# GlacioHack/xdem

Hardware: AMD Instinct MI355X
Metric: Mpixels/s full terrain-attribute set, 40000² f32 DEM; variogram Gpairs/s (higher is better)
Workload: dtype f32 in/out, mixed f64/f32 arithmetic (f64 where cancellation demands: stencil sums, curvature numerators, discriminants); 1 GPU; 40000x40000 float32 fBm DEM (H=0.7, 1000+-300 m, res 10 m), Florinsky fit, geometric curvatures, 11 attributes, device-resident in/out (planes: the library's scattered 32 MiB-piece backing, kept by the allocator's calibration of both placements before the warm-up); partition=1 row block(s), halo depth 2, bytes_per_pixel=48, rccl_ranks=1, visible_gpus=1

## Files before the change

include/xdemhip.h:

```cpp
#ifndef XDEMHIP_H
#define XDEMHIP_H

#include <stdint.h>

#ifdef __cplusplus
extern "C" {
#endif

typedef struct xdemhip_ctx xdemhip_ctx;

enum { XDEMHIP_OK = 0, XDEMHIP_EINVAL = -1, XDEMHIP_ENODEV = -2, XDEMHIP_EHIP = -3, XDEMHIP_ENOMEM = -4,
       XDEMHIP_EUNSUPPORTED = -5 };
enum { XDEMHIP_F32 = 0, XDEMHIP_F64 = 1 };
enum { XDEMHIP_HOST = 0, XDEMHIP_DEVICE = 1 };

enum { XDEMHIP_FIT_HORN = 0, XDEMHIP_FIT_ZEVENBERGTHORNE = 1, XDEMHIP_FIT_FLORINSKY = 2 };
enum { XDEMHIP_CURV_GEOMETRIC = 0, XDEMHIP_CURV_DIRECTIONAL = 1 };
enum { XDEMHIP_TRI_RILEY = 0, XDEMHIP_TRI_WILSON = 1 };

enum {
    XDEMHIP_ATTR_SLOPE = 1u << 0,
    XDEMHIP_ATTR_ASPECT = 1u << 1,
    XDEMHIP_ATTR_HILLSHADE = 1u << 2,
    XDEMHIP_ATTR_CURVATURE = 1u << 3,
    XDEMHIP_ATTR_PROFILE_CURVATURE = 1u << 4,
    XDEMHIP_ATTR_TANGENTIAL_CURVATURE = 1u << 5,
    XDEMHIP_ATTR_PLANFORM_CURVATURE = 1u << 6,
    XDEMHIP_ATTR_FLOWLINE_CURVATURE = 1u << 7,
    XDEMHIP_ATTR_MAX_CURVATURE = 1u << 8,
    XDEMHIP_ATTR_MIN_CURVATURE = 1u << 9,
    XDEMHIP_ATTR_TPI = 1u << 10,
    XDEMHIP_ATTR_TRI = 1u << 11,
    XDEMHIP_ATTR_ROUGHNESS = 1u << 12,
    XDEMHIP_ATTR_RUGOSITY = 1u << 13,
    XDEMHIP_ATTR_FRACTAL_ROUGHNESS = 1u << 14,
    XDEMHIP_ATTR_COUNT = 15
};

int xdemhip_version(void);
int xdemhip_create(int device_id, xdemhip_ctx** out_ctx);
void xdemhip_destroy(xdemhip_ctx* ctx);
const char* xdemhip_last_error(const xdemhip_ctx* ctx);
#define XDEMHIP_OWN_STREAM ((void*)(intptr_t)-1)
int xdemhip_set_stream(xdemhip_ctx* ctx, void* hip_stream);
int xdemhip_synchronize(xdemhip_ctx* ctx);
enum { XDEMHIP_ALLOC_CONTIGUOUS = 1, XDEMHIP_ALLOC_RECYCLED = 2, XDEMHIP_ALLOC_CHUNKED = 4, XDEMHIP_ALLOC_SCATTERED = 8 };
int xdemhip_device_alloc(xdemhip_ctx* ctx, size_t bytes, int flags, void** ptr, int* got_contiguous);
int xdemhip_device_free(xdemhip_ctx* ctx, void* ptr);
int xdemhip_last_kernel_ms(xdemhip_ctx* ctx, float* ms);
int xdemhip_clock_probe(xdemhip_ctx* ctx, void* hip_stream, int sleeps, uint64_t* out_device);
int xdemhip_set_option(xdemhip_ctx* ctx, const char* name, int value);

enum { XDEMHIP_RED_SUM_U64 = 0, XDEMHIP_RED_SUM_F64 = 1, XDEMHIP_RED_MIN_U64 = 2, XDEMHIP_RED_MAX_U64 = 3 };
typedef int (*xdemhip_allreduce_fn)(void* host_array, int64_t count, int kind, void* user);
int xdemhip_set_allreduce(xdemhip_ctx* ctx, xdemhip_allreduce_fn fn, void* user);
typedef int (*xdemhip_allreduce_device_fn)(void* device_array, int64_t count, int kind, void* hip_stream, void* user);
int xdemhip_set_allreduce_device(xdemhip_ctx* ctx, xdemhip_allreduce_device_fn fn, void* user);
int xdemhip_reduction_calls(xdemhip_ctx* ctx, int64_t* host_calls, int64_t* device_calls);
int xdemhip_host_ring_sample(const uint8_t* valid, int64_t ny, int64_t nx, double gsd, int64_t runs, const int64_t* cx, const int64_t* cy,
                             int n_rings, const double* ring_lo, const double* ring_hi, int64_t samples, uint64_t seed, int threads,
                             int64_t* out_idx, int64_t* out_count);
int xdemhip_host_gather_points(const void* values, int dtype, int64_t nx, double gsd, int n_blocks, const int64_t* off, const int64_t* idx,
                               int threads, double* x_out, double* y_out, void* v_out, double* sx_out, double* sy_out, void* sv_out);
int xdemhip_host_count_finite(const void* values, int dtype, int64_t n, int threads, int64_t* n_finite, uint8_t* valid_out);
int xdemhip_set_rank(xdemhip_ctx* ctx, int rank, int world);

int xdemhip_terrain(xdemhip_ctx* ctx, const void* dem, int dem_dtype, int64_t H, int64_t W, int64_t row_stride,
                    int64_t halo_top, int64_t halo_bottom, double resolution, int surface_fit, int curv_method,
                    uint32_t attr_mask, int tri_method, int window_size, double hillshade_altitude_deg,
                    double hillshade_azimuth_deg, double hillshade_z_factor, int degrees, int out_dtype,
                    void* const* out_planes, int memspace);

int xdemhip_fractal_constants(int window_size, int max_q, int* q, double* log_q, double* mean_log_q, double* ss_xx);

int xdemhip_texture_shading(xdemhip_ctx* ctx, const void* dem, int dem_dtype, int64_t H, int64_t W, double alpha, int out_dtype,
                            void* out, int memspace);

typedef struct xdemhip_nk_plan xdemhip_nk_plan;
int xdemhip_nk_create(xdemhip_ctx* ctx, const void* ref, const void* tba, const uint8_t* inlier_mask_or_null, int dtype,
                      int64_t H, int64_t W, int memspace, xdemhip_nk_plan** out_plan, int64_t* n_valid);
int xdemhip_nk_step(xdemhip_nk_plan* plan, double shift_x, double shift_y, double res_x, double res_y, int n_bins,
                    double* vshift, int64_t* n_valid, double* y_mean, double* y_std, double* edges, int64_t* counts,
                    double* medians);
int xdemhip_nk_create_block(xdemhip_ctx* ctx, const void* ref_block, const void* tba_block, const uint8_t* inlier_block_or_null,
                            int dtype, int64_t H, int64_t W, int64_t row_begin, int64_t row_end, int64_t halo_top,
                            int64_t halo_bottom, int memspace, xdemhip_nk_plan** out_plan, int64_t* n_valid);
int xdemhip_nk_set_rows(xdemhip_nk_plan* plan, int64_t row_begin, int64_t row_end, int64_t* n_valid);
int xdemhip_nk_step_fit(xdemhip_nk_plan* plan, double shift_x, double shift_y, double res_x, double res_y, double* vshift,
                        int64_t* n_valid, double* y_mean, double* y_std, double* sums );
int xdemhip_nk_step_values(xdemhip_nk_plan* plan, double shift_x, double shift_y, double res_x, double res_y, int n_bins, double* vshift,
                           int64_t* n_valid, double* y_mean, double* y_std, double* edges , void* y_out,
                           uint16_t* bins_out, int memspace);
int xdemhip_nk_set_bin_edges(xdemhip_nk_plan* plan, const double* edges, int n_edges, int decimal);
#define XDEMHIP_BINSTAT_MEDIAN 0
#define XDEMHIP_BINSTAT_MEAN 1
int xdemhip_nk_set_statistic(xdemhip_nk_plan* plan, int bin_stat);
int xdemhip_nk_get_aux(xdemhip_nk_plan* plan, void* slope_tan, void* aspect, uint8_t* valid);
int xdemhip_nk_subsample(xdemhip_nk_plan* plan, const int64_t* ranks, int64_t k, int memspace, int64_t* n_valid);
int xdemhip_nk_route_counts(xdemhip_nk_plan* plan, int64_t* onepass, int64_t* plain);
int xdemhip_nk_predict_counts(xdemhip_nk_plan* plan, int64_t* predicted, int64_t* predicted_dh_only, int64_t* missed);
void xdemhip_nk_destroy(xdemhip_nk_plan* plan);
int xdemhip_binned_median(xdemhip_ctx* ctx, const void* x, const void* y, int dtype, int64_t n, int n_bins, double* edges,
                          int64_t* counts, double* medians);

typedef struct xdemhip_dh_plan xdemhip_dh_plan;
int xdemhip_dh_create(xdemhip_ctx* ctx, const void* ref, const void* tba, const uint8_t* inlier_mask_or_null, int dtype, int64_t H, int64_t W,
                      int memspace, xdemhip_dh_plan** out_plan, int64_t* n_valid);
int xdemhip_dh_subsample(xdemhip_dh_plan* plan, const int64_t* ranks, int64_t k, int memspace, int64_t* n_drawn);
int xdemhip_dh_poly_moments(xdemhip_dh_plan* plan, int order, int64_t row_offset, int64_t H_global, int64_t W_global, double* m_out,
                            double* r_out, int64_t* count);
int xdemhip_dh_median(xdemhip_dh_plan* plan, double* median, int64_t* count);
int xdemhip_dh_values(xdemhip_dh_plan* plan, void* dh_out, int64_t* col_out, int64_t* row_out, int memspace, int64_t* count);
int xdemhip_dh_shift_nmad(xdemhip_dh_plan* plan, double shift_x, double shift_y, double res_x, double res_y, double nfact, double* median,
                          double* nmad, int64_t* count);
int xdemhip_dh_shift_values(xdemhip_dh_plan* plan, double shift_x, double shift_y, double res_x, double res_y, void* dh_out, int memspace,
                            int64_t* count);
void xdemhip_dh_destroy(xdemhip_dh_plan* plan);

enum { XDEMHIP_VAR_PLANE = 0, XDEMHIP_VAR_ROTATED = 1, XDEMHIP_VAR_REF = 2, XDEMHIP_VAR_TBA = 3 };
enum { XDEMHIP_CORR_GRID = 0, XDEMHIP_CORR_PERBIN = 1, XDEMHIP_CORR_POLY = 2, XDEMHIP_CORR_SUMSIN = 3 };
typedef struct xdemhip_varsrc {
    int kind;
    int dtype;
    const void* plane;
    double cos_t, sin_t, res_x, res_y, offset;
} xdemhip_varsrc;
int xdemhip_dh_restrict_finite(xdemhip_dh_plan* plan, const void* var, int dtype, int memspace, int64_t* n_valid);
int xdemhip_dh_var_columns(xdemhip_dh_plan* plan, int n_var, const xdemhip_varsrc* vars, void* dh_out, void* const* var_out, int memspace,
                           int64_t* count);
int xdemhip_corr_apply(xdemhip_ctx* ctx, const void* elev, int dtype, int64_t H, int64_t W, int kind, int n_var, const xdemhip_varsrc* vars,
                       const int* n_tab, const double* a, const double* b, const double* table, const unsigned char* pass, void* out,
                       int64_t* n_missing, int memspace);

int xdemhip_dh_lzd_gradients(xdemhip_dh_plan* plan, const double* transform6, void* gradx_out, void* grady_out, int memspace);
int xdemhip_dh_lzd_centroid(xdemhip_dh_plan* plan, const double* transform6, double* centroid_out, int64_t* count);
int xdemhip_dh_lzd_normal(xdemhip_dh_plan* plan, const double* transform6, const double* matrix16, const double* centroid3, double* sums_out,
                          int64_t* count);
int xdemhip_dh_lzd_values(xdemhip_dh_plan* plan, const double* transform6, const double* matrix16, const double* centroid3, double* out,
                          int64_t* count);
int xdemhip_apply_matrix_rst(xdemhip_ctx* ctx, const void* dem, int dtype, int64_t H, int64_t W, const double* transform6, const double* matrix16,
                             const double* centroid3_or_null, void* out, int memspace);

typedef struct xdemhip_pts_plan xdemhip_pts_plan;
int xdemhip_pts_create(xdemhip_ctx* ctx, const void* raster, const uint8_t* inlier_mask_or_null, int dtype, int64_t H, int64_t W,
                       const double* transform6, const double* x, const double* y, const void* z, int64_t n_pts, int pts_is_ref, int with_nk_aux,
                       int memspace, xdemhip_pts_plan** out_plan, int64_t* n_valid);
int xdemhip_pts_subsample(xdemhip_pts_plan* plan, const int64_t* ranks, int64_t k, int memspace, int64_t* n_selected);
int xdemhip_pts_selection(xdemhip_pts_plan* plan, int64_t* idx_out_or_null, int64_t* count);
int xdemhip_pts_set_bin_edges(xdemhip_pts_plan* plan, const double* edges_or_null, int n_edges, int decimal);
int xdemhip_pts_nk_step(xdemhip_pts_plan* plan, double shift_x, double shift_y, int n_bins, double* vshift, int64_t* n_valid, double* y_mean,
                        double* y_std, double* edges, int64_t* counts, double* medians);
int xdemhip_pts_step_y(xdemhip_pts_plan* plan, void* y_out, int memspace, int64_t* count);
int xdemhip_pts_shift_nmad(xdemhip_pts_plan* plan, double shift_x, double shift_y, double nfact, double* median, double* nmad, int64_t* count);
int xdemhip_pts_shift_values(xdemhip_pts_plan* plan, double shift_x, double shift_y, void* dh_out, void* slope_out_or_null,
                             void* aspect_out_or_null, int memspace, int64_t* count);
void xdemhip_pts_destroy(xdemhip_pts_plan* plan);
int xdemhip_apply_matrix_pts(xdemhip_ctx* ctx, const double* x, const double* y, const double* z, int64_t n, const double* matrix16,
                             const double* centroid3_or_null, int invert, double* x_out, double* y_out, double* z_out, int memspace);

typedef struct xdemhip_icp xdemhip_icp;
int xdemhip_dh_icp_normals(xdemhip_dh_plan* plan, const double* transform6, void* nx_out, void* ny_out, void* nz_out, int memspace, int64_t* n_valid);
int xdemhip_icp_create_plan(xdemhip_dh_plan* plan, const double* transform6, int with_normals, int standardize, xdemhip_icp** out, double* centroid3,
                            double* std_fac, int64_t* count);
int xdemhip_icp_create_points(xdemhip_ctx* ctx, const double* ref3n, int64_t n, const double* query3m, int64_t m, const double* norms3n_or_null,
                              xdemhip_icp** out);
int xdemhip_icp_cloud(xdemhip_icp* icp, double* out7n);
int xdemhip_icp_grid(xdemhip_icp* icp, double* x0_y0_h, int64_t* gx_gy);
int xdemhip_icp_query(xdemhip_icp* icp, const double* matrix16_or_null, int64_t* ind_out, double* dist_out);
int xdemhip_icp_set_pairs(xdemhip_icp* icp, const int64_t* ind, const double* dist);
int xdemhip_icp_pairs(xdemhip_icp* icp, int picky, int64_t* n_kept, int64_t* query_idx_out, int64_t* ref_idx_out);
int xdemhip_icp_sums(xdemhip_icp* icp, const double* step16, int method, double* sums_out, int64_t* count);
int xdemhip_icp_values(xdemhip_icp* icp, double* out9k);
void xdemhip_icp_destroy(xdemhip_icp* icp);

typedef struct xdemhip_cpd xdemhip_cpd;
int xdemhip_cpd_create_plan(xdemhip_dh_plan* plan, const double* transform6, int standardize, xdemhip_cpd** out, double* centroid3, double* std_fac,
                            int64_t* count);
int xdemhip_cpd_create_points(xdemhip_ctx* ctx, const double* ref3n, int64_t n, const double* tba3m, int64_t m, xdemhip_cpd** out);
int xdemhip_cpd_estep(xdemhip_cpd* cpd, const double* matrix16_or_null, double sigma2_or_nan, double weight, double* sums_out, double* sigma2_used);
int xdemhip_cpd_terms(xdemhip_cpd* cpd, double* p1_out, double* pt1_out, double* px_out);
void xdemhip_cpd_destroy(xdemhip_cpd* cpd);

int xdemhip_poly2d_apply(xdemhip_ctx* ctx, const void* elev, int dtype, int64_t H, int64_t W, int64_t row_offset, const double* coeffs,
// ... 79 lines not shown
```

xdem_amd/_lib.py:

```python
from __future__ import annotations

import contextlib
import ctypes
import os
import threading
import weakref

HERE = os.path.dirname(os.path.abspath(__file__))
LIB_PATH = os.path.join(HERE, "csrc", "libxdemhip.so")

OK = 0
F32, F64 = 0, 1
HOST, DEVICE = 0, 1

_lib = None
_lock = threading.Lock()


THIRDPARTY_DEFAULTS = {"nk_nan_rule": 0, "vario_edge": 0, "vario_diff": 0}
_THIRDPARTY_RANGE = {"nk_nan_rule": (0, 3), "vario_edge": (0, 1), "vario_diff": (0, 1)}


def thirdparty_decision() -> dict:
    import json
# ... 44 lines not shown
            raise XdemHipError(
                f"{LIB_PATH} is missing: build it with `python -c 'import __graft_entry__ as g; g.build()'` "
                "(hipcc --offload-arch=gfx950). xdem_amd has no CPU fallback."
            )
        try:
            import torch
        except Exception:
            pass
        L = ctypes.CDLL(LIB_PATH, mode=ctypes.RTLD_GLOBAL)
        c_ctx = ctypes.c_void_p
        L.xdemhip_version.restype = ctypes.c_int
        L.xdemhip_create.argtypes = [ctypes.c_int, ctypes.POINTER(c_ctx)]
        L.xdemhip_destroy.argtypes = [c_ctx]
        L.xdemhip_destroy.restype = None
        L.xdemhip_last_error.argtypes = [c_ctx]
        L.xdemhip_last_error.restype = ctypes.c_char_p
        L.xdemhip_set_stream.argtypes = [c_ctx, ctypes.c_void_p]
        L.xdemhip_synchronize.argtypes = [c_ctx]
        L.xdemhip_device_alloc.argtypes = [c_ctx, ctypes.c_size_t, ctypes.c_int, ctypes.POINTER(ctypes.c_void_p), ctypes.POINTER(ctypes.c_int)]
        L.xdemhip_device_free.argtypes = [c_ctx, ctypes.c_void_p]
        L.xdemhip_set_option.argtypes = [c_ctx, ctypes.c_char_p, ctypes.c_int]
        L.xdemhip_set_test_switch.argtypes = [c_ctx, ctypes.c_char_p, ctypes.c_int]
        L.xdemhip_set_allreduce.argtypes = [c_ctx, ctypes.c_void_p, ctypes.c_void_p]
        L.xdemhip_set_allreduce_device.argtypes = [c_ctx, ctypes.c_void_p, ctypes.c_void_p]
        L.xdemhip_reduction_calls.argtypes = [c_ctx, ctypes.POINTER(ctypes.c_int64), ctypes.POINTER(ctypes.c_int64)]
        L.xdemhip_set_rank.argtypes = [c_ctx, ctypes.c_int, ctypes.c_int]
        L.xdemhip_last_kernel_ms.argtypes = [c_ctx, ctypes.POINTER(ctypes.c_float)]
        L.xdemhip_clock_probe.argtypes = [c_ctx, ctypes.c_void_p, ctypes.c_int, ctypes.c_void_p]
        L.xdemhip_terrain.argtypes = [
            c_ctx, ctypes.c_void_p, ctypes.c_int, ctypes.c_int64, ctypes.c_int64, ctypes.c_int64, ctypes.c_int64,
            ctypes.c_int64, ctypes.c_double, ctypes.c_int, ctypes.c_int, ctypes.c_uint32, ctypes.c_int, ctypes.c_int,
            ctypes.c_double, ctypes.c_double, ctypes.c_double, ctypes.c_int, ctypes.c_int,
            ctypes.POINTER(ctypes.c_void_p), ctypes.c_int,
        ]
        c_i64p, c_dp = ctypes.POINTER(ctypes.c_int64), ctypes.POINTER(ctypes.c_double)
        L.xdemhip_fractal_constants.argtypes = [ctypes.c_int, ctypes.c_int, ctypes.POINTER(ctypes.c_int), c_dp, c_dp, c_dp]
        L.xdemhip_texture_shading.argtypes = [c_ctx, ctypes.c_void_p, ctypes.c_int, ctypes.c_int64, ctypes.c_int64, ctypes.c_double,
                                              ctypes.c_int, ctypes.c_void_p, ctypes.c_int]
        L.xdemhip_nk_create.argtypes = [c_ctx, ctypes.c_void_p, ctypes.c_void_p, ctypes.c_void_p, ctypes.c_int, ctypes.c_int64,
                                        ctypes.c_int64, ctypes.c_int, ctypes.POINTER(ctypes.c_void_p), c_i64p]
        L.xdemhip_nk_create_block.argtypes = [c_ctx, ctypes.c_void_p, ctypes.c_void_p, ctypes.c_void_p, ctypes.c_int, ctypes.c_int64,
                                              ctypes.c_int64, ctypes.c_int64, ctypes.c_int64, ctypes.c_int64, ctypes.c_int64,
                                              ctypes.c_int, ctypes.POINTER(ctypes.c_void_p), c_i64p]
        L.xdemhip_nk_step.argtypes = [ctypes.c_void_p, ctypes.c_double, ctypes.c_double, ctypes.c_double, ctypes.c_double,
                                      ctypes.c_int, c_dp, c_i64p, c_dp, c_dp, c_dp, c_i64p, c_dp]
        L.xdemhip_nk_step_fit.argtypes = [ctypes.c_void_p, ctypes.c_double, ctypes.c_double, ctypes.c_double, ctypes.c_double,
                                          c_dp, c_i64p, c_dp, c_dp, c_dp]
        L.xdemhip_nk_set_bin_edges.argtypes = [ctypes.c_void_p, c_dp, ctypes.c_int, ctypes.c_int]
        L.xdemhip_nk_get_aux.argtypes = [ctypes.c_void_p, ctypes.c_void_p, ctypes.c_void_p, ctypes.c_void_p]
        L.xdemhip_nk_destroy.argtypes = [ctypes.c_void_p]
        L.xdemhip_nk_destroy.restype = None
        L.xdemhip_binned_median.argtypes = [c_ctx, ctypes.c_void_p, ctypes.c_void_p, ctypes.c_int, ctypes.c_int64, ctypes.c_int,
                                            c_dp, c_i64p, c_dp]
        L.xdemhip_mean_filter_nan.argtypes = [c_ctx, ctypes.c_void_p, ctypes.c_int, ctypes.c_int64, ctypes.c_int64, ctypes.c_int,
                                              ctypes.c_int, ctypes.c_void_p, ctypes.c_void_p, ctypes.POINTER(ctypes.c_int), ctypes.c_int]
        L.xdemhip_binstats_bin_numbers.argtypes = [ctypes.c_void_p, ctypes.c_void_p]
        L.xdemhip_convolution.argtypes = [c_ctx, ctypes.c_void_p, ctypes.c_int, ctypes.c_int64, ctypes.c_int64, ctypes.c_int64, c_dp, ctypes.c_int,
                                          ctypes.c_int, ctypes.c_int, ctypes.c_int, ctypes.c_void_p, ctypes.c_int]
        L.xdemhip_perbin_lookup.argtypes = [c_ctx, ctypes.POINTER(ctypes.c_void_p), ctypes.POINTER(ctypes.c_int), ctypes.c_int, ctypes.c_int64,
                                            ctypes.POINTER(ctypes.c_int), c_dp, c_dp, c_dp, ctypes.c_char_p, ctypes.c_int, ctypes.c_void_p,
                                            c_i64p, ctypes.c_int]
        L.xdemhip_bw_create.argtypes = [c_ctx, ctypes.c_void_p, ctypes.c_void_p, ctypes.c_void_p, ctypes.c_int, ctypes.c_int64, ctypes.c_int64,
                                        ctypes.c_int, c_i64p, ctypes.c_int, ctypes.POINTER(ctypes.c_void_p), c_i64p]
        L.xdemhip_bw_nk_step.argtypes = [ctypes.c_void_p, ctypes.c_void_p, c_dp, c_dp, ctypes.c_double, ctypes.c_double, ctypes.c_int,
                                         c_dp, c_i64p, c_dp, c_dp, c_dp, c_i64p, c_dp]
        L.xdemhip_bw_get_aux.argtypes = [ctypes.c_void_p, ctypes.c_void_p, ctypes.c_void_p, ctypes.c_void_p]
        L.xdemhip_bw_destroy.argtypes = [ctypes.c_void_p]
        L.xdemhip_bw_destroy.restype = None
        L.xdemhip_bw_apply.argtypes = [c_ctx, ctypes.c_void_p, ctypes.c_int, ctypes.c_int64, ctypes.c_int64, c_dp, c_dp, c_dp, c_dp,
                                       ctypes.c_void_p, ctypes.c_int]
        L.xdemhip_shift_bilinear.argtypes = [c_ctx, ctypes.c_void_p, ctypes.c_int, ctypes.c_int64, ctypes.c_int64, ctypes.c_double,
                                             ctypes.c_double, ctypes.c_double, ctypes.c_void_p, ctypes.c_int]
        L.xdemhip_set_allreduce.argtypes = [c_ctx, ctypes.c_void_p, ctypes.c_void_p]
        L.xdemhip_nk_set_rows.argtypes = [ctypes.c_void_p, ctypes.c_int64, ctypes.c_int64, c_i64p]
        L.xdemhip_nk_set_statistic.argtypes = [ctypes.c_void_p, ctypes.c_int]
        L.xdemhip_nk_route_counts.argtypes = [ctypes.c_void_p, c_i64p, c_i64p]
        L.xdemhip_host_ring_sample.argtypes = [ctypes.c_void_p, ctypes.c_int64, ctypes.c_int64, ctypes.c_double, ctypes.c_int64, c_i64p, c_i64p,
                                               ctypes.c_int, c_dp, c_dp, ctypes.c_int64, ctypes.c_uint64, ctypes.c_int, c_i64p, c_i64p]
        L.xdemhip_host_gather_points.argtypes = [ctypes.c_void_p, ctypes.c_int, ctypes.c_int64, ctypes.c_double, ctypes.c_int, c_i64p, c_i64p,
                                                 ctypes.c_int, c_dp, c_dp, ctypes.c_void_p, c_dp, c_dp, ctypes.c_void_p]
        L.xdemhip_nk_step_values.argtypes = [ctypes.c_void_p, ctypes.c_double, ctypes.c_double, ctypes.c_double, ctypes.c_double, ctypes.c_int,
                                             c_dp, c_i64p, c_dp, c_dp, c_dp, ctypes.c_void_p, ctypes.c_void_p, ctypes.c_int]
        L.xdemhip_nk_predict_counts.argtypes = [ctypes.c_void_p, c_i64p, c_i64p, c_i64p]
        L.xdemhip_nk_subsample.argtypes = [ctypes.c_void_p, ctypes.c_void_p, ctypes.c_int64, ctypes.c_int, c_i64p]
        L.xdemhip_host_count_finite.argtypes = [ctypes.c_void_p, ctypes.c_int, ctypes.c_int64, ctypes.c_int, c_i64p, ctypes.c_void_p]
        c_u64p = ctypes.POINTER(ctypes.c_uint64)
        L.xdemhip_pairs_create.argtypes = [c_ctx, ctypes.c_int, ctypes.c_void_p, ctypes.c_void_p, ctypes.c_void_p, ctypes.c_void_p,
                                           ctypes.c_void_p, ctypes.c_void_p, ctypes.c_void_p, ctypes.c_void_p, ctypes.c_int,
                                           ctypes.c_void_p, ctypes.c_int, ctypes.c_int, ctypes.POINTER(ctypes.c_void_p), c_i64p]
        L.xdemhip_pairs_sums.argtypes = [ctypes.c_void_p, ctypes.c_int, c_dp, c_i64p]
        L.xdemhip_pairs_hist.argtypes = [ctypes.c_void_p, ctypes.c_int, ctypes.c_int, c_u64p, c_u64p]
        L.xdemhip_pairs_succ.argtypes = [ctypes.c_void_p, c_u64p, c_u64p]
        L.xdemhip_pairs_medians.argtypes = [ctypes.c_void_p, c_i64p, c_dp]
        L.xdemhip_pairs_link_sorted.argtypes = [ctypes.c_void_p, ctypes.c_void_p]
        L.xdemhip_pairs_link_shadow.argtypes = [ctypes.c_void_p, ctypes.c_void_p]
        L.xdemhip_pairs_takes_brackets.argtypes = [ctypes.c_void_p, ctypes.POINTER(ctypes.c_int)]
        L.xdemhip_pairs_destroy.argtypes = [ctypes.c_void_p]
        L.xdemhip_pairs_destroy.restype = None
        c_ip = ctypes.POINTER(ctypes.c_int)
        L.xdemhip_binstats_create.argtypes = [c_ctx, ctypes.c_void_p, ctypes.c_int, ctypes.c_int64, ctypes.c_int,
                                              ctypes.POINTER(ctypes.c_void_p)]
        L.xdemhip_binstats_add_var.argtypes = [ctypes.c_void_p, ctypes.c_void_p, ctypes.c_int, ctypes.c_int]
        L.xdemhip_binstats_finalize.argtypes = [ctypes.c_void_p, c_i64p, c_dp, c_dp]
        L.xdemhip_binstats_run.argtypes = [ctypes.c_void_p, ctypes.c_int, c_ip, c_dp, c_ip, c_ip, ctypes.c_int, ctypes.c_int,
                                           ctypes.c_double, c_i64p, c_dp, c_dp]
        L.xdemhip_binstats_destroy.argtypes = [ctypes.c_void_p]
        L.xdemhip_binstats_destroy.restype = None
        L.xdemhip_cov_double_sum.argtypes = [c_ctx, c_dp, c_dp, c_dp, ctypes.c_int64, c_dp, c_dp, c_dp, ctypes.c_int64, ctypes.c_int, c_ip,
                                             c_dp, c_dp, c_dp, c_dp, ctypes.c_int]
        L.xdemhip_nmad.argtypes = [c_ctx, ctypes.c_void_p, ctypes.c_int, ctypes.c_int64, ctypes.c_double, ctypes.c_double,
                                   ctypes.c_int, c_dp, c_dp, c_i64p]
        L.xdemhip_interp_grid_linear.argtypes = [c_ctx, ctypes.c_int, c_dp, c_ip, c_dp, ctypes.POINTER(ctypes.c_void_p), c_ip,
                                                 ctypes.c_int64, ctypes.c_double, c_dp, ctypes.c_int]
        L.xdemhip_dh_create.argtypes = [c_ctx, ctypes.c_void_p, ctypes.c_void_p, ctypes.c_void_p, ctypes.c_int, ctypes.c_int64,
                                        ctypes.c_int64, ctypes.c_int, ctypes.POINTER(ctypes.c_void_p), c_i64p]
        L.xdemhip_dh_subsample.argtypes = [ctypes.c_void_p, ctypes.c_void_p, ctypes.c_int64, ctypes.c_int, c_i64p]
        L.xdemhip_dh_poly_moments.argtypes = [ctypes.c_void_p, ctypes.c_int, ctypes.c_int64, ctypes.c_int64, ctypes.c_int64, c_dp, c_dp,
                                              c_i64p]
        L.xdemhip_dh_median.argtypes = [ctypes.c_void_p, c_dp, c_i64p]
        L.xdemhip_dh_values.argtypes = [ctypes.c_void_p, ctypes.c_void_p, ctypes.c_void_p, ctypes.c_void_p, ctypes.c_int, c_i64p]
        L.xdemhip_dh_shift_nmad.argtypes = [ctypes.c_void_p, ctypes.c_double, ctypes.c_double, ctypes.c_double, ctypes.c_double, ctypes.c_double,
                                            c_dp, c_dp, c_i64p]
        L.xdemhip_dh_shift_values.argtypes = [ctypes.c_void_p, ctypes.c_double, ctypes.c_double, ctypes.c_double, ctypes.c_double,
                                              ctypes.c_void_p, ctypes.c_int, c_i64p]
        L.xdemhip_dh_destroy.argtypes = [ctypes.c_void_p]
        L.xdemhip_dh_destroy.restype = None
        L.xdemhip_dh_lzd_gradients.argtypes = [ctypes.c_void_p, c_dp, ctypes.c_void_p, ctypes.c_void_p, ctypes.c_int]
        L.xdemhip_dh_lzd_centroid.argtypes = [ctypes.c_void_p, c_dp, c_dp, c_i64p]
        L.xdemhip_dh_lzd_normal.argtypes = [ctypes.c_void_p, c_dp, c_dp, c_dp, c_dp, c_i64p]
        L.xdemhip_dh_lzd_values.argtypes = [ctypes.c_void_p, c_dp, c_dp, c_dp, c_dp, c_i64p]
        L.xdemhip_dh_restrict_finite.argtypes = [ctypes.c_void_p, ctypes.c_void_p, ctypes.c_int, ctypes.c_int, c_i64p]
        L.xdemhip_dh_var_columns.argtypes = [ctypes.c_void_p, ctypes.c_int, ctypes.POINTER(VarSrc), ctypes.c_void_p,
                                             ctypes.POINTER(ctypes.c_void_p), ctypes.c_int, c_i64p]
        L.xdemhip_corr_apply.argtypes = [c_ctx, ctypes.c_void_p, ctypes.c_int, ctypes.c_int64, ctypes.c_int64, ctypes.c_int, ctypes.c_int,
                                         ctypes.POINTER(VarSrc), c_ip, c_dp, c_dp, c_dp, ctypes.c_char_p, ctypes.c_void_p, c_i64p, ctypes.c_int]
        L.xdemhip_dh_icp_normals.argtypes = [ctypes.c_void_p, c_dp, ctypes.c_void_p, ctypes.c_void_p, ctypes.c_void_p, ctypes.c_int, c_i64p]
        L.xdemhip_icp_create_plan.argtypes = [ctypes.c_void_p, c_dp, ctypes.c_int, ctypes.c_int, ctypes.POINTER(ctypes.c_void_p), c_dp, c_dp, c_i64p]
        L.xdemhip_icp_create_points.argtypes = [c_ctx, c_dp, ctypes.c_int64, c_dp, ctypes.c_int64, c_dp, ctypes.POINTER(ctypes.c_void_p)]
        L.xdemhip_icp_cloud.argtypes = [ctypes.c_void_p, c_dp]
        L.xdemhip_icp_grid.argtypes = [ctypes.c_void_p, c_dp, c_i64p]
        L.xdemhip_icp_query.argtypes = [ctypes.c_void_p, c_dp, c_i64p, c_dp]
        L.xdemhip_icp_set_pairs.argtypes = [ctypes.c_void_p, c_i64p, c_dp]
        L.xdemhip_icp_pairs.argtypes = [ctypes.c_void_p, ctypes.c_int, c_i64p, c_i64p, c_i64p]
        L.xdemhip_icp_sums.argtypes = [ctypes.c_void_p, c_dp, ctypes.c_int, c_dp, c_i64p]
        L.xdemhip_icp_values.argtypes = [ctypes.c_void_p, c_dp]
        L.xdemhip_icp_destroy.argtypes = [ctypes.c_void_p]
        L.xdemhip_icp_destroy.restype = None
        L.xdemhip_cpd_create_plan.argtypes = [ctypes.c_void_p, c_dp, ctypes.c_int, ctypes.POINTER(ctypes.c_void_p), c_dp, c_dp, c_i64p]
        L.xdemhip_cpd_create_points.argtypes = [c_ctx, c_dp, ctypes.c_int64, c_dp, ctypes.c_int64, ctypes.POINTER(ctypes.c_void_p)]
        L.xdemhip_cpd_estep.argtypes = [ctypes.c_void_p, c_dp, ctypes.c_double, ctypes.c_double, c_dp, c_dp]
        L.xdemhip_cpd_terms.argtypes = [ctypes.c_void_p, c_dp, c_dp, c_dp]
        L.xdemhip_cpd_destroy.argtypes = [ctypes.c_void_p]
        L.xdemhip_cpd_destroy.restype = None
        L.xdemhip_apply_matrix_rst.argtypes = [c_ctx, ctypes.c_void_p, ctypes.c_int, ctypes.c_int64, ctypes.c_int64, c_dp, c_dp, c_dp,
                                               ctypes.c_void_p, ctypes.c_int]
        L.xdemhip_pts_create.argtypes = [c_ctx, ctypes.c_void_p, ctypes.c_void_p, ctypes.c_int, ctypes.c_int64, ctypes.c_int64, c_dp,
                                         ctypes.c_void_p, ctypes.c_void_p, ctypes.c_void_p, ctypes.c_int64, ctypes.c_int, ctypes.c_int,
                                         ctypes.c_int, ctypes.POINTER(ctypes.c_void_p), c_i64p]
        L.xdemhip_pts_subsample.argtypes = [ctypes.c_void_p, ctypes.c_void_p, ctypes.c_int64, ctypes.c_int, c_i64p]
        L.xdemhip_pts_selection.argtypes = [ctypes.c_void_p, ctypes.c_void_p, c_i64p]
        L.xdemhip_pts_set_bin_edges.argtypes = [ctypes.c_void_p, c_dp, ctypes.c_int, ctypes.c_int]
        L.xdemhip_pts_nk_step.argtypes = [ctypes.c_void_p, ctypes.c_double, ctypes.c_double, ctypes.c_int, c_dp, c_i64p, c_dp, c_dp, c_dp,
                                          c_i64p, c_dp]
        L.xdemhip_pts_step_y.argtypes = [ctypes.c_void_p, ctypes.c_void_p, ctypes.c_int, c_i64p]
        L.xdemhip_pts_shift_nmad.argtypes = [ctypes.c_void_p, ctypes.c_double, ctypes.c_double, ctypes.c_double, c_dp, c_dp, c_i64p]
        L.xdemhip_pts_shift_values.argtypes = [ctypes.c_void_p, ctypes.c_double, ctypes.c_double, ctypes.c_void_p, ctypes.c_void_p,
# ... 160 lines not shown
            self.check(self._L.xdemhip_set_allreduce(self.handle, None, None))
            self.check(self._L.xdemhip_set_rank(self.handle, 0, 0))
            return
        import torch.distributed as dist

        pg = None if group == "world" else group
        self.check(self._L.xdemhip_set_rank(self.handle, dist.get_rank(pg), dist.get_world_size(pg)))
        hook = make_reduce_hook(group, self.device)
        CB = ctypes.CFUNCTYPE(ctypes.c_int, ctypes.c_void_p, ctypes.c_int64, ctypes.c_int, ctypes.c_void_p)
        self._hook = CB(hook)
        self.check(self._L.xdemhip_set_allreduce(self.handle, ctypes.cast(self._hook, ctypes.c_void_p), None))
        if device_side is None:
            import torch.distributed as dist

            device_side = dist.get_backend(None if group == "world" else group) == "nccl"
        if device_side:
            CBD = ctypes.CFUNCTYPE(ctypes.c_int, ctypes.c_void_p, ctypes.c_int64, ctypes.c_int, ctypes.c_void_p, ctypes.c_void_p)
            self._dev_hook = CBD(make_device_reduce_hook(group, self.device))
            self.check(self._L.xdemhip_set_allreduce_device(self.handle, ctypes.cast(self._dev_hook, ctypes.c_void_p), None))
        else:
            self._dev_hook = None
            self.check(self._L.xdemhip_set_allreduce_device(self.handle, None, None))

    def reduction_calls(self) -> tuple[int, int]:
        h, d = ctypes.c_int64(), ctypes.c_int64()
        self.check(self._L.xdemhip_reduction_calls(self.handle, ctypes.byref(h), ctypes.byref(d)))
        return int(h.value), int(d.value)

    def synchronize(self) -> None:
        self.check(self._L.xdemhip_synchronize(self.handle))

    def device_tensor(self, shape, dtype="float32", contiguous: bool = True, recycled: bool = False, chunked: bool = False,
                      scattered: bool = False):
        import numpy as np
        import torch

        np_dt = np.dtype(dtype)
        count = int(np.prod(shape))
        ptr, got = ctypes.c_void_p(), ctypes.c_int()
        flags = 8 if scattered else (4 if chunked else ((1 if contiguous else 0) | (2 if recycled else 0)))
        nbytes = count * np_dt.itemsize
        pooled = self._take_pooled(nbytes, flags)
        if pooled:
            torch.cuda.synchronize(self.device)
            ptr.value, got.value = pooled, 0
        else:
            rc = self._L.xdemhip_device_alloc(self.handle, nbytes, flags, ctypes.byref(ptr), ctypes.byref(got))
            if rc != OK and self._pool:
                self.release_pool()
                rc = self._L.xdemhip_device_alloc(self.handle, nbytes, flags, ctypes.byref(ptr), ctypes.byref(got))
            self.check(rc)
        owner = _OwnedDeviceArray(self, int(ptr.value), count, np_dt.str, nbytes, flags)
        t = torch.as_tensor(owner, device=torch.device("cuda", self.device)).view(*shape)
        t.xdem_contiguous = bool(got.value)
        return t

    def _take_pooled(self, nbytes: int, flags: int) -> int:
        with self._pool_lock:
            for i, (b, f, p) in enumerate(self._pool):
                if b == nbytes and f == flags:
                    del self._pool[i]
                    return p
        return 0

    def _give_back(self, ptr: int, nbytes: int, flags: int) -> None:
        if flags == 8 and 0 < nbytes <= self._pool_cap:
            evict = []
            with self._pool_lock:
                self._pool.append((nbytes, flags, ptr))
                while sum(b for b, _, _ in self._pool) > self._pool_cap:
                    evict.append(self._pool.pop(0))
            for _, _, p in evict:
                self._L.xdemhip_device_free(self.handle, ctypes.c_void_p(p))
            return
        self._L.xdemhip_device_free(self.handle, ctypes.c_void_p(ptr))

    def release_pool(self) -> None:
        with self._pool_lock:
            items, self._pool = self._pool, []
        for _, _, p in items:
            self._L.xdemhip_device_free(self.handle, ctypes.c_void_p(p))

    TEST_SWITCHES = frozenset(("terrain_stream", "terrain_order", "terrain_ring_wait", "terrain_window_lds", "nk_narrow",
                               "vario_grid", "vario_runs", "vario_sort", "hypso_seg_lds", "pts_tile_order", "bw_seg_lds"))

    def set_option(self, name: str, value: int) -> None:
        fn = self._L.xdemhip_set_test_switch if name in self.TEST_SWITCHES else self._L.xdemhip_set_option
        self.check(fn(self.handle, name.encode(), int(value)))
        self.options[name] = int(value)

    @contextlib.contextmanager
    def option_scope(self, name: str, value: int):
        with self.call_lock:
            prev = self.options.get(name, 0)
            if int(value) != prev:
                self.set_option(name, value)
            try:
                yield
            finally:
                if int(value) != prev:
                    self.set_option(name, prev)

    def clock_probe(self, stream, out, sleeps: int = 2000) -> None:
        self.check(self._L.xdemhip_clock_probe(self.handle, ctypes.c_void_p(int(stream.cuda_stream)), int(sleeps), ctypes.c_void_p(int(out.data_ptr()))))

    def last_kernel_ms(self) -> float:
        ms = ctypes.c_float()
        self.check(self._L.xdemhip_last_kernel_ms(self.handle, ctypes.byref(ms)))
        return float(ms.value)

    def adopt(self, obj) -> None:
        self._dependants.add(obj)

    def close(self) -> None:
        if getattr(self, "handle", None):
            for obj in list(getattr(self, "_dependants", ())):
                try:
                    obj.close()
                except Exception:
                    pass
            self.release_pool()
            self._L.xdemhip_destroy(self.handle)
            self.handle = None

    def __del__(self) -> None:
        try:
            self.close()
        except Exception:
            pass


_default_ctx: dict[int, Context] = {}
_ctx_lock = threading.Lock()
_tls = threading.local()


class use_context:

    def __init__(self, ctx: Context):
        self.ctx = ctx

    def __enter__(self):
        self.prev = getattr(_tls, "ctx", None)
        _tls.ctx = self.ctx
        return self.ctx

    def __exit__(self, *exc):
        _tls.ctx = self.prev
        return False


def default_context(device: int | None = None) -> Context:
    cur = getattr(_tls, "ctx", None)
    if cur is not None and (device is None or device == cur.device):
        return cur
    if device is None:
        device = int(os.environ.get("XDEM_AMD_DEVICE", os.environ.get("LOCAL_RANK", "0")))
    if device not in _default_ctx:
        with _ctx_lock:
            if device not in _default_ctx:
                _default_ctx[device] = Context(device)
    return _default_ctx[device]
```

xdem_amd/coreg.py:

```python
from __future__ import annotations

import ctypes
import logging
import warnings
from typing import Any, Callable

import numpy as np
import scipy.optimize

from . import _lib
from . import epc as _epc
from ._coregbase import NO_VALID, CoregPipeline, _Plan, _Step, apply_translation, draw, raster_pair
from ._coregbase import subsample_ranks, subsample_valid_mask
from .biascorr import Deramp, DhPlan, VerticalShift, _check_weights, polynomial_2d
from .bincorr import BiasCorr, DirectionalBias, TerrainBias, rotated_x
from .rigid import (LZD, apply_matrix, invert_matrix, matrix_from_translations_rotations,
                    translations_rotations_from_matrix, _make_matrix_valid)
from .icp import ICP, nearest
from .cpd import CPD, cpd_expectation, cpd_update
from .epc import EPC
from .blockwise import BlockwiseCoreg, tiling_grid
from .spatialstats import nmad

TWO_CLOUDS = ("This pre-processing function is only intended for raster-point or raster-raster methods, "
# ... 66 lines not shown
        if group is not None and block is None:
            import torch.distributed as dist

            from .dist import row_block

            pg = None if group == "world" else group
            r0, r1 = row_block(self.shape[0], dist.get_world_size(pg), dist.get_rank(pg))
            self.ctx.set_allreduce(group)
            self.ctx.check(self.ctx._L.xdemhip_nk_set_rows(self.handle, r0, r1, ctypes.byref(nv)))
            self.n_valid = int(nv.value)

    def step(self, shift_x: float, shift_y: float, res: tuple[float, float], n_bins: int = 72) -> dict[str, Any]:
        n_bins = getattr(self, "_n_custom_bins", None) or int(n_bins)
        if getattr(self, "_bin_callable", None) is not None:
            return self._step_callable(shift_x, shift_y, res, n_bins)
        edges = np.empty(n_bins + 1, dtype=np.float64)
        counts = np.empty(n_bins, dtype=np.int64)
        med = np.empty(n_bins, dtype=np.float64)
        vshift, ymean, ystd = ctypes.c_double(), ctypes.c_double(), ctypes.c_double()
        nv = ctypes.c_int64()
        dp, ip = ctypes.POINTER(ctypes.c_double), ctypes.POINTER(ctypes.c_int64)
        rc = self.ctx._L.xdemhip_nk_step(self.handle, float(shift_x), float(shift_y), float(res[0]), float(res[1]), int(n_bins),
                                         ctypes.byref(vshift), ctypes.byref(nv), ctypes.byref(ymean), ctypes.byref(ystd),
                                         edges.ctypes.data_as(dp), counts.ctypes.data_as(ip), med.ctypes.data_as(dp))
        if rc != _lib.OK:
            self._raise_step_error(rc)
        return {"vshift": vshift.value, "n_valid": int(nv.value), "y_mean": ymean.value, "y_std": ystd.value,
                "edges": edges, "counts": counts, "medians": med}

    def _step_callable(self, shift_x: float, shift_y: float, res: tuple[float, float], n_bins: int) -> dict[str, Any]:
        if self.group is not None:
            raise NotImplementedError("a bin_statistic other than np.nanmedian / np.nanmean needs all values of a bin in one process: "
                                      "not available for partitioned (group=...) fits")
        if getattr(self, "_vals", None) is None:
            self._vals = (np.empty(self.shape, dtype=self.dtype), np.empty(self.shape, dtype=np.uint16))
        y, bins = self._vals
        edges = np.empty(n_bins + 1, dtype=np.float64)
        vshift, ymean, ystd = ctypes.c_double(), ctypes.c_double(), ctypes.c_double()
        nv = ctypes.c_int64()
        dp = ctypes.POINTER(ctypes.c_double)
        rc = self.ctx._L.xdemhip_nk_step_values(self.handle, float(shift_x), float(shift_y), float(res[0]), float(res[1]), int(n_bins),
                                                ctypes.byref(vshift), ctypes.byref(nv), ctypes.byref(ymean), ctypes.byref(ystd),
                                                edges.ctypes.data_as(dp), y.ctypes.data, bins.ctypes.data, _lib.HOST)
        if rc != _lib.OK:
            self._raise_step_error(rc)
        ok = (bins != 0xFFFF) & np.isfinite(y)
        b, v = bins[ok], y[ok]
        counts = np.bincount(b, minlength=n_bins).astype(np.int64)
        from ._binstat_host import binned_statistic_host

        stat = binned_statistic_host(self._bin_callable, b, v, n_bins)
        return {"vshift": vshift.value, "n_valid": int(nv.value), "y_mean": ymean.value, "y_std": ystd.value,
                "edges": edges, "counts": counts, "medians": stat}

    def _raise_step_error(self, rc: int) -> None:
        msg = self.ctx._L.xdemhip_last_error(self.ctx.handle).decode()
        if "no more valid values" in msg:
            raise ValueError(
                "The subsample contains no more valid values. This can happen is the horizontal shift to "
                "correct is very large, or if the algorithm diverged. To ensure all possible points can "
                "be used at any iteration step, use subsample=1."
            )
        if "halo too small" in msg:
            raise HaloTooSmall(msg)
        raise _lib.XdemHipError(f"libxdemhip status {rc}: {msg}")

    def step_fit(self, shift_x: float, shift_y: float, res: tuple[float, float]) -> dict[str, Any]:
        sums = np.empty(10, dtype=np.float64)
        vshift, ymean, ystd = ctypes.c_double(), ctypes.c_double(), ctypes.c_double()
        nv = ctypes.c_int64()
        dp = ctypes.POINTER(ctypes.c_double)
        rc = self.ctx._L.xdemhip_nk_step_fit(self.handle, float(shift_x), float(shift_y), float(res[0]), float(res[1]),
                                             ctypes.byref(vshift), ctypes.byref(nv), ctypes.byref(ymean), ctypes.byref(ystd),
                                             sums.ctypes.data_as(dp))
        if rc != _lib.OK:
            self._raise_step_error(rc)
        return {"vshift": vshift.value, "n_valid": int(nv.value), "y_mean": ymean.value, "y_std": ystd.value, "sums": sums}

    def route_counts(self) -> dict[str, int]:
        a, c = ctypes.c_int64(), ctypes.c_int64()
        self.ctx.check(self.ctx._L.xdemhip_nk_route_counts(self.handle, ctypes.byref(a), ctypes.byref(c)))
        p, d, m = ctypes.c_int64(), ctypes.c_int64(), ctypes.c_int64()
        self.ctx.check(self.ctx._L.xdemhip_nk_predict_counts(self.handle, ctypes.byref(p), ctypes.byref(d), ctypes.byref(m)))
        return {"onepass": int(a.value), "plain": int(c.value), "predicted": int(p.value),
                "predicted_dh_only": int(d.value), "predict_missed": int(m.value)}

    def set_bin_edges(self, edges) -> None:
        dp = ctypes.POINTER(ctypes.c_double)
        if edges is None:
            self.ctx.check(self.ctx._L.xdemhip_nk_set_bin_edges(self.handle, None, 0, 0))
            self._n_custom_bins = None
            return
        e = np.ascontiguousarray(edges, dtype=np.float64).ravel()
        decimal = int(-np.log10(np.diff(e.astype(self.dtype)).min())) + 6
        self.ctx.check(self.ctx._L.xdemhip_nk_set_bin_edges(self.handle, e.ctypes.data_as(dp), int(e.size), decimal))
        self._n_custom_bins = int(e.size) - 1

    def set_statistic(self, bin_statistic) -> None:
        sid = _bin_statistic_id(bin_statistic)
        self._bin_callable = bin_statistic if sid == 2 else None
        self.ctx.check(self.ctx._L.xdemhip_nk_set_statistic(self.handle, 0 if sid == 2 else sid))

    def aux(self):
        st = np.empty(self.shape, dtype=self.dtype)
        asp = np.empty(self.shape, dtype=self.dtype)
        valid = np.empty(self.shape, dtype=np.uint8)
        self.ctx.check(self.ctx._L.xdemhip_nk_get_aux(self.handle, st.ctypes.data, asp.ctypes.data, valid.ctypes.data))
        return st, asp, valid.astype(bool)

    def subsample(self, ranks: np.ndarray) -> int:
        ranks = np.ascontiguousarray(ranks, dtype=np.int64)
        nv = ctypes.c_int64()
        self.ctx.check(self.ctx._L.xdemhip_nk_subsample(self.handle, ranks.ctypes.data, int(ranks.size), _lib.HOST, ctypes.byref(nv)))
        self.n_valid = int(nv.value)
        return self.n_valid

    def close(self) -> None:
        hooked = getattr(self, "handle", None) and getattr(self.ctx, "handle", None) and getattr(self, "group", None) is not None
        super().close()
        if hooked:
            self.ctx.set_allreduce(None)


def binned_median(x: np.ndarray, y: np.ndarray, n_bins: int = 72, ctx: _lib.Context | None = None):
    x = np.ascontiguousarray(x).ravel()
    y = np.ascontiguousarray(y).ravel()
    dt = np.float64 if np.float64 in (x.dtype, y.dtype) else np.float32
    x, y = x.astype(dt, copy=False), y.astype(dt, copy=False)
    ctx = ctx or _lib.default_context()
    edges = np.empty(n_bins + 1, dtype=np.float64)
    counts = np.empty(n_bins, dtype=np.int64)
    med = np.empty(n_bins, dtype=np.float64)
    dp, ip = ctypes.POINTER(ctypes.c_double), ctypes.POINTER(ctypes.c_int64)
    ctx.check(ctx._L.xdemhip_binned_median(ctx.handle, x.ctypes.data, y.ctypes.data, _lib.F32 if dt == np.float32 else _lib.F64,
                                           x.size, int(n_bins), edges.ctypes.data_as(dp), counts.ctypes.data_as(ip),
                                           med.ctypes.data_as(dp)))
    return edges, counts, med


def _bin_fit_from_step(det: dict[str, Any], fit_optimizer: Callable[..., Any], dtype) -> tuple[float, float, float]:
    p0 = (3 * det["y_std"] / (2**0.5), 0.0, det["y_mean"])
    edges = det["edges"]
    mids = 0.5 * (edges[:-1] + edges[1:])
    med = det["medians"]
    ok = np.isfinite(med) & np.isfinite(mids)
    if np.all(~ok):
        raise ValueError("Only NaN values after binning, did you pass the right bin edges?")
    results = fit_optimizer(f=_nuth_kaab_fit_func, xdata=mids[ok], ydata=med[ok], p0=p0, sigma=None, absolute_sigma=True)
    a, b, c = results[0]
    return a * np.sin(b), a * np.cos(b), c


def _fit_from_sums(det: dict[str, Any]) -> tuple[float, float, float]:
    n, sc, ss, scc, sss, scs, sy, syc, sys_, _ = det["sums"]
    m = np.array([[scc, scs, sc], [scs, sss, ss], [sc, ss, n]], dtype=np.float64)
    rhs = np.array([syc, sys_, sy], dtype=np.float64)
    a_, b_, c_ = np.linalg.lstsq(m, rhs, rcond=None)[0]
    return float(b_), float(a_), float(c_)


def _check_unbinned_optimizer(fit_optimizer, bin_before_fit: bool) -> None:
    import scipy.optimize

    if not bin_before_fit and fit_optimizer is not None and fit_optimizer is not scipy.optimize.curve_fit:
        raise NotImplementedError(
            "bin_before_fit=False is solved from least-squares sums on the GPU, which equals scipy.optimize.curve_fit only; "
            "a custom fit_optimizer would need every point on the host. Use bin_before_fit=True with it."
        )
# ... 295 lines not shown
```

xdem_amd/csrc/capi.hip:

```cpp
#include <math.h>
#include <string.h>

#include <functional>
#include <mutex>
#include <thread>
#include <vector>

#include "common.h"

#define XDEMHIP_VERSION_NUM 100

extern "C" {

int xdemhip_version(void) { return XDEMHIP_VERSION_NUM; }

int xdemhip_create(int device_id, xdemhip_ctx** out_ctx) {
    if (!out_ctx) return XDEMHIP_EINVAL;
    *out_ctx = nullptr;
    int n = 0;
    if (hipGetDeviceCount(&n) != hipSuccess || n <= 0) return XDEMHIP_ENODEV;
    if (device_id < 0 || device_id >= n) return XDEMHIP_ENODEV;
    xdemhip_ctx* c = new xdemhip_ctx();
    c->device = device_id;
    if (hipSetDevice(device_id) != hipSuccess) { delete c; return XDEMHIP_EHIP; }
// ... 185 lines not shown
bool device_free_chunked(void* p) {
    ChunkedAlloc c;
    {
        std::lock_guard<std::mutex> lock(g_chunk_mu);
        size_t i = 0;
        for (; i < g_chunked.size(); ++i)
            if (g_chunked[i].base == p) break;
        if (i == g_chunked.size()) return false;
        c = std::move(g_chunked[i]);
        g_chunked.erase(g_chunked.begin() + (long)i);
    }
    (void)hipDeviceSynchronize();
    chunked_release(c, c.pieces.size());
    return true;
}
}

int xdemhip_device_alloc(xdemhip_ctx* ctx, size_t bytes, int flags, void** ptr, int* got_contiguous) {
    if (!ctx || !ptr || bytes == 0) return ctx ? xd_fail(ctx, XDEMHIP_EINVAL, "bad argument") : XDEMHIP_EINVAL;
    XD_HIP_CHECK(ctx, hipSetDevice(ctx->device));
    if (flags & (XDEMHIP_ALLOC_CHUNKED | XDEMHIP_ALLOC_SCATTERED)) {
        *ptr = nullptr;
        if (got_contiguous) *got_contiguous = 0;
        const bool scattered = (flags & XDEMHIP_ALLOC_SCATTERED) != 0;
        size_t piece_mb = scattered ? 32 : 64;
        if (const char* e = getenv("XDEMHIP_SCATTER_PIECE_MB")) {
            const long v = atol(e);
            if (scattered && v >= 1 && v <= 4096) piece_mb = (size_t)v;
        }
        return device_alloc_chunked(ctx, bytes, piece_mb << 20, scattered, ptr);
    }
    const bool contiguous = (flags & XDEMHIP_ALLOC_CONTIGUOUS) != 0;
    if (flags & XDEMHIP_ALLOC_RECYCLED) {
        void* first = nullptr;
        int rc = device_alloc_once(ctx, bytes, contiguous, &first, nullptr);
        if (rc) return rc;
        const size_t touch = bytes < ((size_t)64 << 20) ? bytes : ((size_t)64 << 20);
        (void)hipMemsetAsync(first, 0, touch, ctx->stream);
        (void)hipMemsetAsync(static_cast<char*>(first) + (bytes - touch), 0, touch, ctx->stream);
        (void)hipStreamSynchronize(ctx->stream);
        XD_HIP_CHECK(ctx, hipFree(first));
    }
    return device_alloc_once(ctx, bytes, contiguous, ptr, got_contiguous);
}

int xdemhip_device_free(xdemhip_ctx* ctx, void* ptr) {
    if (!ctx) return XDEMHIP_EINVAL;
    if (!ptr) return XDEMHIP_OK;
    XD_HIP_CHECK(ctx, hipSetDevice(ctx->device));
    if (device_free_chunked(ptr)) return XDEMHIP_OK;
    XD_HIP_CHECK(ctx, hipFree(ptr));
    return XDEMHIP_OK;
}

int xdemhip_synchronize(xdemhip_ctx* ctx) {
    if (!ctx) return XDEMHIP_EINVAL;
    XD_HIP_CHECK(ctx, hipSetDevice(ctx->device));
    XD_HIP_CHECK(ctx, hipStreamSynchronize(ctx->stream));
    return XDEMHIP_OK;
}

namespace {
struct XdOpt { const char* name; int lo, hi; int xdemhip_ctx::*field; const char* what; };
const XdOpt kOptions[] = {
    {"host_chunk_mb", 0, 1 << 30, &xdemhip_ctx::host_chunk_mb, "host_chunk_mb must be >= 0"},
    {"host_chunk_rows", 0, 1 << 30, &xdemhip_ctx::host_chunk_rows, "host_chunk_rows must be >= 0"},
    {"pairs_launch_cap", 0, 1 << 30, &xdemhip_ctx::pairs_launch_cap, "pairs_launch_cap must be >= 0"},
    {"terrain_nonfinite", 0, 1, &xdemhip_ctx::terrain_nonfinite, "terrain_nonfinite: 0 window rule (SciPy engine), 1 arithmetic rule (Numba engine)"},
    {"terrain_math", 0, 2, &xdemhip_ctx::terrain_math, "terrain_math: 0 mixed precision, 1 float64, 2 lean"},
    {"vario_edge", 0, 1, &xdemhip_ctx::vario_edge, "vario_edge: 0 or 1"},
    {"vario_diff", 0, 1, &xdemhip_ctx::vario_diff, "vario_diff: 0 or 1"},
    {"nk_nan_rule", 0, 3, &xdemhip_ctx::nk_nan_rule, "nk_nan_rule: 0 4tap, 1 weighted, 2 dilate3x3, 3 dilate_cross"},
    {"selection", 0, 3, &xdemhip_ctx::selection_mode, "selection: 0 auto, 1 plain, 2 degenerate brackets, 3 bracketed"},
    {"nk_fused", 0, 1, &xdemhip_ctx::nk_fused, "nk_fused: 0 or 1"},
    {"nk_fused_dist", 0, 1, &xdemhip_ctx::nk_fused_dist, "nk_fused_dist: 0 or 1"},
    {"nk_predict", 0, 1, &xdemhip_ctx::nk_predict, "nk_predict: 0 or 1"},
};
const XdOpt kTestSwitches[] = {
    {"terrain_stream", 0, 512, &xdemhip_ctx::terrain_stream, "terrain_stream: 0, 1, 2, 3, 128, 256 or 512"},
    {"terrain_order", 0, 3, &xdemhip_ctx::terrain_order, "terrain_order: 0 XCD bands, 1 natural order, 2 permuted strips, 3 column-major strips"},
    {"terrain_ring_wait", 0, 1, &xdemhip_ctx::terrain_ring_wait, "terrain_ring_wait: 0 counted wait, 1 vmcnt(0)"},
    {"terrain_window_lds", 0, 1, &xdemhip_ctx::terrain_window_lds, "terrain_window_lds: 0 or 1"},
    {"nk_narrow", -1, 2, &xdemhip_ctx::nk_narrow, "nk_narrow: -1 (adaptive), 0, 1 or 2"},
    {"vario_grid", 0, 1, &xdemhip_ctx::vario_grid, "vario_grid: 0 or 1"},
    {"vario_runs", 0, 1, &xdemhip_ctx::vario_runs, "vario_runs: 0 or 1"},
    {"vario_sort", 0, 1, &xdemhip_ctx::vario_sort, "vario_sort: 0 or 1"},
    {"pts_tile_order", 0, 1, &xdemhip_ctx::pts_tile_order, "pts_tile_order: 0 or 1"},
    {"bw_seg_lds", 0, 4096, &xdemhip_ctx::bw_seg_lds, "bw_seg_lds: 0 (default: 4096) or 1 to 4096 values"},
    {"hypso_seg_lds", 0, 16384, &xdemhip_ctx::hypso_seg_lds, "hypso_seg_lds: 0 (default: 8192) or 1 to 16384 values"},
};
int xd_set_from(xdemhip_ctx* ctx, const XdOpt* tab, size_t n, const char* name, int value, bool* found) {
    *found = false;
    for (size_t k = 0; k < n; ++k)
        if (const XdOpt& o = tab[k]; strcmp(o.name, name) == 0) {
            *found = true;
            if (value < o.lo || value > o.hi) return xd_fail(ctx, XDEMHIP_EINVAL, o.what);
            ctx->*(o.field) = value;
            return XDEMHIP_OK;
        }
    return XDEMHIP_OK;
}
}

int xdemhip_set_option(xdemhip_ctx* ctx, const char* name, int value) {
    if (!ctx || !name) return XDEMHIP_EINVAL;
    if (strcmp(name, "host_release") == 0) {
        for (int q = 0; q < 2; ++q) {
            if (ctx->stage_in[q]) (void)hipHostFree(ctx->stage_in[q]);
            if (ctx->stage_out[q]) (void)hipHostFree(ctx->stage_out[q]);
            ctx->stage_in[q] = ctx->stage_out[q] = nullptr;
        }
        ctx->stage_in_bytes = ctx->stage_out_bytes = 0;
        return XDEMHIP_OK;
    }
    if (strcmp(name, "host_copy_threads") == 0) {
        if (value < 0 || value > xdemhip_ctx::MAX_COPY_THREADS) return xd_fail(ctx, XDEMHIP_EINVAL, "host_copy_threads must be 0..16");
        ctx->host_copy_threads = value ? value : 8;
        return XDEMHIP_OK;
    }
    bool found = false;
    const int rc = xd_set_from(ctx, kOptions, sizeof kOptions / sizeof kOptions[0], name, value, &found);
    if (found) return rc;
    for (const XdOpt& o : kTestSwitches)
        if (strcmp(o.name, name) == 0) return xd_fail(ctx, XDEMHIP_EINVAL, std::string(name) + " is a test switch, not an option: xdemhip_set_test_switch (include/xdemhip_test.h)");
    return xd_fail(ctx, XDEMHIP_EINVAL, std::string("unknown option: ") + name);
}

int xdemhip_set_test_switch(xdemhip_ctx* ctx, const char* name, int value) {
    if (!ctx || !name) return XDEMHIP_EINVAL;
    if (strcmp(name, "terrain_stream") == 0 && !(value == 0 || value == 1 || value == 2 || value == 3 || value == 128 || value == 256 || value == 512))
        return xd_fail(ctx, XDEMHIP_EINVAL, "terrain_stream: 0, 1, 2, 3, 128, 256 or 512");
    bool found = false;
    const int rc = xd_set_from(ctx, kTestSwitches, sizeof kTestSwitches / sizeof kTestSwitches[0], name, value, &found);
    if (found) return rc;
    return xd_fail(ctx, XDEMHIP_EINVAL, std::string("unknown test switch: ") + name);
}

int xdemhip_last_kernel_ms(xdemhip_ctx* ctx, float* ms) {
    if (!ctx || !ms) return XDEMHIP_EINVAL;
    if (!ctx->timed) return xd_fail(ctx, XDEMHIP_EINVAL, "no timed launch on this context yet");
    XD_HIP_CHECK(ctx, hipEventSynchronize(ctx->ev_stop));
    XD_HIP_CHECK(ctx, hipEventElapsedTime(ms, ctx->ev_start, ctx->ev_stop));
    return XDEMHIP_OK;
}

static __global__ void xd_clock_probe_kernel(uint64_t* out, int sleeps) {
    const uint64_t t0 = wall_clock64(), c0 = clock64();
    for (int i = 0; i < sleeps; ++i) __builtin_amdgcn_s_sleep(127);
    const uint64_t t1 = wall_clock64(), c1 = clock64();
    if (threadIdx.x == 0) { out[0] = c1 - c0; out[1] = t1 - t0; }
}

int xdemhip_clock_probe(xdemhip_ctx* ctx, void* hip_stream, int sleeps, uint64_t* out_device) {
    if (!ctx || !out_device || sleeps < 1) return XDEMHIP_EINVAL;
    XD_HIP_CHECK(ctx, hipSetDevice(ctx->device));
    hipLaunchKernelGGL(xd_clock_probe_kernel, dim3(1), dim3(64), 0, static_cast<hipStream_t>(hip_stream), out_device, sleeps);
    XD_HIP_CHECK(ctx, hipGetLastError());
    return XDEMHIP_OK;
}

int xdemhip_fractal_constants(int window_size, int max_q, int* q, double* log_q, double* mean_log_q, double* ss_xx) {
    if (window_size < 3 || (window_size & 1) == 0 || window_size > 1023 || !q || !log_q || !mean_log_q || !ss_xx)
        return XDEMHIP_EINVAL;
    int qs[24];
    double x[24];
    const int n = xd::fractal_constants(window_size, qs, x, mean_log_q, ss_xx);
// ... 216 lines not shown
```

xdem_amd/csrc/common.h:

```cpp
#pragma once
#include <hip/hip_runtime.h>
#include <stdint.h>
#include <stdio.h>
#include <string.h>
#include <string>
#include <thread>
#include <vector>

#include "../../include/xdemhip.h"

struct xdemhip_ctx {
    int device = 0;
    hipStream_t own_stream = nullptr;
    hipStream_t stream = nullptr;
    hipEvent_t ev_start = nullptr, ev_stop = nullptr, ev_copy = nullptr;
    static constexpr int MAX_COPY_THREADS = 16;
    hipStream_t copy_streams[MAX_COPY_THREADS] = {};
    int host_copy_threads = 8;
    void* stage_in[2] = {nullptr, nullptr};
    void* stage_out[2] = {nullptr, nullptr};
    size_t stage_in_bytes = 0, stage_out_bytes = 0;
    int pairs_launch_cap = 0;
    bool timed = false;
    int num_cu = 256;
    xdemhip_allreduce_fn allreduce = nullptr;
    void* allreduce_user = nullptr;
    xdemhip_allreduce_device_fn allreduce_dev = nullptr;
    void* allreduce_dev_user = nullptr;
    int64_t n_red_host = 0, n_red_dev = 0;
    int rank = 0, world = 0;
    int nk_fused_dist = 1;
    int host_chunk_rows = 0;
    int host_chunk_mb = 0;
    int nk_narrow = -1;
    int vario_runs = 1;
    int vario_sort = 1;
    int nk_predict = 1;
    int nk_fused = 1;
    int terrain_stream = 1;
    int terrain_order = 0;
    int terrain_window_lds = 1;
    int terrain_ring_wait = 0;
    int terrain_nonfinite = 0;
    int* nf_flag = nullptr;
    int terrain_math = 2;
    int vario_grid = 1;
    int vario_edge = 0;
    int vario_diff = 0;
    int nk_nan_rule = 0;
    int pts_tile_order = 0;
    int hypso_seg_lds = 0;
    int bw_seg_lds = 0;
    int selection_mode = 0;
    unsigned char* pin = nullptr;
    size_t pin_cap = 0, pin_used = 0;
    struct Pending { void* dst; size_t off, bytes; };
    std::vector<Pending> pending;
    std::string err;
};

#define XD_HIP_CHECK(ctx, expr)                                                                   \
    do {                                                                                          \
        hipError_t _e = (expr);                                                                   \
        if (_e != hipSuccess) {                                                                   \
            char _b[512];                                                                         \
            snprintf(_b, sizeof _b, "%s failed: %s (%s:%d)", #expr, hipGetErrorString(_e), __FILE__, __LINE__); \
            (ctx)->err = _b;                                                                      \
            return XDEMHIP_EHIP;                                                                  \
        }                                                                                         \
    } while (0)

inline int xd_fail(xdemhip_ctx* ctx, int code, const std::string& msg) {
    if (ctx) ctx->err = msg;
    return code;
}

inline int launched(xdemhip_ctx* ctx, const char* what) {
    return hipGetLastError() == hipSuccess ? XDEMHIP_OK : xd_fail(ctx, XDEMHIP_EHIP, std::string(what) + " launch failed");
}

inline int xd_sync(xdemhip_ctx* ctx);

struct XdBuffers {
    xdemhip_ctx* ctx;
    const char* who;
    int rc = XDEMHIP_OK;
    struct Out { void* host; const void* dev; size_t bytes; };
    std::vector<void*> owned;
    std::vector<Out> outs;
    XdBuffers(xdemhip_ctx* c, const char* w) : ctx(c), who(w) {}
    void* alloc(size_t bytes) {
        void* p = nullptr;
        if (rc != XDEMHIP_OK) return nullptr;
        if (hipMalloc(&p, bytes) != hipSuccess) {
            (void)hipGetLastError();
            rc = xd_fail(ctx, XDEMHIP_ENOMEM, std::string("hipMalloc failed (") + who + ")");
            return nullptr;
        }
        if (p) owned.push_back(p);
        return p;
    }
    template <typename T> T* alloc(size_t count) { return static_cast<T*>(alloc(count * sizeof(T))); }
    template <typename T> const T* input(const T* src, size_t bytes, int memspace) {
        if (memspace == XDEMHIP_DEVICE || !src) return src;
        T* d = static_cast<T*>(alloc(bytes));
        if (d && hipMemcpyAsync(d, src, bytes, hipMemcpyHostToDevice, ctx->stream) != hipSuccess) {
            rc = xd_fail(ctx, XDEMHIP_EHIP, std::string("H2D copy failed (") + who + ")");
            return nullptr;
        }
        return d;
    }
    template <typename T> T* output(T* dst, size_t bytes, int memspace) {
        if (memspace == XDEMHIP_DEVICE || !dst) return dst;
        T* d = static_cast<T*>(alloc(bytes));
        if (d) outs.push_back({dst, d, bytes});
        return d;
    }
    int finish() {
        for (const Out& o : outs)
            if (rc == XDEMHIP_OK && hipMemcpyAsync(o.host, o.dev, o.bytes, hipMemcpyDeviceToHost, ctx->stream) != hipSuccess)
// ... 162 lines not shown
```

xdem_amd/csrc/nk_onepass.h:

```cpp
#pragma once

namespace xd {

__device__ __forceinline__ unsigned long long cm_nlt(float a, float b) { unsigned long long m; asm("v_cmp_nlt_f32_e64 %0, %1, %2" : "=s"(m) : "v"(a), "v"(b)); return m; }
__device__ __forceinline__ unsigned long long cm_ngt(float a, float b) { unsigned long long m; asm("v_cmp_ngt_f32_e64 %0, %1, %2" : "=s"(m) : "v"(a), "v"(b)); return m; }
__device__ __forceinline__ unsigned long long cm_nlt(double a, double b) { unsigned long long m; asm("v_cmp_nlt_f64_e64 %0, %1, %2" : "=s"(m) : "v"(a), "v"(b)); return m; }
__device__ __forceinline__ unsigned long long cm_ngt(double a, double b) { unsigned long long m; asm("v_cmp_ngt_f64_e64 %0, %1, %2" : "=s"(m) : "v"(a), "v"(b)); return m; }
__device__ __forceinline__ uint32_t sel_mask(uint32_t a, uint32_t b, unsigned long long mask) {
    uint32_t r;
    asm("v_cndmask_b32_e64 %0, %1, %2, %3" : "=v"(r) : "v"(a), "v"(b), "s"(mask));
    return r;
}
__device__ __forceinline__ float sel_mask(float a, float b, unsigned long long mask) { return __uint_as_float(sel_mask(__float_as_uint(a), __float_as_uint(b), mask)); }
__device__ __forceinline__ int sel_mask(int a, int b, unsigned long long mask) { return (int)sel_mask((uint32_t)a, (uint32_t)b, mask); }
__device__ __forceinline__ uint32_t* sel_mask_ptr(uint32_t* a, uint32_t* b, unsigned long long mask) {
    typedef __attribute__((address_space(3))) uint32_t* lp;
    const uint32_t r = sel_mask((uint32_t)(uintptr_t)(lp)a, (uint32_t)(uintptr_t)(lp)b, mask);
    return (uint32_t*)(lp)(uintptr_t)r;
}

template <typename T> struct FzEps;
template <> struct FzEps<float> { static constexpr float rel = 4e-6f, grow = 1.00002f, tiny = 1e-37f; };
template <> struct FzEps<double> { static constexpr double rel = 1e-14, grow = 1.0000000001, tiny = 1e-300; };
__device__ __forceinline__ float fz_rcp(float x) { return __builtin_amdgcn_rcpf(x); }
__device__ __forceinline__ double fz_rcp(double x) { return 1.0 / x; }

template <typename T>
__global__ void nk_fz_prep_kernel(const DhStats* stats, const unsigned long long* ext_survivors, int nb, int custom_edges, T* edges,
                                  BinCacheRec* rec, int force, unsigned long long* ctr) {
    typedef typename KeyT<T>::type K;
    if (threadIdx.x != 0 || blockIdx.x != 0) return;
    if (ext_survivors[0] == 0 || ext_survivors[1] == 0) { ctr[3] = 1ull; ctr[6] = 1ull; }
    if (!custom_edges) make_edges_into<T>((double)val_of((K)stats->asp_min), (double)val_of((K)stats->asp_max), nb, edges);
    const double e0 = (double)edges[0], eN = (double)edges[nb];
    rec->fresh = (!force && rec->nb == nb && rec->e0 == e0 && rec->eN == eN) ? 1 : 0;
}

template <typename T> __device__ __forceinline__ uint16_t fz_digitize(const T* e, double inv_width, int nb, T x, int last_decimal) {
    int idx = (int)(((double)x - (double)e[0]) * inv_width);
    idx = idx < 0 ? 0 : (idx > nb ? nb : idx);
    while (idx > 0 && !(e[idx] <= x)) --idx;
    while (idx < nb && e[idx + 1] <= x) ++idx;
    if (!(e[0] <= x)) idx = -1;
    if (idx == nb && on_last_edge<T>(x, e[nb], last_decimal)) idx = nb - 1;
    return (idx >= 0 && idx < nb) ? (uint16_t)idx : (uint16_t)0xFFFF;
}
template <typename T>
__global__ __launch_bounds__(256) void nk_bin_fill_kernel(const T* __restrict__ aspect, int64_t n, const T* __restrict__ edges, int nb,
                                                          int last_decimal, const BinCacheRec* rec, nk_bin_t* __restrict__ bcache) {
    if (rec->fresh == 1) return;
    extern __shared__ __attribute__((aligned(16))) unsigned char fz_smem[];
    T* e = reinterpret_cast<T*>(fz_smem);
    for (int k = threadIdx.x; k <= nb; k += blockDim.x) e[k] = edges[k];
    __syncthreads();
    const double inv_width = (double)nb / ((double)e[nb] - (double)e[0]);
    for (int64_t p = (int64_t)blockIdx.x * blockDim.x + threadIdx.x; p < n; p += (int64_t)gridDim.x * blockDim.x)
        bcache[p] = nk_bin8(fz_digitize<T>(e, inv_width, nb, aspect[p], last_decimal));
}

template <typename T>
__global__ __launch_bounds__(256) void nk_sample_dh_kernel(const T* __restrict__ ref_m, const T* __restrict__ tba, NkGeom g, int64_t q0, int64_t n,
                                                           double invW, int64_t n_slots, T* __restrict__ s_d, SelReset reset) {
    if (reset.base) select_reset_slice(reset, (int64_t)blockIdx.x * blockDim.x + threadIdx.x, (int64_t)gridDim.x * blockDim.x);
    for (int64_t i = (int64_t)blockIdx.x * blockDim.x + threadIdx.x; i < n_slots; i += (int64_t)gridDim.x * blockDim.x) {
        const int64_t p = (sel_sampled_line(i >> SEL_LINE_LOG2) << SEL_LINE_LOG2) + (i & (SEL_LINE - 1));
        T out = (T)NAN;
        if (p < n) {
            const int64_t q = q0 + p;
            int64_t li, j;
            row_col(q, g.W, invW, li, j);
            const BiTap t = bi_locate(g, li + g.roff, j);
            const BiVals<T> tv = bi_load<T>(tba, t);
            T val;
            const bool in = bi_value<T>(g, tba, t, tv.a00, tv.a01, tv.a10, tv.a11, val);
            const T d = t_sub(ref_m[q], val);
            if (in && t_finite(d)) out = d;
        }
        s_d[i] = out;
    }
}

template <typename T>
__device__ __forceinline__ bool nk_vhat_of(uint64_t sample_count, typename KeyT<T>::type lo, typename KeyT<T>::type hi, T& vhat, T& delta) {
    typedef typename KeyT<T>::type K;
    if (sample_count == 0) { vhat = (T)0; delta = (T)0; return false; }
    const K mid = (K)(lo + (K)((K)(hi - lo) >> 1));
    const double vl = (double)val_of(lo), vh = (double)val_of(hi), vm = (double)val_of(mid);
    const double d = fmax(vm - vl, vh - vm);
    vhat = val_of(mid);
    T df = (T)(d * 1.000001 + 1e-300);
    if ((double)df < d * 1.0000005) df = (T)((double)df * 1.000001);
    delta = df;
    return (vl <= vm && vm <= vh) && t_finite((T)vl) && t_finite((T)vh);
}

template <typename T>
__global__ __launch_bounds__(256) void nk_sample_y_kernel(T* __restrict__ s_v, uint16_t* __restrict__ s_b, const T* __restrict__ slope_tan,
                                                          const nk_bin_t* __restrict__ bcache, int64_t n, int64_t n_slots, const T* vhat_p,
                                                          const typename KeyT<T>::type* klo_d = nullptr, const typename KeyT<T>::type* khi_d = nullptr,
                                                          T* vhat_out = nullptr, T* delta_out = nullptr, unsigned long long* ctr = nullptr,
                                                          SelReset reset = SelReset()) {
    T vhat;
    if (klo_d) {
        typedef typename KeyT<T>::type K;
        T delta;
        const K lo = klo_d[0], hi = khi_d[0];
        const bool ok = nk_vhat_of<T>((lo == (K)0 && hi == (K)~(K)0) ? 0u : 1u, lo, hi, vhat, delta);
        if (blockIdx.x == 0 && threadIdx.x == 0) {
            *vhat_out = vhat;
            *delta_out = delta;
            if (!ok) ctr[3] = 1ull;
        }
    } else {
        vhat = *vhat_p;
    }
    if (reset.base) select_reset_slice(reset, (int64_t)blockIdx.x * blockDim.x + threadIdx.x, (int64_t)gridDim.x * blockDim.x);
    for (int64_t i = (int64_t)blockIdx.x * blockDim.x + threadIdx.x; i < n_slots; i += (int64_t)gridDim.x * blockDim.x) {
        const int64_t p = (sel_sampled_line(i >> SEL_LINE_LOG2) << SEL_LINE_LOG2) + (i & (SEL_LINE - 1));
        const T d = s_v[i];
        T y = (T)NAN;
        uint16_t b = 0xFFFF;
        if (p < n && d == d) {
            b = nk_bin16(bcache[p]);
            y = t_div(t_sub(d, vhat), slope_tan[p]);
            if (b == 0xFFFF || !(y == y)) y = (T)NAN;
        }
        s_v[i] = y;
        s_b[i] = b;
    }
}

template <typename T>
__global__ __launch_bounds__(256) void nk_sample_dy_kernel(const T* __restrict__ ref_m, const T* __restrict__ tba, NkGeom g, int64_t q0, int64_t n,
                                                           double invW, int64_t n_slots, T* __restrict__ s_v, uint16_t* __restrict__ s_b,
                                                           const T* __restrict__ slope_tan , const nk_bin_t* __restrict__ bcache ,
                                                           const typename KeyT<T>::type* klo_d, const typename KeyT<T>::type* khi_d, T* vhat_out,
                                                           T* delta_out, unsigned long long* ctr, SelReset reset) {
    typedef typename KeyT<T>::type K;
    T vhat, delta;
    const K lo = klo_d[0], hi = khi_d[0];
    const bool ok = nk_vhat_of<T>((lo == (K)0 && hi == (K)~(K)0) ? 0u : 1u, lo, hi, vhat, delta);
    if (blockIdx.x == 0 && threadIdx.x == 0) {
        *vhat_out = vhat;
        *delta_out = delta;
        if (!ok) ctr[3] = 1ull;
    }
    if (reset.base) select_reset_slice(reset, (int64_t)blockIdx.x * blockDim.x + threadIdx.x, (int64_t)gridDim.x * blockDim.x);
    for (int64_t i = (int64_t)blockIdx.x * blockDim.x + threadIdx.x; i < n_slots; i += (int64_t)gridDim.x * blockDim.x) {
        const int64_t p = (sel_sampled_line(i >> SEL_LINE_LOG2) << SEL_LINE_LOG2) + (i & (SEL_LINE - 1));
        T y = (T)NAN;
        uint16_t b = 0xFFFF;
        if (p < n) {
            const int64_t q = q0 + p;
            int64_t li, j;
            row_col(q, g.W, invW, li, j);
            const BiTap t = bi_locate(g, li + g.roff, j);
            const BiVals<T> tv = bi_load<T>(tba, t);
            T val;
            const bool in = bi_value<T>(g, tba, t, tv.a00, tv.a01, tv.a10, tv.a11, val);
            const T d = t_sub(ref_m[q], val);
            if (in && t_finite(d)) {
                b = nk_bin16(bcache[p]);
                y = t_div(t_sub(d, vhat), slope_tan[p]);
                if (b == 0xFFFF || !(y == y)) y = (T)NAN;
            }
        }
        s_v[i] = y;
        s_b[i] = b;
    }
}

constexpr int NK_PREDICT_MAX_BINS = 128;
template <typename T> struct NkPredicted { T dlo, dhi; T lo[NK_PREDICT_MAX_BINS], hi[NK_PREDICT_MAX_BINS]; };
template <typename T>
__global__ __launch_bounds__(64) void nk_predict_kernel(const NkPredicted<T> pr, int nb, typename KeyT<T>::type* klo_d, typename KeyT<T>::type* khi_d,
                                                        uint32_t* rbs_d, T* vhat, T* delta, typename KeyT<T>::type* klo_y,
                                                        typename KeyT<T>::type* khi_y, uint32_t* rbs_y, unsigned long long* ctr) {
    typedef typename KeyT<T>::type K;
    const int lane = threadIdx.x;
    K r = 0;
    for (int b = lane; b < nb; b += 64) {
        K lo = (K)0, hi = (K)~(K)0;
        if (pr.lo[b] <= pr.hi[b]) { lo = key_of(pr.lo[b]); hi = key_of(pr.hi[b]); }
        klo_y[b] = lo;
        khi_y[b] = hi;
        const K d = hi >= lo ? (K)(hi - lo) : (K)0;
        r = d > r ? d : r;
    }
    for (int off = 32; off > 0; off >>= 1) {
        const K o = k_shfl_down(r, off);
        r = o > r ? o : r;
    }
    if (lane == 0) {
        *rbs_y = rebase_shift_of(r);
        const K lo = key_of(pr.dlo), hi = key_of(pr.dhi);
        *klo_d = lo;
        *khi_d = hi;
        *rbs_d = rebase_shift_of(hi >= lo ? (K)(hi - lo) : (K)0);
        T v = (T)0, d = (T)0;
        if (!(pr.dlo <= pr.dhi) || !nk_vhat_of<T>(1u, lo, hi, v, d)) ctr[3] = 1ull;
        *vhat = v;
        *delta = d;
    }
}

constexpr int NK_SUMS_THREADS = 256;
__device__ __forceinline__ void nk_sums_reduce(const double* __restrict__ wg_sums, int n_wg, double (*s_part)[5], double* out5) {
    const int t = threadIdx.x;
    if (t < NK_SUMS_THREADS) {
        double a[5] = {0.0, 0.0, 0.0, 0.0, 0.0};
        for (int w = t; w < n_wg; w += NK_SUMS_THREADS)
#pragma unroll
            for (int k = 0; k < 5; ++k) a[k] += wg_sums[(size_t)w * 5 + k];
#pragma unroll
        for (int k = 0; k < 5; ++k) s_part[t][k] = a[k];
    }
    __syncthreads();
    for (int half = NK_SUMS_THREADS / 2; half > 0; half >>= 1) {
        if (t < half)
#pragma unroll
            for (int k = 0; k < 5; ++k) s_part[t][k] += s_part[t + half][k];
        __syncthreads();
    }
    if (t < 5) out5[t] = s_part[0][t];
}

constexpr int NKZ_ROWS = 8;
constexpr int NKZ_PF = 4;
constexpr int NKZ_CAP = 1024;
template <typename T> struct FzPair { T lo, hi; };

constexpr int NKZ_CHUNK_MAX = 256;
template <typename T, int RULE>
__global__ __launch_bounds__(256, (sizeof(T) == 8 ? (RULE == 2 ? 4 : 5) : (RULE == 2 ? 6 : 7))) void nk_fused_kernel(const T* __restrict__ ref, const T* __restrict__ tba, const T* __restrict__ slope_tan,
                                                       const nk_bin_t* __restrict__ bcache, NkGeom g, int64_t row0, int64_t row1, int64_t nbuf,
                                                       int nb, int copies, const typename KeyT<T>::type* __restrict__ klo_p,
                                                       const typename KeyT<T>::type* __restrict__ khi_p, const T* vhat_p, const T* delta_p,
                                                       const typename KeyT<T>::type* __restrict__ klo_y,
                                                       const typename KeyT<T>::type* __restrict__ khi_y, uint64_t* cnt_d ,
                                                       uint64_t* cls_y , T* cd_vals, int64_t cd_cap,
                                                       T* cy_d, T* cy_st, uint16_t* cy_b, int64_t cy_cap,
                                                       unsigned long long* ctr ,
                                                       double* wg_sums ,
                                                       const uint64_t* __restrict__ badbits = nullptr, int64_t bad_wpr = 0) {
    typedef typename KeyT<T>::type K;
    constexpr int SEG = NKZ_CAP / 4;
    static_assert(SEG >= 2 * 64, "a segment holds at least two rows of candidates");
    constexpr int SEG_D = 128;
    __shared__ NkRowTab tab[NKZ_CHUNK_MAX + 1];
    __shared__ T stage_d[4 * SEG_D + 4];
    __shared__ T sy_d[NKZ_CAP + 4];
    __shared__ T sy_st[NKZ_CAP + 4];
    __shared__ uint16_t sy_b[NKZ_CAP + 4];
    __shared__ int s_cnt[2][4];
    __shared__ unsigned long long s_base[2];
    __shared__ unsigned long long s_red[4][3];
    __shared__ double s_sum[4][5];
    extern __shared__ __attribute__((aligned(16))) unsigned char fz_smem[];
    FzPair<T>* lohi = reinterpret_cast<FzPair<T>*>(fz_smem);
    uint32_t* c = reinterpret_cast<uint32_t*>(lohi + nb);
    const int cs = (3 * nb) | 1;
    const int lane = threadIdx.x & 63;
    const int wave = __builtin_amdgcn_readfirstlane((int)(threadIdx.x >> 6));
    for (int k = threadIdx.x; k < nb; k += blockDim.x) { lohi[k].lo = val_of(klo_y[k]); lohi[k].hi = val_of(khi_y[k]); }
    for (int k = threadIdx.x; k < cs * copies; k += blockDim.x) c[k] = 0;
    const K klo = *klo_p, khi = *khi_p;
    const T vhat = *vhat_p;
    const T dgrow = (T)(*delta_p * FzEps<T>::grow);
    const int64_t chunk = (row1 - row0 + gridDim.y - 1) / gridDim.y;
    const int64_t i0 = row0 + (int64_t)blockIdx.y * chunk;
    const int nrow = __builtin_amdgcn_readfirstlane((int)((i0 + chunk < row1 ? i0 + chunk : row1) - i0));
    for (int r = threadIdx.x; r <= nrow && r <= NKZ_CHUNK_MAX; r += blockDim.x) {
        const BiAxis a = bi_axis(i0 + (r < nrow ? r : nrow - 1), g.dr, g.H, RULE);
        int64_t kl = a.k0 - g.roff;
        kl = (a.in && kl >= 0 && kl + a.d1 < nbuf) ? kl : 0;
        NkRowTab e;
        e.fr = a.f; e.k0l = (int)kl; e.flags = (a.in ? 1 : 0) | (a.d1 ? 2 : 0);
        const int64_t rn = nk_nearest(a.pos);
        e.rnl = (rn >= 1 && rn + 1 < g.H && rn - g.roff >= 0 && rn - g.roff < nbuf) ? (int)(rn - g.roff) : -1;
        e.pad_ = 0;
        tab[r] = e;
    }
    __syncthreads();
    if (nrow <= 0) {
        if (threadIdx.x < 5) wg_sums[((size_t)blockIdx.y * gridDim.x + blockIdx.x) * 5 + threadIdx.x] = 0.0;
        return;
    }
    uint32_t* cc = c + (threadIdx.x % (unsigned)copies) * cs;
    const int64_t j = (int64_t)blockIdx.x * blockDim.x + threadIdx.x;
    const bool jin = j < g.W;
    const BiAxis col = bi_axis(j, g.dc, g.W, RULE);
    const bool cin = col.in & jin;
    int64_t cnc = nk_nearest(col.pos);
    cnc = cnc < -1 ? -1 : (cnc > g.W ? g.W : cnc);
    const uint32_t bad_ob = (uint32_t)(2 + (cnc >> 5)) * 4u;
    const int bad_sh = (int)(cnc & 31);
    const char* const bad_base = reinterpret_cast<const char*>(badbits);
    const int64_t bad_rowb = bad_wpr * 8;
    const unsigned long long m_cin = __builtin_amdgcn_ballot_w64(cin);
    const uint32_t c0b = (cin ? (uint32_t)col.k0 : 0u) * (uint32_t)sizeof(T);
    const uint32_t c1b = c0b + (cin ? (uint32_t)col.d1 : 0u) * (uint32_t)sizeof(T);
    const uint32_t jl = jin ? (uint32_t)j : 0u;
    const double fc = col.f;
    auto hlerp = [&](T a, T b) -> double {
        const double v0 = a, v1 = b;
        return t_add(v0, t_mul(fc, t_sub(v1, v0)));
    };
    uint32_t n_all = 0, n_below = 0, n_in = 0;
    int held_d = 0, held_y = 0;
    T* const seg_d = stage_d + wave * SEG_D;
    const int trash_d = 4 * SEG_D + wave - wave * SEG_D;
    T* const seg_yd = sy_d + wave * SEG;
    T* const seg_ys = sy_st + wave * SEG;
    uint16_t* const seg_yb = sy_b + wave * SEG;
    const int trash = NKZ_CAP + wave - wave * SEG;
    typedef __attribute__((address_space(3))) uint32_t* lds_u32p;
    auto lds_addr = [](uint32_t* p) { return (uint32_t)(uintptr_t)(lds_u32p)p; };
    auto lds_u32 = [](uint32_t a) { return (uint32_t*)(lds_u32p)(uintptr_t)a; };
    const uint32_t dummy_a = lds_addr(c + cs * copies + lane);
    const uint32_t cls_a = lds_addr(cc), cls_b = lds_addr(cc + nb), cls_c = lds_addr(cc + 2 * nb);
    auto block_flush = [&](int threshold) {
        if (lane == 0) { s_cnt[0][wave] = held_d; s_cnt[1][wave] = held_y; }
        __syncthreads();
        int n0[4], n1[4];
#pragma unroll
        for (int w = 0; w < 4; ++w) { n0[w] = __builtin_amdgcn_readfirstlane(s_cnt[0][w]); n1[w] = __builtin_amdgcn_readfirstlane(s_cnt[1][w]); }
        const int m0 = max(max(n0[0], n0[1]), max(n0[2], n0[3])), m1 = max(max(n1[0], n1[1]), max(n1[2], n1[3]));
        const bool f0 = m0 > (threshold < SEG_D / 2 ? threshold : SEG_D / 2), f1 = m1 > threshold;
// ... 1084 lines not shown
```

xdem_amd/csrc/nuthkaab.hip:

```cpp
#include <math.h>
#include <string.h>

#include <vector>

#include "common.h"
#include "select.h"
#include "select_run.h"
#include "nk_geom.h"
#include "nk_aux.h"
#include "rank_select.h"

namespace xd {

static __global__ void nk_stats_init_kernel(DhStats* s) {
    if (threadIdx.x == 0) { s->asp_min = ~(uint64_t)0; s->asp_max = 0; }
}
static __global__ void nk_step_init_kernel(DhStats* s, uint64_t* fz, int64_t fz_words, unsigned long long* ext_survivors ) {
    for (int64_t w = threadIdx.x; w < fz_words; w += blockDim.x) fz[w] = 0;
    if (threadIdx.x == 0) { s->asp_min = ~(uint64_t)0; s->asp_max = 0; ext_survivors[0] = 0; ext_survivors[1] = 0; }
}

template <typename T>
__global__ __launch_bounds__(256) void nk_dh_kernel(const T* __restrict__ ref, const T* __restrict__ tba,
                                                    const uint8_t* __restrict__ valid, const T* __restrict__ aspect,
                                                    NkGeom g, T* __restrict__ dh, DhStats* stats, int64_t row0, int64_t row1) {
    typedef typename KeyT<T>::type K;
    K kmin = ~(K)0, kmax = 0;
    const int64_t j = (int64_t)blockIdx.x * blockDim.x + threadIdx.x;
    const BiAxis col = bi_axis(j, g.dc, g.W, g.rule);
    if (j < g.W)
    for (int64_t i = row0 + blockIdx.y; i < row1; i += gridDim.y) {
        const int64_t p = (i - g.roff) * g.W + j;
        const BiTap t = bi_combine(g, bi_axis(i, g.dr, g.H, g.rule), col);
        const BiVals<T> tv = bi_load<T>(tba, t);
            const T a00 = tv.a00, a01 = tv.a01, a10 = tv.a10, a11 = tv.a11;
        const T rv = ref[p];
        const T av = aspect[p];
        const uint8_t vd = valid[p];
        T val;
        const bool ok = bi_value<T>(g, tba, t, a00, a01, a10, a11, val) & (vd != 0);
        T out = t_sub(rv, val);
        if (ok && t_finite(out)) {
            const K ka = key_of(av);
            kmin = ka < kmin ? ka : kmin;
            kmax = ka > kmax ? ka : kmax;
        } else {
            out = (T)NAN;
        }
        dh[p] = out;
    }
    for (int off = 32; off > 0; off >>= 1) {
        const K a = k_shfl_down(kmin, off), b = k_shfl_down(kmax, off);
        kmin = a < kmin ? a : kmin;
        kmax = b > kmax ? b : kmax;
    }
    if ((threadIdx.x & 63) == 0) {
        if (kmin != ~(K)0) k_atomic_min(&stats->asp_min, (uint64_t)kmin);
        if (kmax != 0) k_atomic_max(&stats->asp_max, (uint64_t)kmax);
    }
}

constexpr int EXT_TARGET = 16384, EXT_CAP = 4 * EXT_TARGET;
template <typename T>
__global__ __launch_bounds__(256) void nk_ext_build_kernel(const T* __restrict__ ref, const uint8_t* __restrict__ valid,
                                                           const T* __restrict__ aspect, int64_t q0, int64_t n, T thr_lo, T thr_hi,
                                                           T* __restrict__ ref_m, int64_t* __restrict__ ext_idx,
                                                           unsigned long long* __restrict__ ext_cnt ) {
    const int lane = threadIdx.x & 63;
    for (int64_t base = (int64_t)blockIdx.x * blockDim.x; base < n; base += (int64_t)gridDim.x * blockDim.x) {
        const int64_t p = base + threadIdx.x;
        bool lo = false, hi = false;
        if (p < n) {
            const int64_t q = q0 + p;
            const bool v = valid[q] != 0;
            ref_m[q] = v ? ref[q] : (T)NAN;
            const T a = aspect[q];
            lo = v && a < thr_lo;
            hi = v && a > thr_hi;
        }
#pragma unroll
        for (int w = 0; w < 2; ++w) {
            const bool mine = w ? hi : lo;
            const unsigned long long m = __builtin_amdgcn_ballot_w64(mine);
            if (m) {
                const int leader = __ffsll((long long)m) - 1;
                unsigned long long b = 0;
                if (lane == leader) b = atomicAdd(&ext_cnt[w], (unsigned long long)__popcll(m));
                b = ((unsigned long long)(uint32_t)__builtin_amdgcn_readlane((int)(b >> 32), leader) << 32) |
                    (unsigned long long)(uint32_t)__builtin_amdgcn_readlane((int)b, leader);
                const unsigned long long pos = b + (unsigned long long)__popcll(m & ((1ull << lane) - 1ull));
                if (mine && pos < (unsigned long long)EXT_CAP) ext_idx[(int64_t)w * EXT_CAP + (int64_t)pos] = q0 + p;
// ... 266 lines not shown
    }
    st.sync_and_flush_at(0, out_v, out_b, &ctr[1], cap, &ctr[2]);
    for (int off = 32; off > 0; off >>= 1) { s1 += __shfl_down(s1, off); s2 += __shfl_down(s2, off); }
    if (lane == 0) { atomicAdd(&sums[0], s1); atomicAdd(&sums[1], s2); }
    for (int k = threadIdx.x; k < nb; k += blockDim.x) {
        unsigned long long above = 0, below = 0, inside = 0;
        for (int q = 0; q < copies; ++q) {
            above += c[q * cs + k]; below += c[q * cs + nb + k]; inside += c[q * cs + 2 * nb + k];
        }
        if (above + below + inside) atomicAdd(reinterpret_cast<unsigned long long*>(&counters[k]), above + below + inside);
        if (below) atomicAdd(reinterpret_cast<unsigned long long*>(&counters[nb + k]), below);
        if (inside) atomicAdd(reinterpret_cast<unsigned long long*>(&counters[2 * nb + k]), inside);
    }
}

template <typename T>
int NkYSource<T>::launch_lean(xdemhip_ctx* ctx, int64_t n, int nb, const typename KeyT<T>::type* d_klo, const typename KeyT<T>::type* d_khi,
                              uint64_t* d_cnt, T* c_vals, uint16_t* c_bins, unsigned long long* d_flags, int64_t c_cap) const {
    typedef typename KeyT<T>::type K;
    if (!bcache || n <= 0) return XDEMHIP_OK;
    int copies = (28 * 1024) / (nb * 12);
    copies = copies < 1 ? 1 : (copies > 32 ? 32 : copies);
    const size_t lds = (size_t)SEL_STAGE_CAP * (sizeof(T) + 2) + 16 + (size_t)nb * 2 * sizeof(K) + (size_t)((3 * nb) | 1) * 4 * (size_t)copies;
    int rc = set_big_lds(ctx, nk_bins_lean_kernel<T>, lds);
    if (rc) return rc;
    hipLaunchKernelGGL((nk_bins_lean_kernel<T>), dim3(grid_for(ctx, n, HIST_THREADS * NKB_TILE, 2)), dim3(HIST_THREADS), lds, ctx->stream, dh,
                       slope_tan, bcache, rec, vshift_p, n, nb, copies, d_klo, d_khi, d_cnt, c_vals, c_bins, d_flags, c_cap, sums);
    XD_HIP_CHECK(ctx, hipGetLastError());
    return XDEMHIP_OK;
}


}

#include "nk_onepass.h"


using namespace xd;

struct xdemhip_nk_plan {
    xdemhip_ctx* ctx = nullptr;
    int dtype = XDEMHIP_F32;
    int64_t H = 0, W = 0;
    int64_t roff = 0, nbuf = 0;
    int64_t row0 = 0, row1 = 0;
    void *ref = nullptr, *tba = nullptr;
    uint8_t* inlier = nullptr;
    uint8_t* sub_inlier = nullptr;
    uint8_t* inlier_user = nullptr;
    bool subsampled = false;
    bool own_inputs = false;
    void *slope_tan = nullptr, *aspect = nullptr, *dh = nullptr, *y = nullptr;
    uint8_t* valid = nullptr;
    uint16_t* bins = nullptr;
    nk_bin_t* bcache = nullptr;
    bool bcache_force = true;
    void* ref_m = nullptr;
    int64_t* ext_idx = nullptr;
    unsigned long long* ext_cnt = nullptr;
    bool ext_ok = false;
    uint64_t* fz = nullptr;
    size_t fz_bytes = 0;
    void* cd_vals = nullptr;
    int64_t cd_cap = 0;
    void* c_st = nullptr;
    double* wg_sums = nullptr;
    size_t wg_sums_cap = 0;
    unsigned char* fz_pack = nullptr;
    size_t fz_pack_bytes = 0;
    std::vector<unsigned char> fz_host;
    int64_t n_onepass = 0, n_plain = 0;
    int fz_narrow = 0;
    double fz_unit_min = 0.25;
    double fz_worst = 0.0;
    double fz_off2 = 0.0;
    int64_t fz_offn = 0;
    bool pr_have = false;
    int pr_nb = 0;
    double pr_sx = 0, pr_sy = 0, pr_rx = 0, pr_ry = 0;
    double pr_v = 0, pr_wd = 0;
    double pr_st = 0;
    std::vector<double> pr_med, pr_w, pr_mid;
    std::vector<unsigned char> pr_ok;
    double pr_err = 1e30, pr_err_d = 1e30;
    double pr_dpx = 1e30;
    int pr_cooldown = 0;
    int64_t n_predicted = 0, n_predicted_d = 0, n_predict_miss = 0;
    uint64_t *mr_a = nullptr, *mr_b = nullptr, *mr_small = nullptr;
    size_t mr_a_words = 0, mr_b_words = 0;
    int64_t mr_key[8] = {-1, -1, -1, -1, -1, -1, -1, -1};
    bool mr_can = false;
    int64_t mr_nglob = 0;
    void* scratch = nullptr;
    size_t scratch_bytes = 0;
    int max_bins = 0;
    long long n_valid0 = 0;
    xd::SelWorkspace ws;
    uint64_t* badbits = nullptr;
    int64_t bad_wpr = 0;
    int bin_stat = XDEMHIP_BINSTAT_MEDIAN;
    int nan_rule = 0;
    int custom_decimal = 0;
    std::vector<double> custom_edges;
};

namespace {

constexpr size_t OFF_INFO = 12288;

dim3 grid2d(const xdemhip_ctx* ctx, int64_t W, int64_t rows) {
    const int64_t gx = (W + 255) / 256;
    int64_t gy = ((int64_t)ctx->num_cu * 16 + gx - 1) / gx;
    gy = gy < 1 ? 1 : (gy > rows ? (rows > 0 ? rows : 1) : gy);
    return dim3((unsigned)gx, (unsigned)gy);
}

template <typename T> void make_edges(double smin, double smax, int nb, std::vector<T>& e) {
    e.resize(nb + 1);
    make_edges_into<T>(smin, smax, nb, e.data());
}

NkGeom geom_of(const xdemhip_nk_plan* P, double dr, double dc) {
    NkGeom g;
    g.H = P->H; g.W = P->W; g.roff = P->roff; g.dr = dr; g.dc = dc; g.rule = P->nan_rule;
    return g;
}

template <typename T> int nk_aux_typed(xdemhip_nk_plan* P) {
    xdemhip_ctx* ctx = P->ctx;
    const int64_t rows = P->row1 - P->row0;
    unsigned long long* d_cnt = reinterpret_cast<unsigned long long*>(static_cast<unsigned char*>(P->scratch) + OFF_STATS);
    XD_HIP_CHECK(ctx, hipMemsetAsync(d_cnt, 0, 8, ctx->stream));
    if (rows > 0) {
        hipLaunchKernelGGL((nk_aux_kernel<T>), grid2d(ctx, P->W, rows), dim3(256), 0, ctx->stream,
                           static_cast<const T*>(P->ref), static_cast<const T*>(P->tba), P->inlier, geom_of(P, 0.0, 0.0),
                           static_cast<T*>(P->slope_tan), static_cast<T*>(P->aspect), P->valid, d_cnt, P->row0, P->row1);
        XD_HIP_CHECK(ctx, hipGetLastError());
    }
    int rc = xd_allreduce_device(ctx, d_cnt, 1, XDEMHIP_RED_SUM_U64);
    if (rc) return rc;
    unsigned long long c = 0;
    { const int rc_ = xd_d2h(ctx, &c, d_cnt, 8); if (rc_) return rc_; }
    { const int rc_ = xd_sync(ctx); if (rc_) return rc_; }
    P->n_valid0 = (long long)c;
    P->ext_ok = false;
    const bool mr = ctx->allreduce != nullptr;
    if (mr && !(ctx->nk_fused_dist != 0 && ctx->world >= 1 && ctx->world <= MR_WORLD_MAX)) return XDEMHIP_OK;
    if (P->n_valid0 >= 8 * (long long)EXT_TARGET) {
        const bool local_ok = P->ref_m != nullptr && rows > 0;
        unsigned long long ec[2] = {0, 0};
        if (local_ok) {
            const double frac = (double)EXT_TARGET / (double)P->n_valid0;
            const T thr_lo = (T)(6.283185307179586 * frac), thr_hi = (T)(6.283185307179586 * (1.0 - frac));
            const int64_t q0 = (P->row0 - P->roff) * P->W, nown = rows * P->W;
            XD_HIP_CHECK(ctx, hipMemsetAsync(P->ext_cnt, 0, 32, ctx->stream));
            hipLaunchKernelGGL((nk_ext_build_kernel<T>), dim3(grid_for(ctx, nown, 256, 16)), dim3(256), 0, ctx->stream, static_cast<const T*>(P->ref),
                               P->valid, static_cast<const T*>(P->aspect), q0, nown, thr_lo, thr_hi, static_cast<T*>(P->ref_m), P->ext_idx, P->ext_cnt);
            XD_HIP_CHECK(ctx, hipGetLastError());
            { const int rc_ = xd_d2h(ctx, ec, P->ext_cnt, 16); if (rc_) return rc_; }
            { const int rc_ = xd_sync(ctx); if (rc_) return rc_; }
        }
        const bool over = ec[0] > (unsigned long long)EXT_CAP || ec[1] > (unsigned long long)EXT_CAP;
        if (mr) {
            uint64_t v[3] = {ec[0], ec[1], (uint64_t)((!local_ok || over) ? 1 : 0)};
            const int rc_ = xd_allreduce_host(ctx, v, 3, XDEMHIP_RED_SUM_U64);
            if (rc_) return rc_;
// ... 32 lines not shown
        if ((threadIdx.x & 63) == 0) atomicAdd(&blk[k], v);
    }
    __syncthreads();
    if (threadIdx.x < 10) atomicAdd(&sums[threadIdx.x], blk[threadIdx.x]);
}

template <typename T>
int nk_stage_a(xdemhip_nk_plan* P, const NkGeom& g, int64_t q0, int64_t n, int nb) {
    typedef typename KeyT<T>::type K;
    xdemhip_ctx* ctx = P->ctx;
    unsigned char* base = static_cast<unsigned char*>(P->scratch);
    DhStats* d_stats = reinterpret_cast<DhStats*>(base + OFF_STATS);
    T* d_edges = reinterpret_cast<T*>(base);
    DhStats hs0;
    hipLaunchKernelGGL(nk_stats_init_kernel, dim3(1), dim3(64), 0, ctx->stream, d_stats);
    XD_HIP_CHECK(ctx, hipGetLastError());
    int rc = XDEMHIP_OK;
    {
        if (n > 0) {
            hipLaunchKernelGGL((nk_dh_kernel<T>), grid2d(ctx, P->W, P->row1 - P->row0), dim3(256), 0, ctx->stream,
                               static_cast<const T*>(P->ref), static_cast<const T*>(P->tba), P->valid, static_cast<const T*>(P->aspect),
                               g, static_cast<T*>(P->dh), d_stats, P->row0, P->row1);
            XD_HIP_CHECK(ctx, hipGetLastError());
        }
        rc = xd_allreduce_device(ctx, &d_stats->asp_min, 1, XDEMHIP_RED_MIN_U64);
        if (rc) return rc;
        rc = xd_allreduce_device(ctx, &d_stats->asp_max, 1, XDEMHIP_RED_MAX_U64);
        if (rc) return rc;
        std::vector<SelResult<K>> g0;
        rc = run_select<T>(ctx, static_cast<const T*>(P->dh) + q0, nullptr, n, 1, base, g0, &P->ws);
        if (rc) return rc;
        { const int rc_ = xd_d2h(ctx, &hs0, d_stats, sizeof hs0); if (rc_) return rc_; }
        { const int rc_ = xd_sync(ctx); if (rc_) return rc_; }
        unsigned char info[32] = {0};
        const T vs_t = (T)median_from<T>(g0[0]);
        const uint64_t total = g0[0].st.count, flags = 0;
        const double vs = g0[0].st.count ? (double)vs_t : (double)NAN;
        memcpy(info, &vs_t, sizeof(T));
        memcpy(info + 8, &total, 8);
        memcpy(info + 16, &flags, 8);
        memcpy(info + 24, &vs, 8);
        std::vector<T> edges;
        make_edges<T>((double)val_of((K)hs0.asp_min), (double)val_of((K)hs0.asp_max), nb, edges);
        XD_HIP_CHECK(ctx, hipMemcpyAsync(base + OFF_INFO, info, 32, hipMemcpyHostToDevice, ctx->stream));
        XD_HIP_CHECK(ctx, hipMemcpyAsync(d_edges, edges.data(), sizeof(T) * (nb + 1), hipMemcpyHostToDevice, ctx->stream));
        { const int rc_ = xd_sync(ctx); if (rc_) return rc_; }
    }
    if (!P->custom_edges.empty()) {
        std::vector<T> e(P->custom_edges.size());
        for (size_t k = 0; k < e.size(); ++k) e[k] = (T)P->custom_edges[k];
        XD_HIP_CHECK(ctx, hipMemcpyAsync(d_edges, e.data(), sizeof(T) * e.size(), hipMemcpyHostToDevice, ctx->stream));
        { const int rc_ = xd_sync(ctx); if (rc_) return rc_; }
    }
    return XDEMHIP_OK;
}


int nk_mr_alloc(xdemhip_nk_plan* P, int nb, int world, size_t es) {
    auto mx = [](size_t a, size_t b) { return a > b ? a : b; };
    const size_t wa = mx(mx(4, 3 + 3 * (size_t)nb + 5 * (size_t)world + (size_t)world * (DSEL_BUCKETS / 2)), 2 + 2 * (size_t)nb + (size_t)world * nb * (SEL_RADIX / 2));
    const size_t wb = mx((size_t)world * DSEL_HDR_WORDS + (size_t)DSEL_CAP * es / 8, (size_t)nb * MR_GSEG * es / 8);
    if (!P->mr_small && hipMalloc(reinterpret_cast<void**>(&P->mr_small), (size_t)(11 + BINSEG_CTR_STRIDE) * P->ws.nb_max * 8) != hipSuccess) {
        (void)hipGetLastError();
        P->mr_small = nullptr;
        return XDEMHIP_ENOMEM;
    }
    if (P->mr_a_words < wa) {
        if (P->mr_a) (void)hipFree(P->mr_a);
        P->mr_a = nullptr; P->mr_a_words = 0;
        if (hipMalloc(reinterpret_cast<void**>(&P->mr_a), wa * 8) != hipSuccess) { (void)hipGetLastError(); P->mr_a = nullptr; return XDEMHIP_ENOMEM; }
        P->mr_a_words = wa;
    }
    if (P->mr_b_words < wb) {
        if (P->mr_b) (void)hipFree(P->mr_b);
        P->mr_b = nullptr; P->mr_b_words = 0;
        if (hipMalloc(reinterpret_cast<void**>(&P->mr_b), wb * 8) != hipSuccess) { (void)hipGetLastError(); P->mr_b = nullptr; return XDEMHIP_ENOMEM; }
        P->mr_b_words = wb;
    }
    return XDEMHIP_OK;
}

template <typename T>
int nk_step_onepass(xdemhip_nk_plan* P, const NkGeom& g, int64_t q0, int64_t n, int nb, bool* done, double* vshift, int64_t* n_valid,
                    double* y_mean, double* y_std, double* edges_out, int64_t* counts, double* medians, bool allow_predict = true) {
    typedef typename KeyT<T>::type K;
    *done = false;
    xdemhip_ctx* ctx = P->ctx;
    SelWorkspace* ws = &P->ws;
    const int64_t rows = P->row1 - P->row0;
    const int64_t n_slots = ((((n + SEL_LINE - 1) >> SEL_LINE_LOG2) + 63) >> 6) << SEL_LINE_LOG2;
    const bool mr = ctx->allreduce != nullptr;
    const int world = ctx->world, rank = ctx->rank;
    bool cannot = !ctx->nk_fused || !P->fz || !P->cd_vals || !P->c_st || !P->bcache || !P->ext_ok || (g.rule > 1 && !P->badbits) || rows <= 0 ||
                  P->bin_stat != XDEMHIP_BINSTAT_MEDIAN || !(ctx->selection_mode == 0 || ctx->selection_mode == 3) || !ws->d_small ||
                  (int64_t)P->nbuf * P->W < ws->c_cap ||
                  ws->es != sizeof(T) || nb > ws->nb_max || nb > MAX_BINS_PER_SWEEP || n_slots > ws->s_cap ||
                  (int64_t)(NKZ_CHUNK_MAX + 2) * P->W * (int64_t)sizeof(T) >= ((int64_t)1 << 32);
    int64_t n_all = n;
    if (mr && (world < 1 || !ctx->nk_fused_dist || !ctx->nk_fused)) return XDEMHIP_OK;
    if (mr) {
        const int64_t key[8] = {nb, P->row0, P->row1, (int64_t)P->ext_ok, (int64_t)P->bin_stat, (int64_t)ctx->selection_mode,
                                (int64_t)(ctx->nk_fused * 4 + ctx->nk_fused_dist * 2), (int64_t)world * 64 + rank};
        if (memcmp(key, P->mr_key, sizeof key) != 0) {
            cannot = cannot || !ctx->nk_fused_dist || world < 1 || world > MR_WORLD_MAX || rank < 0 || rank >= world ||
                     (int64_t)P->nbuf * P->W < ws->c_cap;
            if (!cannot && nk_mr_alloc(P, nb, world, sizeof(T)) != XDEMHIP_OK) cannot = true;
            uint64_t v[2] = {(uint64_t)n, (uint64_t)(cannot ? 1 : 0)};
            const int rc_ = xd_allreduce_host(ctx, v, 2, XDEMHIP_RED_SUM_U64);
            if (rc_) return rc_;
            P->mr_nglob = (int64_t)v[0];
            P->mr_can = v[1] == 0;
            memcpy(P->mr_key, key, sizeof key);
        }
        if (!P->mr_can) return XDEMHIP_OK;
        n_all = P->mr_nglob;
    } else if (cannot) {
        return XDEMHIP_OK;
    }
    if (n_all < SEL_BRACKET_MIN_N || (ctx->selection_mode == 0 && n_all < SEL_BRACKET_MIN_PER_BIN * nb)) return XDEMHIP_OK;
    unsigned char* scratch = static_cast<unsigned char*>(P->scratch);
    T* d_edges = reinterpret_cast<T*>(scratch);
    DhStats* d_stats = reinterpret_cast<DhStats*>(scratch + OFF_STATS);
    BinCacheRec* d_rec = reinterpret_cast<BinCacheRec*>(scratch + OFF_INFO + 64);
    const SelState<K>* d_st = reinterpret_cast<const SelState<K>*>(scratch + OFF_STATE);
    const int nbm = ws->nb_max;
    uint64_t* fz = P->fz;
    unsigned long long* ctr = reinterpret_cast<unsigned long long*>(fz);
    uint32_t* rbs_d = reinterpret_cast<uint32_t*>(fz + 8);
    uint32_t* rbs_y = reinterpret_cast<uint32_t*>(fz + 9);
    uint64_t* cnt_d = fz + 10;
    K* klo_d = reinterpret_cast<K*>(fz + 14);
    K* khi_d = reinterpret_cast<K*>(fz + 15);
    T* d_vhat = reinterpret_cast<T*>(fz + 16);
    T* d_delta = reinterpret_cast<T*>(fz + 17);
    double* d_sums = reinterpret_cast<double*>(fz + 18);
    K* klo_y = reinterpret_cast<K*>(fz + 24);
    K* khi_y = reinterpret_cast<K*>(fz + 24 + nbm);
    uint64_t* cls_y = fz + 24 + 3 * nbm;
    uint64_t* res_y = fz + 24 + 6 * nbm;
    uint64_t* cnt_y = fz + 24 + 8 * nbm;
    const bool custom = !P->custom_edges.empty();
    const int last_decimal = custom ? P->custom_decimal : NK_AUTO_EDGES;
    if (custom) {
        std::vector<T> e(P->custom_edges.size());
        for (size_t k = 0; k < e.size(); ++k) e[k] = (T)P->custom_edges[k];
        XD_HIP_CHECK(ctx, hipMemcpyAsync(d_edges, e.data(), sizeof(T) * e.size(), hipMemcpyHostToDevice, ctx->stream));
        { const int rc_ = xd_sync(ctx); if (rc_) return rc_; }
    }
    const T* ref_m = static_cast<const T*>(P->ref_m);
    const T* tba = static_cast<const T*>(P->tba);
    const T* st_all = static_cast<const T*>(P->slope_tan);
    static_assert(MAX_BINS_PER_SWEEP <= NK_BINCACHE_MAX_BINS, "the one-pass step's bins fit the byte-wide cache");
    hipLaunchKernelGGL(nk_step_init_kernel, dim3(1), dim3(1024), 0, ctx->stream, d_stats, fz, (int64_t)(P->fz_bytes / 8), P->ext_cnt + 2);
    hipLaunchKernelGGL((nk_ext_eval_kernel<T>), dim3(EXT_CAP / 256, 2), dim3(256), 0, ctx->stream, ref_m, tba, static_cast<const T*>(P->aspect), g,
                       P->ext_idx, P->ext_cnt, d_stats, P->ext_cnt + 2);
    int rc = XDEMHIP_OK;
    uint64_t* ext_slots = reinterpret_cast<uint64_t*>(scratch + off_hist(2)) + 2 * SEL_RADIX;
    if (mr) hipLaunchKernelGGL(nk_mr_ext_pack_kernel, dim3(1), dim3(64), 0, ctx->stream, d_stats, P->ext_cnt + 2, rank, world, ext_slots);
    auto edges_and_bins = [&]() -> int {
        hipLaunchKernelGGL((nk_fz_prep_kernel<T>), dim3(1), dim3(64), 0, ctx->stream, d_stats, P->ext_cnt + 2, nb, (int)custom, d_edges, d_rec,
                           (int)P->bcache_force, ctr);
        hipLaunchKernelGGL((nk_bin_fill_kernel<T>), dim3(grid_for(ctx, n, 256, 16)), dim3(256), sizeof(T) * (nb + 1), ctx->stream,
                           static_cast<const T*>(P->aspect) + q0, n, d_edges, nb, last_decimal, d_rec, P->bcache + q0);
        hipLaunchKernelGGL((nk_bin_cache_commit_kernel<T>), dim3(1), dim3(64), 0, ctx->stream, d_edges, nb, d_rec);
        XD_HIP_CHECK(ctx, hipGetLastError());
        P->bcache_force = false;
        return XDEMHIP_OK;
    };
    if (!mr) { rc = edges_and_bins(); if (rc) return rc; }
    const double dE = g.dc - P->pr_sx, dN = -(g.dr - P->pr_sy);
    const double dpx = sqrt(dE * dE + dN * dN);
    const bool pr_scaled = P->pr_dpx > 0 && P->pr_dpx < 1e29;
    const double pr_expect = pr_scaled ? fmax(0.02, P->pr_err * (dpx / P->pr_dpx)) : 1e30;
    const double pr_expect_d = pr_scaled ? fmax(0.02, P->pr_err_d * (dpx / P->pr_dpx)) : 1e30;
    bool predict = allow_predict && ctx->nk_predict != 0 && P->pr_have && P->pr_nb == nb && nb <= NK_PREDICT_MAX_BINS && P->pr_cooldown == 0 &&
                   pr_expect <= 0.20 && pr_expect_d <= 0.20 && dpx <= 0.05 && P->pr_wd > 0;
    const bool predict_d = !predict && allow_predict && ctx->nk_predict != 0 && P->pr_have && P->pr_nb == nb && P->pr_cooldown == 0 &&
                           pr_expect_d <= 0.35 && dpx <= 0.6 && P->pr_wd > 0;
    if (P->pr_cooldown > 0 && allow_predict) --P->pr_cooldown;
    double pr_h = 1.0;
    T* s_v = static_cast<T*>(ws->s_vals);
    bool fused = false;
    constexpr int BR_PASSES = 3;
    const K low_mask = (K)(((K)1 << (8 * (KeyT<T>::passes - BR_PASSES))) - 1);
    const int narrow = P->fz_narrow;
    if (predict) {
        pr_h = fmin(1.0, fmax(0.25, 2.0 * pr_expect + 0.15));
        NkPredicted<T> pr;
        const double hd = fmin(1.0, fmax(0.25, 2.0 * pr_expect_d + 0.15)) * P->pr_wd;
        pr.dlo = (T)(P->pr_v - hd);
        pr.dhi = (T)(P->pr_v + hd);
        for (int b = 0; b < nb; ++b) {
            if (!P->pr_ok[b]) { pr.lo[b] = (T)1; pr.hi[b] = (T)0; continue; }
            const double c = P->pr_med[b] - (dE * sin(P->pr_mid[b]) + dN * cos(P->pr_mid[b]));
            const double h = pr_h * P->pr_w[b] + 0.05 * dpx;
            pr.lo[b] = (T)(c - h);
            pr.hi[b] = (T)(c + h);
        }
        if (mr) {
            rc = xd_allreduce_device(ctx, ext_slots, 4 * (int64_t)world, XDEMHIP_RED_SUM_U64);
            if (rc) return rc;
            hipLaunchKernelGGL(nk_mr_ext_unpack_kernel, dim3(1), dim3(64), 0, ctx->stream, ext_slots, world, d_stats, P->ext_cnt + 2);
            rc = edges_and_bins();
            if (rc) return rc;
        }
        hipLaunchKernelGGL((nk_predict_kernel<T>), dim3(1), dim3(64), 0, ctx->stream, pr, nb, klo_d, khi_d, rbs_d, d_vhat, d_delta, klo_y, khi_y, rbs_y, ctr);
        XD_HIP_CHECK(ctx, hipGetLastError());
    } else {
    if (!predict_d) {
        hipLaunchKernelGGL((nk_sample_dh_kernel<T>), dim3(grid_for(ctx, n_slots, 256, 8)), dim3(256), 0, ctx->stream, ref_m, tba, g, q0, n,
                           1.0 / (double)P->W, n_slots, s_v, select_reset_plan<K>(scratch, 1, SEL_BRACKET_DUAL));
        XD_HIP_CHECK(ctx, hipGetLastError());
    }
    if (predict_d) {
        NkPredicted<T> pr;
        const double hd = fmin(1.0, fmax(0.25, 2.0 * pr_expect_d + 0.15)) * P->pr_wd;
        pr.dlo = (T)(P->pr_v - hd);
        pr.dhi = (T)(P->pr_v + hd);
        if (mr) {
            rc = xd_allreduce_device(ctx, ext_slots, 4 * (int64_t)world, XDEMHIP_RED_SUM_U64);
            if (rc) return rc;
        }
        hipLaunchKernelGGL((nk_predict_kernel<T>), dim3(1), dim3(64), 0, ctx->stream, pr, 0, klo_d, khi_d, rbs_d, d_vhat, d_delta, klo_y, khi_y, rbs_y, ctr);
        XD_HIP_CHECK(ctx, hipGetLastError());
    } else {
    rc = select_enqueue<T>(ctx, s_v, nullptr, n_slots, n_slots, nullptr, 1, scratch, SEL_BRACKET_DUAL, nullptr, BR_PASSES, false, nullptr, nullptr,
                           false, narrow, klo_d, khi_d, rbs_d, low_mask, &fused, true, mr ? 0 : -1, mr ? 4 * (int64_t)world : 0);
    if (rc) return rc;
    if (!fused) hipLaunchKernelGGL((bracket_finish_kernel<K>), dim3(1), dim3(64), 0, ctx->stream, d_st, 1, 0, low_mask, klo_d, khi_d, rbs_d);
    }
    if (mr) {
        hipLaunchKernelGGL(nk_mr_ext_unpack_kernel, dim3(1), dim3(64), 0, ctx->stream, ext_slots, world, d_stats, P->ext_cnt + 2);
        rc = edges_and_bins();
        if (rc) return rc;
    }
    if (predict_d)
        hipLaunchKernelGGL((nk_sample_dy_kernel<T>), dim3(grid_for(ctx, n_slots, 256, 8)), dim3(256), 0, ctx->stream, ref_m, tba, g, q0, n,
                           1.0 / (double)P->W, n_slots, s_v, ws->s_bins, st_all + q0, P->bcache + q0, klo_d, khi_d, d_vhat, d_delta, ctr,
                           select_reset_plan<K>(scratch, nb, SEL_BRACKET_DUAL));
    else
    hipLaunchKernelGGL((nk_sample_y_kernel<T>), dim3(grid_for(ctx, n_slots, 256, 8)), dim3(256), 0, ctx->stream, s_v, ws->s_bins, st_all + q0,
                       P->bcache + q0, n, n_slots, d_vhat, klo_d, khi_d, d_vhat, d_delta, ctr, select_reset_plan<K>(scratch, nb, SEL_BRACKET_DUAL));
    XD_HIP_CHECK(ctx, hipGetLastError());
    rc = select_enqueue<T>(ctx, s_v, nb == 1 ? nullptr : ws->s_bins, n_slots, n_slots, nullptr, nb, scratch, SEL_BRACKET_DUAL, nullptr, BR_PASSES,
                           false, nullptr, nullptr, false, narrow, klo_y, khi_y, rbs_y, low_mask, &fused, true);
    if (rc) return rc;
    if (!fused) hipLaunchKernelGGL((bracket_finish_kernel<K>), dim3(1), dim3(64), 0, ctx->stream, d_st, nb, 0, low_mask, klo_y, khi_y, rbs_y);
    XD_HIP_CHECK(ctx, hipGetLastError());
    }
    int n_wg = 0;
    {
        dim3 grid = grid2d(ctx, P->W, rows);
        if ((rows + grid.y - 1) / grid.y > NKZ_CHUNK_MAX) grid.y = (unsigned)((rows + NKZ_CHUNK_MAX - 1) / NKZ_CHUNK_MAX);
        n_wg = (int)(grid.x * grid.y);
        if ((size_t)n_wg > P->wg_sums_cap) {
            if (P->wg_sums) (void)hipFree(P->wg_sums);
            P->wg_sums = nullptr; P->wg_sums_cap = 0;
            if (hipMalloc(reinterpret_cast<void**>(&P->wg_sums), (size_t)n_wg * 5 * sizeof(double)) != hipSuccess) {
                (void)hipGetLastError();
                return xd_fail(ctx, XDEMHIP_ENOMEM, "hipMalloc(per-workgroup sums of the one-pass step) failed");
            }
            P->wg_sums_cap = (size_t)n_wg;
        }
        int copies = (4608) / (nb * 12);
        copies = copies < 1 ? 1 : (copies > 16 ? 16 : copies);
        const size_t lds = (size_t)nb * sizeof(FzPair<T>) + (size_t)((3 * nb) | 1) * 4 * (size_t)copies + 64 * 4;
        T* cy_d = static_cast<T*>(ws->c_vals);
#define XD_NK_FZ(RULE)                                                                                                               \
    hipLaunchKernelGGL((nk_fused_kernel<T, RULE>), grid, dim3(256), lds, ctx->stream, ref_m, tba, st_all, P->bcache, g, P->row0, P->row1,  \
                       P->nbuf, nb, copies, klo_d, khi_d, d_vhat, d_delta, klo_y, khi_y, cnt_d, cls_y, static_cast<T*>(P->cd_vals),   \
                       P->cd_cap, cy_d, static_cast<T*>(P->c_st), ws->c_bins, ws->c_cap, ctr, P->wg_sums, P->badbits, P->bad_wpr)
        if (g.rule == 0) XD_NK_FZ(0);
        else if (g.rule == 1) XD_NK_FZ(1);
        else XD_NK_FZ(2);
#undef XD_NK_FZ
        XD_HIP_CHECK(ctx, hipGetLastError());
    }
    uint64_t* cls_loc = mr ? P->mr_small : nullptr;
    uint64_t* cls_f = mr ? cls_loc + 3 * nbm : nullptr;
    uint64_t* res_f = mr ? cls_f + 3 * nbm : nullptr;
    uint64_t* cnt_true = mr ? res_f + 2 * nbm : nullptr;
    unsigned long long* segf_ctr = mr ? reinterpret_cast<unsigned long long*>(cnt_true + 3 * nbm) : nullptr;
    int dsel_grid = grid_for(ctx, n / 32 + 1, HIST_THREADS * 8, 1);
    dsel_grid = dsel_grid > 64 ? 64 : dsel_grid;
    const int64_t words7 = 3 + 3 * (int64_t)nb + 5 * (int64_t)world;
    uint32_t* mr_rows = mr ? reinterpret_cast<uint32_t*>(P->mr_a + words7) : nullptr;
    if (mr) {
        XD_HIP_CHECK(ctx, hipMemsetAsync(mr_rows, 0, (size_t)world * DSEL_BUCKETS * 4, ctx->stream));
        hipLaunchKernelGGL(nk_mr_counts_pack_kernel, dim3(1), dim3(256), 0, ctx->stream, cnt_d, cls_y, P->wg_sums, n_wg, nb, rank, world, P->mr_a, cls_loc);
        hipLaunchKernelGGL((nk_dhsel_hist_kernel<T>), dim3(dsel_grid), dim3(HIST_THREADS), 0, ctx->stream, static_cast<const T*>(P->cd_vals), P->cd_cap, ctr + 1,
                           klo_d, khi_d, mr_rows + (size_t)rank * DSEL_BUCKETS);
        XD_HIP_CHECK(ctx, hipGetLastError());
        rc = xd_allreduce_device(ctx, P->mr_a, words7 + (int64_t)world * (DSEL_BUCKETS / 2), XDEMHIP_RED_SUM_U64);
        if (rc) return rc;
        hipLaunchKernelGGL(nk_mr_counts_unpack_kernel, dim3(1), dim3(256), 0, ctx->stream, P->mr_a, nb, world, cnt_d, cls_y, d_sums);
        XD_HIP_CHECK(ctx, hipGetLastError());
    }
    {
        uint32_t* dsel = reinterpret_cast<uint32_t*>(fz + 24 + (11 + BINSEG_CTR_STRIDE) * nbm);
        K* dsel_keys = reinterpret_cast<K*>(reinterpret_cast<unsigned char*>(fz) + P->fz_bytes);
        const int grid = dsel_grid;
        const size_t lds = (size_t)DSEL_CAP * sizeof(K) + (size_t)(BINSEL_COPIES * (SEL_RADIX + 1) + 1) * 4 + (size_t)(SEL_RADIX + 4 + 16 + 2) * 8;
        rc = set_big_lds(ctx, nk_dhsel_final_kernel<T>, lds);
        if (rc) return rc;
        if (mr) {
            hipLaunchKernelGGL((nk_mr_dh_base_kernel<T>), dim3(1), dim3(HIST_THREADS), 0, ctx->stream, mr_rows, world, rank, cnt_d, klo_d, khi_d, dsel, ctr);
            uint64_t* slots = P->mr_b;
            K* gk = reinterpret_cast<K*>(P->mr_b + (size_t)world * DSEL_HDR_WORDS);
            const int64_t words8 = (int64_t)world * DSEL_HDR_WORDS + (int64_t)DSEL_CAP * (int64_t)sizeof(K) / 8;
            XD_HIP_CHECK(ctx, hipMemsetAsync(P->mr_b, 0, (size_t)words8 * 8, ctx->stream));
            hipLaunchKernelGGL((nk_dhsel_gather_kernel<T>), dim3(grid), dim3(HIST_THREADS), 0, ctx->stream, static_cast<const T*>(P->cd_vals), P->cd_cap, ctr + 1,
                               cnt_d, klo_d, khi_d, dsel, gk, ctr, 0);
            hipLaunchKernelGGL(nk_mr_dh_hdr_pack_kernel, dim3(1), dim3(64), 0, ctx->stream, dsel, rank, slots);
            XD_HIP_CHECK(ctx, hipGetLastError());
            rc = xd_allreduce_device(ctx, P->mr_b, words8, XDEMHIP_RED_SUM_U64);
            if (rc) return rc;
            hipLaunchKernelGGL(nk_mr_dh_hdr_merge_kernel, dim3(1), dim3(64), 0, ctx->stream, slots, world, dsel);
            hipLaunchKernelGGL((nk_dhsel_final_kernel<T>), dim3(1), dim3(HIST_THREADS), lds, ctx->stream, P->cd_cap, ctr + 1, cnt_d, klo_d, khi_d, dsel, gk,
                               ctr, scratch + OFF_INFO, 0);
        } else {
        hipLaunchKernelGGL((nk_dhsel_hist_kernel<T>), dim3(grid), dim3(HIST_THREADS), 0, ctx->stream, static_cast<const T*>(P->cd_vals), P->cd_cap, ctr + 1,
                           klo_d, khi_d, dsel + 2 * DSEL_HDR_WORDS, P->wg_sums, n_wg, d_sums);
        hipLaunchKernelGGL((nk_dhsel_gather_kernel<T>), dim3(grid), dim3(HIST_THREADS), 0, ctx->stream, static_cast<const T*>(P->cd_vals), P->cd_cap, ctr + 1,
                           cnt_d, klo_d, khi_d, dsel, dsel_keys, ctr);
        hipLaunchKernelGGL((nk_dhsel_final_kernel<T>), dim3(1), dim3(HIST_THREADS), lds, ctx->stream, P->cd_cap, ctr + 1, cnt_d, klo_d, khi_d, dsel, dsel_keys,
                           ctr, scratch + OFF_INFO);
        }
        XD_HIP_CHECK(ctx, hipGetLastError());
    }
    {
        unsigned long long* seg_ctr = reinterpret_cast<unsigned long long*>(fz + 24 + 11 * nbm);
        const size_t lds = (size_t)nb * (3 * 8 + 2 * sizeof(K) + 3 * 4) + 16;
        hipLaunchKernelGGL((nk_resolve_scatter_kernel<T>), dim3(grid_for(ctx, n / 16 + 1, HIST_THREADS * BINSEG_U, 2)), dim3(HIST_THREADS), lds, ctx->stream,
                           static_cast<const T*>(ws->c_vals), static_cast<const T*>(P->c_st), ws->c_bins, ws->c_cap, ctr + 5,
                           reinterpret_cast<const T*>(scratch + OFF_INFO), nb, klo_y, khi_y, cls_y, res_y, seg_ctr, static_cast<T*>(P->y),
                           (int64_t)P->nbuf * P->W, ctr, cls_loc);
        const size_t lds2 = (size_t)BINSEL_KEY_BYTES + (size_t)(BINSEL_COPIES * (SEL_RADIX + 1) + 1) * 4 + (size_t)(SEL_RADIX + 8) * 8;
        rc = set_big_lds(ctx, nk_bin_select_kernel<T>, lds2);
        if (rc) return rc;
        if (mr) {
            const int64_t words9 = 2 + 2 * (int64_t)nb + (int64_t)world * nb * (SEL_RADIX / 2);
            XD_HIP_CHECK(ctx, hipMemsetAsync(P->mr_a, 0, (size_t)words9 * 8, ctx->stream));
            hipLaunchKernelGGL((nk_mr_bin_hist_kernel<T>), dim3(nb), dim3(HIST_THREADS), 0, ctx->stream, static_cast<const T*>(P->y), cls_loc, res_y, seg_ctr, nb, klo_y,
                               khi_y, rank, world, P->mr_a, ctr);
            XD_HIP_CHECK(ctx, hipGetLastError());
            rc = xd_allreduce_device(ctx, P->mr_a, words9, XDEMHIP_RED_SUM_U64);
            if (rc) return rc;
            const int64_t words10 = (int64_t)nb * MR_GSEG * (int64_t)sizeof(T) / 8;
            XD_HIP_CHECK(ctx, hipMemsetAsync(P->mr_b, 0, (size_t)words10 * 8, ctx->stream));
            hipLaunchKernelGGL((nk_mr_bin_gather_kernel<T>), dim3(nb), dim3(HIST_THREADS), 0, ctx->stream, static_cast<const T*>(P->y), cls_loc, cls_y, P->mr_a, seg_ctr, nb,
                               klo_y, khi_y, rank, world, reinterpret_cast<T*>(P->mr_b), cls_f, res_f, segf_ctr, cnt_true, ctr);
            XD_HIP_CHECK(ctx, hipGetLastError());
            rc = xd_allreduce_device(ctx, P->mr_b, words10, XDEMHIP_RED_SUM_U64);
            if (rc) return rc;
            hipLaunchKernelGGL((nk_bin_select_kernel<T>), dim3(nb), dim3(HIST_THREADS), lds2, ctx->stream, reinterpret_cast<const T*>(P->mr_b), cls_f, res_f, segf_ctr,
                               nb, klo_y, khi_y, rbs_y, reinterpret_cast<SelState<K>*>(scratch + OFF_STATE), reinterpret_cast<uint64_t*>(scratch + off_succ(nb)),
                               cnt_y, ctr, (int64_t)MR_GSEG);
        } else {
        hipLaunchKernelGGL((nk_bin_select_kernel<T>), dim3(nb), dim3(HIST_THREADS), lds2, ctx->stream, static_cast<const T*>(P->y), cls_y, res_y, seg_ctr, nb,
                           klo_y, khi_y, rbs_y, reinterpret_cast<SelState<K>*>(scratch + OFF_STATE), reinterpret_cast<uint64_t*>(scratch + off_succ(nb)),
                           cnt_y, ctr);
        }
        XD_HIP_CHECK(ctx, hipGetLastError());
    }
    std::vector<uint64_t> cnt(3 * (size_t)nb);
    std::vector<K> klo(nb);
    std::vector<T> edges(nb + 1);
    unsigned long long h_ctr[16];
    uint64_t h_rbs = 0;
    unsigned char info[32];
    double sums[5];
    T h_vhat = (T)0;
    std::vector<SelState<K>> h_st(nb);
    std::vector<uint64_t> h_succ(nb);
    std::vector<uint64_t> cnt_t(mr ? 3 * (size_t)nb : 0);
    std::vector<K> khi(nb);
    K h_kd[2] = {0, 0};
    const int n_pk = mr ? 14 : 13;
    {
        FzPack pk;
        void* dsts[14] = {cnt.data(), klo.data(), h_ctr, &h_rbs, info, sums, &h_vhat, edges.data(), h_st.data(), h_succ.data(), khi.data(), &h_kd[0], &h_kd[1],
                          cnt_t.data()};
        const void* srcs[14] = {cnt_y, klo_y, ctr, rbs_y, scratch + OFF_INFO, d_sums, d_vhat, d_edges, scratch + OFF_STATE, scratch + off_succ(nb), khi_y, klo_d,
                                khi_d, cnt_true};
        const size_t sizes[14] = {8 * 3 * (size_t)nb, sizeof(K) * nb, 128, 8, 32, 40, sizeof(T), sizeof(T) * (nb + 1), sizeof(SelState<K>) * nb, 8 * (size_t)nb,
                                  sizeof(K) * nb, sizeof(K), sizeof(K), 8 * 3 * (size_t)nb};
        uint32_t off = 0;
        pk.n = n_pk;
        for (int k = 0; k < n_pk; ++k) {
            pk.src[k] = static_cast<const unsigned char*>(srcs[k]);
            pk.bytes[k] = (uint32_t)sizes[k];
            pk.off[k] = off;
            off += (uint32_t)((sizes[k] + 15) & ~(size_t)15);
        }
        if (off > P->fz_pack_bytes) return xd_fail(ctx, XDEMHIP_EINVAL, "one-pass step: result block too small");
        P->fz_host.resize(off);
        unsigned char* pin = xd_pin_claim(ctx, P->fz_host.data(), off);
        pk.dst = pin ? pin : P->fz_pack;
        hipLaunchKernelGGL(nk_fz_pack_kernel, dim3(1), dim3(256), 0, ctx->stream, pk);
        XD_HIP_CHECK(ctx, hipGetLastError());
        if (!pin) { const int rc_ = xd_d2h(ctx, P->fz_host.data(), P->fz_pack, off); if (rc_) return rc_; }
        { const int rc_ = xd_sync(ctx); if (rc_) return rc_; }
        for (int k = 0; k < n_pk; ++k) memcpy(dsts[k], P->fz_host.data() + pk.off[k], sizes[k]);
    }
    std::vector<SelResult<K>> hs(nb);
    for (int k = 0; k < nb; ++k) { hs[k].st = h_st[k]; hs[k].succ = h_succ[k]; }
    if ((h_ctr[2] != 0 || h_ctr[3] != 0) && getenv("XDEMHIP_DEBUG"))
        fprintf(stderr, "[xdemhip] one-pass step falls through: overflow flag %llu, miss flag %llu, dh candidates %llu, bin candidates %llu\n", h_ctr[2], h_ctr[3],
                h_ctr[1], h_ctr[5]);
    if ((h_ctr[2] != 0 || h_ctr[3] != 0) && (predict || predict_d)) {
        ++P->n_predict_miss;
        P->pr_cooldown = 1;
        P->pr_err = P->pr_err_d = 1e30;
        return nk_step_onepass<T>(P, g, q0, n, nb, done, vshift, n_valid, y_mean, y_std, edges_out, counts, medians, false);
    }
    if (h_ctr[2] != 0 || h_ctr[3] != 0) {
        if (h_ctr[6] != 0) P->ext_ok = false;
        if (narrow > 0) {
            P->fz_unit_min = fmin(1.0, 1.5 * sel_narrow_unit((uint32_t)narrow));
            P->fz_narrow = 0;
        }
        P->pr_have = false;
        return XDEMHIP_OK;
    }
    if (!predict) {
        auto off_of = [&](uint64_t tot, uint64_t lt, uint64_t in) {
            return fabs(((double)(tot - 1) * 0.5 - (double)lt) - 0.5 * (double)in) / (0.5 * (double)in);
        };
        const double unit = sel_narrow_unit((uint32_t)narrow);
        double worst = 0.0;
        auto take = [&](uint64_t tot, uint64_t lt, uint64_t in) {
            if (tot < 4096 || in < 64 || in >= tot) return;
            const double o = off_of(tot, lt, in) * unit;
            worst = o > worst ? o : worst;
            P->fz_off2 += o * o;
            P->fz_offn += 1;
        };
        if (!predict_d) take(h_ctr[10], h_ctr[11], h_ctr[12]);
        for (int b = 0; b < nb; ++b) {
            if (mr) take(cnt_t[b], cnt_t[nb + b], cnt_t[2 * nb + b]);
            else take(cnt[b], cnt[nb + b], cnt[2 * nb + b]);
        }
        P->fz_worst = worst > P->fz_worst ? worst : P->fz_worst;
        int next = 0;
        if (P->fz_offn >= 24) {
            const double sigma = sqrt(P->fz_off2 / (double)P->fz_offn);
            static const int qs[] = {4, 5, 6, 7, 8, 10, 12};
            for (int q : qs) {
                const double u = (double)q / 16.0;
                if (4.8 * sigma <= u && 1.5 * P->fz_worst <= u && u >= P->fz_unit_min) { next = q == 8 ? 1 : (q == 4 ? 2 : (int)SEL_NARROW_16THS + q); break; }
            }
        }
        if (ctx->nk_narrow >= 0) next = ctx->nk_narrow;
        if (getenv("XDEMHIP_DEBUG"))
            fprintf(stderr, "[xdemhip] one-pass step: brackets x %.4f, offsets rms %.3f worst %.3f of the full half width (%lld brackets) -> next x %.4f\n", unit,
                    P->fz_offn ? sqrt(P->fz_off2 / (double)P->fz_offn) : 0.0, P->fz_worst, (long long)P->fz_offn, sel_narrow_unit((uint32_t)next));
        P->fz_narrow = next;
    }
    uint64_t total;
    double vs;
    memcpy(&total, info + 8, 8);
    memcpy(&vs, info + 24, 8);
    *n_valid = (int64_t)total;
    if (total == 0) return xd_fail(ctx, XDEMHIP_EINVAL, "The subsample contains no more valid values.");
    *vshift = vs;
    const int rbs = (int)(uint32_t)h_rbs;
    for (int b = 0; b < nb; ++b) {
        const uint64_t tot = cnt[b], lt = cnt[nb + b];
        if (tot == 0) { hs[b].st.count = 0; counts[b] = 0; medians[b] = NAN; continue; }
        hs[b].st.count = tot;
        hs[b].st.n_le += lt;
        hs[b].st.prefix = (K)((K)(hs[b].st.prefix >> rbs) + klo[b]);
        if (hs[b].succ != ~(uint64_t)0) hs[b].succ = (uint64_t)(K)((K)((K)hs[b].succ >> rbs) + klo[b]);
        counts[b] = (int64_t)tot;
        medians[b] = median_from<T>(hs[b]);
    }
    for (int k = 0; k <= nb; ++k) edges_out[k] = (double)edges[k];
    const double dlt = (double)h_vhat - vs, cntd = (double)total;
    const double s1 = sums[0] + dlt * sums[2];
    const double s2 = sums[1] + 2.0 * dlt * sums[3] + dlt * dlt * sums[4];
    const double mean = s1 / cntd, var = s2 / cntd - mean * mean;
    *y_mean = mean;
    *y_std = var > 0 ? sqrt(var) : 0.0;
    {
        std::vector<double> mid(nb);
        for (int b = 0; b < nb; ++b) mid[b] = 0.5 * ((double)edges[b] + (double)edges[b + 1]);
        if (P->pr_have && P->pr_nb == nb) {
            double worst = 0.0;
            for (int b = 0; b < nb; ++b) {
                if (!P->pr_ok[b] || counts[b] == 0 || !(P->pr_w[b] > 0)) continue;
                const double e = fabs(medians[b] - (P->pr_med[b] - (dE * sin(P->pr_mid[b]) + dN * cos(P->pr_mid[b])))) / P->pr_w[b];
                worst = e > worst ? e : worst;
            }
            P->pr_err = worst;
            P->pr_err_d = P->pr_wd > 0 ? fabs(vs - P->pr_v) / P->pr_wd : 1e30;
            P->pr_dpx = fmax(dpx, 1e-5);
            if (getenv("XDEMHIP_DEBUG"))
                fprintf(stderr, "[xdemhip] one-pass step (%s, half widths x %.2f): shift change %.2e px, centres off by %.3f (bins) / %.3f (dh) sampled half widths\n",
                        predict ? "PREDICTED brackets" : (predict_d ? "sampled brackets, PREDICTED bracket of the median of dh" : "sampled brackets"), pr_h, dpx, P->pr_err, P->pr_err_d);
        } else {
            P->pr_err = P->pr_err_d = 1e30;
            P->pr_dpx = 1e30;
        }
        if (!predict || (int)P->pr_w.size() != nb) {
            const double norm = narrow >= (int)SEL_NARROW_16THS ? 0.5 / sel_narrow_unit((uint32_t)narrow) : 1.0;
            P->pr_w.assign(nb, 0.0);
            for (int b = 0; b < nb; ++b)
                if (counts[b] > 0 && khi[b] >= klo[b]) P->pr_w[b] = norm * 0.5 * ((double)val_of(khi[b]) - (double)val_of(klo[b]));
            if (!predict_d) P->pr_wd = h_kd[1] >= h_kd[0] ? norm * 0.5 * ((double)val_of(h_kd[1]) - (double)val_of(h_kd[0])) : 0.0;
        }
        P->pr_med.assign(medians, medians + nb);
        P->pr_mid = mid;
        P->pr_ok.assign(nb, 0);
        for (int b = 0; b < nb; ++b) P->pr_ok[b] = (counts[b] > 0 && P->pr_w[b] > 0 && std::isfinite(P->pr_w[b]) && std::isfinite(medians[b])) ? 1 : 0;
        P->pr_v = vs;
        P->pr_st = sums[2] > 0 ? cntd / sums[2] : 0.0;
        P->pr_sx = g.dc;
        P->pr_sy = g.dr;
        P->pr_nb = nb;
        P->pr_have = true;
        if (predict) ++P->n_predicted;
        if (predict_d) ++P->n_predicted_d;
    }
    *done = true;
    return XDEMHIP_OK;
}

template <typename T>
int nk_step_typed(xdemhip_nk_plan* P, double shift_x, double shift_y, double res_x, double res_y, int nb, double* vshift,
                  int64_t* n_valid, double* y_mean, double* y_std, double* edges_out, int64_t* counts, double* medians,
                  double* fit_sums ) {
    typedef typename KeyT<T>::type K;
    xdemhip_ctx* ctx = P->ctx;
    const int64_t q0 = (P->row0 - P->roff) * P->W;
    const int64_t n = (P->row1 - P->row0) * P->W;
    unsigned char* base = static_cast<unsigned char*>(P->scratch);
    double* d_sums = reinterpret_cast<double*>(base + OFF_SUMS);
    const T* dh = static_cast<const T*>(P->dh) + q0;
    const T* st = static_cast<const T*>(P->slope_tan) + q0;
    const T* asp = static_cast<const T*>(P->aspect) + q0;
    T* y = static_cast<T*>(P->y) + q0;
    uint16_t* bins = P->bins + q0;
    T* d_edges = reinterpret_cast<T*>(base);
    T* d_vshift = reinterpret_cast<T*>(base + OFF_INFO);
    if (!P->custom_edges.empty()) nb = (int)P->custom_edges.size() - 1;

    const double dr = -shift_y / res_y, dc = shift_x / res_x;
    const NkGeom g = geom_of(P, dr, dc);
    {
        const int64_t need = (int64_t)floor(fabs(dr)) + (P->nan_rule >= 2 ? 2 : 1);
        const bool top_ok = P->row0 == 0 || P->row0 - P->roff >= need;
        const bool bottom_ok = P->row1 == P->H || P->roff + P->nbuf - P->row1 >= need;
        if (!top_ok || !bottom_ok)
            return xd_fail(ctx, XDEMHIP_EINVAL, "halo too small: the vertical shift moves the bilinear taps outside this rank's row block + halo");
    }
    if (!fit_sums) {
        bool done = false;
        const int rc1 = nk_step_onepass<T>(P, g, q0, n, nb, &done, vshift, n_valid, y_mean, y_std, edges_out, counts, medians);
        if (rc1) return rc1;
        if (done) { ++P->n_onepass; return XDEMHIP_OK; }
    }
    int rc = nk_stage_a<T>(P, g, q0, n, nb);
    if (rc) return rc;
    std::vector<SelResult<K>> hs;
    bool bins_done = false, bins_passed = false, tail_queued = false, committed = false;
    unsigned char info[32];
    std::vector<T> edges_early(nb + 1);
    double sums_early[2] = {0.0, 0.0};
    double* d_bsum = reinterpret_cast<double*>(base + off_hist(nb));
    unsigned long long* d_bcnt = reinterpret_cast<unsigned long long*>(d_bsum + nb);
    double* d_fit = reinterpret_cast<double*>(base + off_hist(1));
    NkYSource<T> src{dh, st, asp, d_vshift, d_edges, d_sums, nullptr, 0.0, (T)0,
                     P->custom_edges.empty() ? NK_AUTO_EDGES : P->custom_decimal};
    BinCacheRec* d_rec = reinterpret_cast<BinCacheRec*>(base + OFF_INFO + 64);
    if (!fit_sums && P->bcache && nb <= NK_BINCACHE_MAX_BINS) {
        src.bcache = P->bcache + q0;
        src.rec = d_rec;
        hipLaunchKernelGGL((nk_bin_cache_check_kernel<T>), dim3(1), dim3(64), 0, ctx->stream, d_edges, nb, d_rec, (int)P->bcache_force);
        XD_HIP_CHECK(ctx, hipGetLastError());
    }
    XD_HIP_CHECK(ctx, hipMemsetAsync(d_sums, 0, 16, ctx->stream));
    if (fit_sums) {
        XD_HIP_CHECK(ctx, hipMemsetAsync(d_fit, 0, 80, ctx->stream));
        if (n > 0) {
            hipLaunchKernelGGL((nk_fit_sums_kernel<T>), dim3(grid_for(ctx, n, 256, 16)), dim3(256), 0, ctx->stream, dh, st, asp, n, d_vshift,
                               d_fit);
            XD_HIP_CHECK(ctx, hipGetLastError());
        }
        rc = xd_allreduce_device(ctx, d_fit, 10, XDEMHIP_RED_SUM_F64);
        if (rc) return rc;
    } else if (P->bin_stat == XDEMHIP_BINSTAT_MEAN) {
        if (nb > 3072) return xd_fail(ctx, XDEMHIP_EINVAL, "n_bins too large for the mean statistic");
        rc = run_bin_sums<T, NkYSource<T>>(ctx, src, n, nb, d_bsum, d_bcnt);
        if (rc) return rc;
        if (src.bcache) {
            hipLaunchKernelGGL((nk_bin_cache_commit_kernel<T>), dim3(1), dim3(64), 0, ctx->stream, d_edges, nb, d_rec);
            P->bcache_force = false;
        }
    } else {
        const std::function<int()> tail = [&]() -> int {
            if (ctx->allreduce) return XDEMHIP_OK;
            if (src.bcache) {
                hipLaunchKernelGGL((nk_bin_cache_commit_kernel<T>), dim3(1), dim3(64), 0, ctx->stream, d_edges, nb, d_rec);
                XD_HIP_CHECK(ctx, hipGetLastError());
                P->bcache_force = false;
// ... 118 lines not shown
    if (total == 0) return xd_fail(ctx, XDEMHIP_EINVAL, "The subsample contains no more valid values.");
    *vshift = vs;
    XD_HIP_CHECK(ctx, hipMemsetAsync(d_sums, 0, 16, ctx->stream));
    hipLaunchKernelGGL((nk_y_kernel<T>), dim3(grid_for(ctx, n, 256, 16)), dim3(256), sizeof(T) * (nb + 1), ctx->stream, static_cast<const T*>(P->dh),
                       static_cast<const T*>(P->slope_tan), static_cast<const T*>(P->aspect), n, (T)vs, d_edges, nb, static_cast<T*>(P->y), P->bins,
                       d_sums, P->custom_edges.empty() ? NK_AUTO_EDGES : P->custom_decimal);
    XD_HIP_CHECK(ctx, hipGetLastError());
    P->bcache_force = true;
    std::vector<T> edges(nb + 1);
    double sums[2];
    { const int rc_ = xd_d2h(ctx, edges.data(), d_edges, sizeof(T) * (nb + 1)); if (rc_) return rc_; }
    { const int rc_ = xd_d2h(ctx, sums, d_sums, 16); if (rc_) return rc_; }
    const hipMemcpyKind kind = memspace == XDEMHIP_DEVICE ? hipMemcpyDeviceToDevice : hipMemcpyDeviceToHost;
    XD_HIP_CHECK(ctx, hipMemcpyAsync(y_out, P->y, (size_t)n * sizeof(T), kind, ctx->stream));
    XD_HIP_CHECK(ctx, hipMemcpyAsync(bins_out, P->bins, (size_t)n * 2, kind, ctx->stream));
    { const int rc_ = xd_sync(ctx); if (rc_) return rc_; }
    const double cnt = (double)total, mean = sums[0] / cnt, var = sums[1] / cnt - mean * mean;
    *y_mean = mean;
    *y_std = var > 0 ? sqrt(var) : 0.0;
    for (int k = 0; k <= nb; ++k) edges_out[k] = (double)edges[k];
    return XDEMHIP_OK;
}

int nk_create_impl(xdemhip_ctx* ctx, const void* ref, const void* tba, const uint8_t* inlier, int dtype, int64_t H, int64_t W,
                   int64_t roff, int64_t nbuf, int64_t row0, int64_t row1, int memspace, bool global_count,
                   xdemhip_nk_plan** out_plan, int64_t* n_valid) {
    if (!ctx) return XDEMHIP_EINVAL;
    if (!ref || !tba || !out_plan) return xd_fail(ctx, XDEMHIP_EINVAL, "null argument");
    if (H < 2 || W < 2) return xd_fail(ctx, XDEMHIP_EINVAL, "Shape of array too small to calculate a numerical gradient, at least 2 elements are required.");
    if (dtype != XDEMHIP_F32 && dtype != XDEMHIP_F64) return xd_fail(ctx, XDEMHIP_EINVAL, "dtype must be float32 or float64");
    XD_HIP_CHECK(ctx, hipSetDevice(ctx->device));
    const size_t es = dtype == XDEMHIP_F32 ? 4 : 8;
    const size_t n = (size_t)nbuf * (size_t)W;
    xdemhip_nk_plan* P = new xdemhip_nk_plan();
    P->ctx = ctx; P->dtype = dtype; P->H = H; P->W = W; P->roff = roff; P->nbuf = nbuf; P->row0 = row0; P->row1 = row1;
    P->nan_rule = ctx->nk_nan_rule;
    auto fail = [&](int code, const char* msg) { xdemhip_nk_destroy(P); return xd_fail(ctx, code, msg); };
    if (memspace == XDEMHIP_HOST) {
        P->own_inputs = true;
        if (hipMalloc(&P->ref, n * es) != hipSuccess || hipMalloc(&P->tba, n * es) != hipSuccess) return fail(XDEMHIP_ENOMEM, "hipMalloc failed");
        if (hipMemcpyAsync(P->ref, ref, n * es, hipMemcpyHostToDevice, ctx->stream) != hipSuccess ||
            hipMemcpyAsync(P->tba, tba, n * es, hipMemcpyHostToDevice, ctx->stream) != hipSuccess) return fail(XDEMHIP_EHIP, "H2D copy failed");
        if (inlier) {
            if (hipMalloc(reinterpret_cast<void**>(&P->inlier), n) != hipSuccess) return fail(XDEMHIP_ENOMEM, "hipMalloc failed");
            if (hipMemcpyAsync(P->inlier, inlier, n, hipMemcpyHostToDevice, ctx->stream) != hipSuccess) return fail(XDEMHIP_EHIP, "H2D copy failed");
        }
    } else {
        P->ref = const_cast<void*>(ref);
        P->tba = const_cast<void*>(tba);
        P->inlier = const_cast<uint8_t*>(inlier);
    }
    P->max_bins = 1024;
    P->scratch_bytes = scratch_size(P->max_bins);
    if (hipMalloc(&P->slope_tan, n * es) != hipSuccess || hipMalloc(&P->aspect, n * es) != hipSuccess ||
        hipMalloc(&P->dh, n * es) != hipSuccess || hipMalloc(&P->y, n * es) != hipSuccess ||
        hipMalloc(reinterpret_cast<void**>(&P->valid), n) != hipSuccess ||
        hipMalloc(reinterpret_cast<void**>(&P->bins), n * 2) != hipSuccess || hipMalloc(reinterpret_cast<void**>(&P->bcache), n * sizeof(nk_bin_t)) != hipSuccess || hipMalloc(&P->scratch, P->scratch_bytes) != hipSuccess)
        return fail(XDEMHIP_ENOMEM, "hipMalloc failed");
    if ((int64_t)n >= SEL_BRACKET_MIN_N && sel_ws_create(ctx, (int64_t)n, es, MAX_BINS_PER_SWEEP, P->ws) != XDEMHIP_OK)
        return fail(XDEMHIP_ENOMEM, "hipMalloc failed");
    if ((int64_t)n >= SEL_BRACKET_MIN_N && ctx->nk_fused != 0) {
        if (hipMalloc(&P->ref_m, n * es) != hipSuccess || hipMalloc(reinterpret_cast<void**>(&P->ext_idx), (size_t)2 * EXT_CAP * 8) != hipSuccess ||
            hipMalloc(reinterpret_cast<void**>(&P->ext_cnt), 32) != hipSuccess) {
            (void)hipGetLastError();
            if (P->ref_m) (void)hipFree(P->ref_m);
            if (P->ext_idx) (void)hipFree(P->ext_idx);
            if (P->ext_cnt) (void)hipFree(P->ext_cnt);
            P->ref_m = nullptr; P->ext_idx = nullptr; P->ext_cnt = nullptr;
        }
    }
    if (P->ref_m && P->ws.d_small && ctx->nk_fused != 0) {
        P->fz_bytes = (size_t)(24 + (11 + BINSEG_CTR_STRIDE) * P->ws.nb_max + DSEL_HDR_WORDS + DSEL_BUCKETS / 2) * 8;
        P->cd_cap = (int64_t)n / 8 + 4096;
        P->fz_pack_bytes = (size_t)P->ws.nb_max * (8 * 3 + 8 + 16 + 64 + 8 + 8 * 3 + 16) + 1024;
        if (hipMalloc(reinterpret_cast<void**>(&P->fz), P->fz_bytes + (size_t)DSEL_CAP * 8) != hipSuccess || hipMalloc(&P->cd_vals, (size_t)P->cd_cap * es) != hipSuccess ||
            hipMalloc(&P->c_st, (size_t)P->ws.c_cap * es) != hipSuccess || hipMalloc(reinterpret_cast<void**>(&P->fz_pack), P->fz_pack_bytes) != hipSuccess) {
            (void)hipGetLastError();
            if (P->fz) (void)hipFree(P->fz);
            if (P->cd_vals) (void)hipFree(P->cd_vals);
            if (P->c_st) (void)hipFree(P->c_st);
            if (P->fz_pack) (void)hipFree(P->fz_pack);
            P->fz = nullptr; P->cd_vals = nullptr; P->c_st = nullptr; P->fz_pack = nullptr;
        }
    }
    if (P->nan_rule >= 2 && (int64_t)n >= SEL_BRACKET_MIN_N) {
        P->bad_wpr = (W + 63) / 64 + 2;
        if (hipMalloc(reinterpret_cast<void**>(&P->badbits), (size_t)P->bad_wpr * (size_t)nbuf * 8) != hipSuccess) {
            (void)hipGetLastError();
            P->badbits = nullptr;
        } else {
            const dim3 bgrid((unsigned)((P->bad_wpr - 2 + 3) / 4), (unsigned)(nbuf < 4096 ? nbuf : 4096));
            if (dtype == XDEMHIP_F32)
                hipLaunchKernelGGL((nk_badbits_kernel<float>), bgrid, dim3(256), 0, ctx->stream, static_cast<const float*>(P->tba), H, W, roff, nbuf, P->nan_rule, P->bad_wpr, P->badbits);
            else
                hipLaunchKernelGGL((nk_badbits_kernel<double>), bgrid, dim3(256), 0, ctx->stream, static_cast<const double*>(P->tba), H, W, roff, nbuf, P->nan_rule, P->bad_wpr, P->badbits);
            if (hipGetLastError() != hipSuccess) return fail(XDEMHIP_EHIP, "nk_badbits_kernel launch failed");
        }
    }
    const xdemhip_allreduce_fn hook = ctx->allreduce;
    if (!global_count) ctx->allreduce = nullptr;
    int rc = dtype == XDEMHIP_F32 ? nk_aux_typed<float>(P) : nk_aux_typed<double>(P);
    ctx->allreduce = hook;
    if (rc != XDEMHIP_OK) { xdemhip_nk_destroy(P); return rc; }
    if (n_valid) *n_valid = P->n_valid0;
    *out_plan = P;
    return XDEMHIP_OK;
}

}

extern "C" {

void xdemhip_nk_destroy(xdemhip_nk_plan* P) {
    if (!P) return;
    (void)hipSetDevice(P->ctx->device);
    uint8_t* inl_created = P->subsampled ? P->inlier_user : P->inlier;
    if (P->own_inputs) { (void)hipFree(P->ref); (void)hipFree(P->tba); if (inl_created) (void)hipFree(inl_created); }
    if (P->sub_inlier) (void)hipFree(P->sub_inlier);
    void* bufs[] = {P->slope_tan, P->aspect, P->dh, P->y, P->valid, P->bins, P->bcache, P->scratch, P->ref_m, P->ext_idx, P->ext_cnt,
                    P->fz, P->cd_vals, P->c_st, P->fz_pack, P->badbits, P->mr_a, P->mr_b, P->mr_small, P->wg_sums};
    for (void* b : bufs)
        if (b) (void)hipFree(b);
    xd::sel_ws_free(P->ws);
    delete P;
}

int xdemhip_nk_create(xdemhip_ctx* ctx, const void* ref, const void* tba, const uint8_t* inlier, int dtype, int64_t H, int64_t W,
                      int memspace, xdemhip_nk_plan** out_plan, int64_t* n_valid) {
    XdFetchScope fetch_scope_(ctx);
    return nk_create_impl(ctx, ref, tba, inlier, dtype, H, W, 0, H, 0, H, memspace, false, out_plan, n_valid);
}

int xdemhip_nk_create_block(xdemhip_ctx* ctx, const void* ref_block, const void* tba_block, const uint8_t* inlier_block, int dtype,
                            int64_t H, int64_t W, int64_t row_begin, int64_t row_end, int64_t halo_top, int64_t halo_bottom,
                            int memspace, xdemhip_nk_plan** out_plan, int64_t* n_valid) {
    XdFetchScope fetch_scope_(ctx);
    if (!ctx) return XDEMHIP_EINVAL;
    if (row_begin < 0 || row_end < row_begin || row_end > H || halo_top < 0 || halo_bottom < 0 || halo_top > row_begin ||
        row_end + halo_bottom > H)
        return xd_fail(ctx, XDEMHIP_EINVAL, "bad row block");
    if ((row_begin > 0 && halo_top < 1) || (row_end < H && halo_bottom < 1))
        return xd_fail(ctx, XDEMHIP_EINVAL, "a row block inside the raster needs >= 1 halo row towards each neighbour");
    return nk_create_impl(ctx, ref_block, tba_block, inlier_block, dtype, H, W, row_begin - halo_top, (row_end - row_begin) + halo_top + halo_bottom,
                          row_begin, row_end, memspace, true, out_plan, n_valid);
}

int xdemhip_nk_set_rows(xdemhip_nk_plan* P, int64_t row_begin, int64_t row_end, int64_t* n_valid) {
    XdFetchScope fetch_scope_(P ? P->ctx : nullptr);
    if (!P) return XDEMHIP_EINVAL;
    xdemhip_ctx* ctx = P->ctx;
    if (row_begin < P->roff || row_end < row_begin || row_end > P->roff + P->nbuf) return xd_fail(ctx, XDEMHIP_EINVAL, "bad row range");
    XD_HIP_CHECK(ctx, hipSetDevice(ctx->device));
    P->row0 = row_begin;
    P->row1 = row_end;
    P->bcache_force = true;
    P->pr_have = false;
    int rc = P->dtype == XDEMHIP_F32 ? nk_aux_typed<float>(P) : nk_aux_typed<double>(P);
    if (rc) return rc;
    if (n_valid) *n_valid = P->n_valid0;
    return XDEMHIP_OK;
}

int xdemhip_nk_subsample(xdemhip_nk_plan* P, const int64_t* ranks, int64_t k, int memspace, int64_t* n_valid) {
    XdFetchScope fetch_scope_(P ? P->ctx : nullptr);
    if (!P) return XDEMHIP_EINVAL;
    xdemhip_ctx* ctx = P->ctx;
    if (ctx->allreduce || P->row0 != 0 || P->row1 != P->H || P->roff != 0 || P->nbuf != P->H)
        return xd_fail(ctx, XDEMHIP_EINVAL, "xdemhip_nk_subsample: whole-raster plans of one process only (partitioned plans: pass the drawn mask as inlier mask)");
    if (!ranks || k < 1 || k > P->n_valid0) return xd_fail(ctx, XDEMHIP_EINVAL, "xdemhip_nk_subsample: 1 <= k <= the plan's valid pixels");
    XD_HIP_CHECK(ctx, hipSetDevice(ctx->device));
    const int64_t n = P->H * P->W, n_tiles = (n + RANK_TILE - 1) / RANK_TILE;
    if (n_tiles > 0x7FFFFFFF) return xd_fail(ctx, XDEMHIP_EINVAL, "xdemhip_nk_subsample: raster too large");
    if (!P->sub_inlier && hipMalloc(reinterpret_cast<void**>(&P->sub_inlier), (size_t)n) != hipSuccess) {
        (void)hipGetLastError();
        P->sub_inlier = nullptr;
        return xd_fail(ctx, XDEMHIP_ENOMEM, "hipMalloc failed (xdemhip_nk_subsample)");
    }
    RankSelect rs;
    unsigned long long total = 0, bad = 0;
    { const int rc_ = rs.run(ctx, "xdemhip_nk_subsample", ranks, k, memspace, P->n_valid0, P->valid, n, nullptr, &total, &bad); if (rc_) return rc_; }
    if ((long long)total != P->n_valid0) return xd_fail(ctx, XDEMHIP_EINVAL, "xdemhip_nk_subsample: the valid mask changed under the call");
    if (bad != 0) return xd_fail(ctx, XDEMHIP_EINVAL, "xdemhip_nk_subsample: a rank is outside [0, n_valid)");
    hipLaunchKernelGGL((rank_select_kernel<RankOut::Mask>), dim3((unsigned)n_tiles), dim3(256), 0, ctx->stream, P->valid, n, rs.off, rs.mark,
                       (unsigned long long*)nullptr, (int64_t*)nullptr, P->sub_inlier);
    if (hipGetLastError() != hipSuccess) return xd_fail(ctx, XDEMHIP_EHIP, "xdemhip_nk_subsample: kernel launch failed");
    if (!P->subsampled) { P->inlier_user = P->inlier; P->subsampled = true; }
    P->inlier = P->sub_inlier;
    P->bcache_force = true;
    P->pr_have = false;
    P->fz_narrow = 0; P->fz_unit_min = 0.25; P->fz_worst = 0.0; P->fz_off2 = 0.0; P->fz_offn = 0;
    const int rc = P->dtype == XDEMHIP_F32 ? nk_aux_typed<float>(P) : nk_aux_typed<double>(P);
    if (rc) return rc;
    if (n_valid) *n_valid = P->n_valid0;
    return XDEMHIP_OK;
}

int xdemhip_nk_predict_counts(xdemhip_nk_plan* P, int64_t* predicted, int64_t* predicted_dh_only, int64_t* missed) {
    if (!P) return XDEMHIP_EINVAL;
    if (predicted) *predicted = P->n_predicted;
    if (predicted_dh_only) *predicted_dh_only = P->n_predicted_d;
    if (missed) *missed = P->n_predict_miss;
    return XDEMHIP_OK;
}

int xdemhip_nk_route_counts(xdemhip_nk_plan* P, int64_t* onepass, int64_t* plain) {
    if (!P) return XDEMHIP_EINVAL;
    if (onepass) *onepass = P->n_onepass;
    if (plain) *plain = P->n_plain;
    return XDEMHIP_OK;
}

int xdemhip_nk_set_statistic(xdemhip_nk_plan* P, int bin_stat) {
    if (!P) return XDEMHIP_EINVAL;
    if (bin_stat != XDEMHIP_BINSTAT_MEDIAN && bin_stat != XDEMHIP_BINSTAT_MEAN) return xd_fail(P->ctx, XDEMHIP_EINVAL, "bin statistic: 0 median, 1 mean");
    P->bin_stat = bin_stat;
    return XDEMHIP_OK;
}

int xdemhip_nk_get_aux(xdemhip_nk_plan* P, void* slope_tan, void* aspect, uint8_t* valid) {
    if (!P) return XDEMHIP_EINVAL;
    xdemhip_ctx* ctx = P->ctx;
    XD_HIP_CHECK(ctx, hipSetDevice(ctx->device));
    { const int rc_ = xd_sync(ctx); if (rc_) return rc_; }
    const size_t es = P->dtype == XDEMHIP_F32 ? 4 : 8, n = (size_t)P->nbuf * (size_t)P->W;
    if (slope_tan) XD_HIP_CHECK(ctx, hipMemcpy(slope_tan, P->slope_tan, n * es, hipMemcpyDeviceToHost));
    if (aspect) XD_HIP_CHECK(ctx, hipMemcpy(aspect, P->aspect, n * es, hipMemcpyDeviceToHost));
    if (valid) XD_HIP_CHECK(ctx, hipMemcpy(valid, P->valid, n, hipMemcpyDeviceToHost));
    return XDEMHIP_OK;
}

int xdemhip_nk_step(xdemhip_nk_plan* P, double shift_x, double shift_y, double res_x, double res_y, int n_bins, double* vshift,
                    int64_t* n_valid, double* y_mean, double* y_std, double* edges, int64_t* counts, double* medians) {
    XdFetchScope fetch_scope_(P ? P->ctx : nullptr);
    if (!P) return XDEMHIP_EINVAL;
    xdemhip_ctx* ctx = P->ctx;
    if (!vshift || !n_valid || !y_mean || !y_std || !edges || !counts || !medians) return xd_fail(ctx, XDEMHIP_EINVAL, "null output");
    if (n_bins < 1 || n_bins > P->max_bins) return xd_fail(ctx, XDEMHIP_EINVAL, "n_bins out of range (1..1024)");
    if (!P->custom_edges.empty() && n_bins != (int)P->custom_edges.size() - 1)
        return xd_fail(ctx, XDEMHIP_EINVAL, "n_bins must equal the number of explicit bin edges - 1 (xdemhip_nk_set_bin_edges)");
    if (!(res_x > 0) || !(res_y > 0)) return xd_fail(ctx, XDEMHIP_EINVAL, "resolution must be > 0");
    XD_HIP_CHECK(ctx, hipSetDevice(ctx->device));
    XD_HIP_CHECK(ctx, hipEventRecord(ctx->ev_start, ctx->stream));
    int rc = P->dtype == XDEMHIP_F32
                 ? nk_step_typed<float>(P, shift_x, shift_y, res_x, res_y, n_bins, vshift, n_valid, y_mean, y_std, edges, counts, medians, nullptr)
                 : nk_step_typed<double>(P, shift_x, shift_y, res_x, res_y, n_bins, vshift, n_valid, y_mean, y_std, edges, counts, medians, nullptr);
    (void)hipEventRecord(ctx->ev_stop, ctx->stream);
    ctx->timed = (rc == XDEMHIP_OK);
    return rc;
}

int xdemhip_nk_step_fit(xdemhip_nk_plan* P, double shift_x, double shift_y, double res_x, double res_y, double* vshift, int64_t* n_valid,
                        double* y_mean, double* y_std, double* sums) {
    XdFetchScope fetch_scope_(P ? P->ctx : nullptr);
    if (!P) return XDEMHIP_EINVAL;
    xdemhip_ctx* ctx = P->ctx;
    if (!vshift || !n_valid || !y_mean || !y_std || !sums) return xd_fail(ctx, XDEMHIP_EINVAL, "null output");
    if (!(res_x > 0) || !(res_y > 0)) return xd_fail(ctx, XDEMHIP_EINVAL, "resolution must be > 0");
    XD_HIP_CHECK(ctx, hipSetDevice(ctx->device));
    XD_HIP_CHECK(ctx, hipEventRecord(ctx->ev_start, ctx->stream));
    int rc = P->dtype == XDEMHIP_F32
                 ? nk_step_typed<float>(P, shift_x, shift_y, res_x, res_y, 72, vshift, n_valid, y_mean, y_std, nullptr, nullptr, nullptr, sums)
                 : nk_step_typed<double>(P, shift_x, shift_y, res_x, res_y, 72, vshift, n_valid, y_mean, y_std, nullptr, nullptr, nullptr, sums);
    (void)hipEventRecord(ctx->ev_stop, ctx->stream);
    ctx->timed = (rc == XDEMHIP_OK);
    return rc;
}

int xdemhip_nk_step_values(xdemhip_nk_plan* P, double shift_x, double shift_y, double res_x, double res_y, int n_bins, double* vshift,
                           int64_t* n_valid, double* y_mean, double* y_std, double* edges, void* y_out, uint16_t* bins_out, int memspace) {
    XdFetchScope fetch_scope_(P ? P->ctx : nullptr);
    if (!P) return XDEMHIP_EINVAL;
    xdemhip_ctx* ctx = P->ctx;
    if (!vshift || !n_valid || !y_mean || !y_std || !edges || !y_out || !bins_out) return xd_fail(ctx, XDEMHIP_EINVAL, "null output");
    if (!(res_x > 0) || !(res_y > 0)) return xd_fail(ctx, XDEMHIP_EINVAL, "resolution must be > 0");
    if (memspace != XDEMHIP_HOST && memspace != XDEMHIP_DEVICE) return xd_fail(ctx, XDEMHIP_EINVAL, "memspace must be XDEMHIP_HOST or XDEMHIP_DEVICE");
    if (n_bins < 1 || n_bins > P->max_bins) return xd_fail(ctx, XDEMHIP_EINVAL, "n_bins out of range (1..1024)");
    if (!P->custom_edges.empty() && n_bins != (int)P->custom_edges.size() - 1)
        return xd_fail(ctx, XDEMHIP_EINVAL, "n_bins must equal the number of explicit bin edges - 1 (xdemhip_nk_set_bin_edges)");
    XD_HIP_CHECK(ctx, hipSetDevice(ctx->device));
    XD_HIP_CHECK(ctx, hipEventRecord(ctx->ev_start, ctx->stream));
    const int rc = P->dtype == XDEMHIP_F32
                       ? nk_step_values<float>(P, shift_x, shift_y, res_x, res_y, n_bins, vshift, n_valid, y_mean, y_std, edges, y_out, bins_out, memspace)
                       : nk_step_values<double>(P, shift_x, shift_y, res_x, res_y, n_bins, vshift, n_valid, y_mean, y_std, edges, y_out, bins_out, memspace);
    (void)hipEventRecord(ctx->ev_stop, ctx->stream);
// ... 133 lines not shown
```

xdem_amd/csrc/select.h:

```cpp
#pragma once
#include <hip/hip_runtime.h>
#include <math.h>
#include <stdint.h>

namespace xd {

constexpr int SEL_RADIX = 256;

__device__ __forceinline__ uint32_t key_of(float v) {
    const uint32_t b = __float_as_uint(v);
    return b ^ ((b >> 31) ? 0xFFFFFFFFu : 0x80000000u);
}
__device__ __forceinline__ uint64_t key_of(double v) {
    const uint64_t b = (uint64_t)__double_as_longlong(v);
    return b ^ ((b >> 63) ? 0xFFFFFFFFFFFFFFFFull : 0x8000000000000000ull);
}
__host__ __device__ inline float val_of(uint32_t k) {
    const uint32_t b = (k >> 31) ? (k ^ 0x80000000u) : ~k;
    float f;
    __builtin_memcpy(&f, &b, 4);
    return f;
}
__host__ __device__ inline double val_of(uint64_t k) {
    const uint64_t b = (k >> 63) ? (k ^ 0x8000000000000000ull) : ~k;
    double f;
    __builtin_memcpy(&f, &b, 8);
    return f;
}
template <typename T> struct KeyT;
template <> struct KeyT<float> { typedef uint32_t type; static constexpr int passes = 4; };
template <> struct KeyT<double> { typedef uint64_t type; static constexpr int passes = 8; };

template <typename K> struct SelState {
    K prefix;
    uint64_t rank;
    uint64_t count;
    uint64_t n_le;
    uint64_t group;
};

enum { SEL_MEDIAN = 0, SEL_BRACKET_LO = 1, SEL_BRACKET_HI = 2, SEL_GIVEN = 3, SEL_BRACKET_LO_WIDE = 4, SEL_BRACKET_HI_WIDE = 5,
       SEL_BRACKET_DUAL = 6  };

__host__ __device__ inline uint64_t sel_bracket_halfwidth(uint64_t m) {
    return (uint64_t)(3.0 * sqrt(8.0 * (double)m)) + 32;
}
constexpr uint32_t SEL_NARROW_16THS = 16;
__host__ __device__ inline uint64_t sel_narrowed(uint64_t h_full, uint32_t narrow) {
    const uint64_t w = h_full - 32;
    return (narrow < SEL_NARROW_16THS ? (w >> narrow) : ((w * (uint64_t)(narrow - SEL_NARROW_16THS)) >> 4)) + 32;
}
__host__ __device__ inline double sel_narrow_unit(uint32_t narrow) {
    return narrow < SEL_NARROW_16THS ? 1.0 / (double)(1u << narrow) : (double)(narrow - SEL_NARROW_16THS) / 16.0;
}
constexpr uint32_t PAIR_DEFF_WIDE = 4096, PAIR_DEFF_SPREAD = 4;
__host__ __device__ inline uint64_t sel_bracket_halfwidth_wide(uint64_t m, uint32_t deff = PAIR_DEFF_WIDE) {
    return (uint64_t)(3.0 * sqrt((double)deff * (double)m)) + 64;
}

template <typename K, bool DEV = false>
__device__ __forceinline__ void select_advance_body(const int b, const int lane, SelState<K>* st, uint64_t* hist, int nb, int shift, int first, int last,
                                                    int mode, const uint64_t* given, const uint32_t* rb_shift, uint32_t wide_deff, int dual_nb,
                                                    uint64_t* succ, uint32_t* need_succ, uint32_t narrow, SelState<K>* lds_states = nullptr) {
    if (b >= nb) return;
    const bool dual_first = first && mode == SEL_BRACKET_DUAL;
    if (dual_first && b >= dual_nb) return;
    if (!first && rb_shift && shift + 8 <= (int)*rb_shift) {
        if (last && lane == 0 && st[b].count) st[b].n_le += st[b].group;
        return;
    }
    const bool eff_last = last || (rb_shift && shift <= (int)*rb_shift);
    uint64_t* h = hist + (size_t)b * SEL_RADIX;
    unsigned long long c[4], mine = 0;
#pragma unroll
    for (int q = 0; q < 4; ++q) {
        c[q] = DEV ? (unsigned long long)__hip_atomic_load(&h[4 * lane + q], __ATOMIC_RELAXED, __HIP_MEMORY_SCOPE_AGENT) : (unsigned long long)h[4 * lane + q];
        mine += c[q];
        h[4 * lane + q] = 0;
    }
    unsigned long long incl = mine;
#pragma unroll
    for (int off = 1; off < 64; off <<= 1) {
        const unsigned long long t = __shfl_up(incl, off);
        if (lane >= off) incl += t;
    }
    const unsigned long long total = __shfl(incl, 63);
    for (int half = 0; half < (dual_first ? 2 : 1); ++half) {
    const int bs = b + half * dual_nb;
    SelState<K> s = st[bs];
    if (first) {
        s.count = total;
        uint64_t r = total ? (total - 1) / 2 : 0;
        const bool lo_end = mode == SEL_BRACKET_LO || (mode == SEL_BRACKET_DUAL && bs < dual_nb);
        const bool hi_end = mode == SEL_BRACKET_HI || (mode == SEL_BRACKET_DUAL && bs >= dual_nb);
        if (lo_end && total) { const uint64_t h = sel_narrowed(sel_bracket_halfwidth(total), narrow); r = r > h ? r - h : 0; }
        if (hi_end && total) { const uint64_t h = sel_narrowed(sel_bracket_halfwidth(total), narrow); r = (r + h < total) ? r + h : total - 1; }
        if (mode == SEL_BRACKET_LO_WIDE && total) { const uint64_t h = sel_bracket_halfwidth_wide(total, wide_deff); r = r > h ? r - h : 0; }
        if (mode == SEL_BRACKET_HI_WIDE && total) { const uint64_t h = sel_bracket_halfwidth_wide(total, wide_deff); r = (r + h < total) ? r + h : total - 1; }
        if (mode == SEL_GIVEN) {
            r = given[bs];
            if (r == ~(uint64_t)0 || r >= total) { s.count = 0; r = 0; }
        }
        s.rank = r;
        s.prefix = 0;
        s.n_le = 0;
        s.group = total;
    }
    if (s.count) {
        const unsigned long long excl = incl - mine;
        const bool here = (s.rank >= excl) && (s.rank < incl);
        const unsigned long long vote = __ballot(here);
        const int src = vote ? (int)__ffsll((long long)vote) - 1 : 63;
        unsigned long long cum = excl;
        int q = 0;
        if (cum + c[0] <= s.rank) { cum += c[0]; q = 1;
            if (cum + c[1] <= s.rank) { cum += c[1]; q = 2;
                if (cum + c[2] <= s.rank) { cum += c[2]; q = 3; } } }
        const unsigned long long hq = q == 0 ? c[0] : (q == 1 ? c[1] : (q == 2 ? c[2] : c[3]));
        const int dsel = __shfl(4 * lane + q, src);
        const unsigned long long cumsel = __shfl(cum, src);
        const unsigned long long hsel = __shfl(hq, src);
        s.prefix |= (K)dsel << shift;
        s.n_le += cumsel;
        s.rank -= cumsel;
        s.group = hsel;
        if (last) s.n_le += hsel;
        if (eff_last && succ) {
            int cand = 0x7fffffff;
#pragma unroll
            for (int q = 3; q >= 0; --q)
                if (c[q] > 0 && 4 * lane + q > dsel) cand = 4 * lane + q;
            const unsigned long long have = __ballot(cand != 0x7fffffff);
            if (have) {
                const int nxt = __shfl(cand, (int)__ffsll((long long)have) - 1);
                if (lane == 0) succ[bs] = (uint64_t)(K)((s.prefix & ~((K)0xFF << shift)) | ((K)nxt << shift));
            } else if (lane == 0 && need_succ) {
                *need_succ = 1u;
// ... 24 lines not shown
```

Baseline: 123,700 Mpixels/s.

## Derive one-pass nuth-kaab bin brackets from value-bucket histograms of the sample

Result: no change. 123,600 Mpixels/s (-0.1%).

```diff
diff --git a/include/xdemhip.h b/include/xdemhip.h
--- a/include/xdemhip.h
+++ b/include/xdemhip.h
@@ -99,6 +99,7 @@
 int xdemhip_nk_subsample(xdemhip_nk_plan* plan, const int64_t* ranks, int64_t k, int memspace, int64_t* n_valid);
 int xdemhip_nk_route_counts(xdemhip_nk_plan* plan, int64_t* onepass, int64_t* plain);
 int xdemhip_nk_predict_counts(xdemhip_nk_plan* plan, int64_t* predicted, int64_t* predicted_dh_only, int64_t* missed);
+int xdemhip_nk_bracket_counts(xdemhip_nk_plan* plan, int64_t* bucketed, int64_t* fell_back);
 void xdemhip_nk_destroy(xdemhip_nk_plan* plan);
 int xdemhip_binned_median(xdemhip_ctx* ctx, const void* x, const void* y, int dtype, int64_t n, int n_bins, double* edges,
                           int64_t* counts, double* medians);
diff --git a/xdem_amd/_lib.py b/xdem_amd/_lib.py
--- a/xdem_amd/_lib.py
+++ b/xdem_amd/_lib.py
@@ -150,6 +150,7 @@
         L.xdemhip_nk_step_values.argtypes = [ctypes.c_void_p, ctypes.c_double, ctypes.c_double, ctypes.c_double, ctypes.c_double, ctypes.c_int,
                                              c_dp, c_i64p, c_dp, c_dp, c_dp, ctypes.c_void_p, ctypes.c_void_p, ctypes.c_int]
         L.xdemhip_nk_predict_counts.argtypes = [ctypes.c_void_p, c_i64p, c_i64p, c_i64p]
+        L.xdemhip_nk_bracket_counts.argtypes = [ctypes.c_void_p, c_i64p, c_i64p]
         L.xdemhip_nk_subsample.argtypes = [ctypes.c_void_p, ctypes.c_void_p, ctypes.c_int64, ctypes.c_int, c_i64p]
         L.xdemhip_host_count_finite.argtypes = [ctypes.c_void_p, ctypes.c_int, ctypes.c_int64, ctypes.c_int, c_i64p, ctypes.c_void_p]
         c_u64p = ctypes.POINTER(ctypes.c_uint64)
@@ -476,7 +477,7 @@
             self._L.xdemhip_device_free(self.handle, ctypes.c_void_p(p))
 
     TEST_SWITCHES = frozenset(("terrain_stream", "terrain_order", "terrain_ring_wait", "terrain_window_lds", "nk_narrow",
-                               "vario_grid", "vario_runs", "vario_sort", "hypso_seg_lds", "pts_tile_order", "bw_seg_lds"))
+                               "nk_bucket_brackets", "vario_grid", "vario_runs", "vario_sort", "hypso_seg_lds", "pts_tile_order", "bw_seg_lds"))
 
     def set_option(self, name: str, value: int) -> None:
         fn = self._L.xdemhip_set_test_switch if name in self.TEST_SWITCHES else self._L.xdemhip_set_option
diff --git a/xdem_amd/coreg.py b/xdem_amd/coreg.py
--- a/xdem_amd/coreg.py
+++ b/xdem_amd/coreg.py
@@ -172,8 +172,11 @@
         self.ctx.check(self.ctx._L.xdemhip_nk_route_counts(self.handle, ctypes.byref(a), ctypes.byref(c)))
         p, d, m = ctypes.c_int64(), ctypes.c_int64(), ctypes.c_int64()
         self.ctx.check(self.ctx._L.xdemhip_nk_predict_counts(self.handle, ctypes.byref(p), ctypes.byref(d), ctypes.byref(m)))
+        k, f = ctypes.c_int64(), ctypes.c_int64()
+        self.ctx.check(self.ctx._L.xdemhip_nk_bracket_counts(self.handle, ctypes.byref(k), ctypes.byref(f)))
         return {"onepass": int(a.value), "plain": int(c.value), "predicted": int(p.value),
-                "predicted_dh_only": int(d.value), "predict_missed": int(m.value)}
+                "predicted_dh_only": int(d.value), "predict_missed": int(m.value),
+                "bucket_brackets": int(k.value), "bucket_fallbacks": int(f.value)}
 
     def set_bin_edges(self, edges) -> None:
         dp = ctypes.POINTER(ctypes.c_double)
diff --git a/xdem_amd/csrc/capi.hip b/xdem_amd/csrc/capi.hip
--- a/xdem_amd/csrc/capi.hip
+++ b/xdem_amd/csrc/capi.hip
@@ -291,6 +291,7 @@
     {"terrain_ring_wait", 0, 1, &xdemhip_ctx::terrain_ring_wait, "terrain_ring_wait: 0 counted wait, 1 vmcnt(0)"},
     {"terrain_window_lds", 0, 1, &xdemhip_ctx::terrain_window_lds, "terrain_window_lds: 0 or 1"},
     {"nk_narrow", -1, 2, &xdemhip_ctx::nk_narrow, "nk_narrow: -1 (adaptive), 0, 1 or 2"},
+    {"nk_bucket_brackets", 0, 2, &xdemhip_ctx::nk_bucket_brackets, "nk_bucket_brackets: 0, 1 or 2"},
     {"vario_grid", 0, 1, &xdemhip_ctx::vario_grid, "vario_grid: 0 or 1"},
     {"vario_runs", 0, 1, &xdemhip_ctx::vario_runs, "vario_runs: 0 or 1"},
     {"vario_sort", 0, 1, &xdemhip_ctx::vario_sort, "vario_sort: 0 or 1"},
diff --git a/xdem_amd/csrc/common.h b/xdem_amd/csrc/common.h
--- a/xdem_amd/csrc/common.h
+++ b/xdem_amd/csrc/common.h
@@ -36,6 +36,7 @@
     int vario_runs = 1;
     int vario_sort = 1;
     int nk_predict = 1;
+    int nk_bucket_brackets = 1;
     int nk_fused = 1;
     int terrain_stream = 1;
     int terrain_order = 0;
diff --git a/xdem_amd/csrc/nk_buckets.h b/xdem_amd/csrc/nk_buckets.h
--- /dev/null
+++ b/xdem_amd/csrc/nk_buckets.h
@@ -0,0 +1,69 @@
+#pragma once
+#include <math.h>
+#include <stdint.h>
+
+#include "sel_rule.h"
+
+namespace xd {
+
+constexpr int NKB_B = 256;
+constexpr int NKB_PER_W = 32;
+constexpr int NKB_ROW = NKB_B + 2;
+
+struct NkbGrid { double lo0, w, inv_w; };
+
+XD_RULE_HD NkbGrid nkb_grid(double centre, double half_width, int per_w = NKB_PER_W) {
+    NkbGrid g;
+    g.w = half_width / (double)per_w;
+    g.lo0 = centre - (double)(NKB_B / 2) * g.w;
+    g.inv_w = 1.0 / g.w;
+    const double reach = fabs(g.lo0) + (double)NKB_B * g.w;
+    if (!(g.w > 0.0) || !(reach < 1e300) || !(g.inv_w < 1e300) || !(reach * 0x1p-48 <= g.w * 0x1p-4)) { g.lo0 = 0.0; g.w = 0.0; g.inv_w = 0.0; }
+    return g;
+}
+
+XD_RULE_HD int nkb_bucket(double x, const NkbGrid& g) {
+    if (!(g.inv_w > 0.0)) return 0;
+    const double t = (x - g.lo0) * g.inv_w;
+    if (!(t >= 0.0)) return 0;
+    if (!(t < (double)NKB_B)) return NKB_B + 1;
+    return (int)t + 1;
+}
+
+XD_RULE_HD double nkb_pad(const NkbGrid& g) { return g.w * 0x1p-20 + (fabs(g.lo0) + (double)NKB_B * g.w) * 0x1p-48; }
+template <typename T> XD_RULE_HD T nkb_round_down(double x);
+template <typename T> XD_RULE_HD T nkb_round_up(double x);
+template <> XD_RULE_HD double nkb_round_down<double>(double x) { return x; }
+template <> XD_RULE_HD double nkb_round_up<double>(double x) { return x; }
+template <> XD_RULE_HD float nkb_round_down<float>(double x) { const float e = (float)x; return (double)e > x ? nextafterf(e, -INFINITY) : e; }
+template <> XD_RULE_HD float nkb_round_up<float>(double x) { const float e = (float)x; return (double)e < x ? nextafterf(e, INFINITY) : e; }
+template <typename T> XD_RULE_HD T nkb_edge_lo(const NkbGrid& g, int k) { return nkb_round_down<T>(g.lo0 + (double)(k - 1) * g.w - nkb_pad(g)); }
+template <typename T> XD_RULE_HD T nkb_edge_hi(const NkbGrid& g, int k) { return nkb_round_up<T>(g.lo0 + (double)k * g.w + nkb_pad(g)); }
+
+struct NkbBracket { uint64_t count, below, upto, r, h; int k_lo, k_hi, flag; };
+XD_RULE_HD int nkb_counter_of_rank(const uint32_t* incl, uint64_t rank) {
+    int lo = 0, hi = NKB_ROW - 1;
+    while (lo < hi) {
+        const int mid = (lo + hi) >> 1;
+        if ((uint64_t)incl[mid] > rank) hi = mid;
+        else lo = mid + 1;
+    }
+    return lo;
+}
+XD_RULE_HD NkbBracket nkb_bracket(const uint32_t* incl , uint32_t narrow, const NkbGrid& g) {
+    NkbBracket o;
+    const uint64_t total = incl[NKB_ROW - 1];
+    o.count = total; o.below = 0; o.upto = 0; o.r = 0; o.h = 0; o.k_lo = 0; o.k_hi = NKB_B + 1; o.flag = 0;
+    if (total == 0) return o;
+    const uint64_t r = (total - 1) / 2, h = sel_narrowed(sel_bracket_halfwidth(total), narrow);
+    const uint64_t r_lo = r > h ? r - h : 0, r_hi = (r + h < total) ? r + h : total - 1;
+    o.r = r; o.h = h;
+    o.k_lo = nkb_counter_of_rank(incl, r_lo);
+    o.k_hi = nkb_counter_of_rank(incl, r_hi);
+    o.below = o.k_lo > 0 ? incl[o.k_lo - 1] : 0;
+    o.upto = incl[o.k_hi];
+    o.flag = (o.k_lo < 1 || o.k_hi > NKB_B || !(g.w > 0.0)) ? 1 : 0;
+    return o;
+}
+
+}
diff --git a/xdem_amd/csrc/nk_onepass.h b/xdem_amd/csrc/nk_onepass.h
--- a/xdem_amd/csrc/nk_onepass.h
+++ b/xdem_amd/csrc/nk_onepass.h
@@ -95,6 +95,39 @@
 }
 
 template <typename T>
+__device__ __forceinline__ void nk_slot_y(T d, int64_t p, int64_t n, const T* __restrict__ slope_tan, const nk_bin_t* __restrict__ bcache, T vhat, T& y,
+                                          uint16_t& b) {
+    y = (T)NAN;
+    b = 0xFFFF;
+    if (p < n && d == d) {
+        b = nk_bin16(bcache[p]);
+        y = t_div(t_sub(d, vhat), slope_tan[p]);
+        if (b == 0xFFFF || !(y == y)) y = (T)NAN;
+    }
+}
+template <typename T>
+__device__ __forceinline__ void nk_slot_dy(const T* __restrict__ ref_m, const T* __restrict__ tba, const NkGeom& g, int64_t q0, int64_t p, int64_t n,
+                                           double invW, const T* __restrict__ slope_tan, const nk_bin_t* __restrict__ bcache, T vhat, T& y, uint16_t& b) {
+    y = (T)NAN;
+    b = 0xFFFF;
+    if (p < n) {
+        const int64_t q = q0 + p;
+        int64_t li, j;
+        row_col(q, g.W, invW, li, j);
+        const BiTap t = bi_locate(g, li + g.roff, j);
+        const BiVals<T> tv = bi_load<T>(tba, t);
+        T val;
+        const bool in = bi_value<T>(g, tba, t, tv.a00, tv.a01, tv.a10, tv.a11, val);
+        const T d = t_sub(ref_m[q], val);
+        if (in && t_finite(d)) {
+            b = nk_bin16(bcache[p]);
+            y = t_div(t_sub(d, vhat), slope_tan[p]);
+            if (b == 0xFFFF || !(y == y)) y = (T)NAN;
+        }
+    }
+}
+
+template <typename T>
 __global__ __launch_bounds__(256) void nk_sample_y_kernel(T* __restrict__ s_v, uint16_t* __restrict__ s_b, const T* __restrict__ slope_tan,
                                                           const nk_bin_t* __restrict__ bcache, int64_t n, int64_t n_slots, const T* vhat_p,
                                                           const typename KeyT<T>::type* klo_d = nullptr, const typename KeyT<T>::type* khi_d = nullptr,
@@ -117,14 +150,9 @@
     if (reset.base) select_reset_slice(reset, (int64_t)blockIdx.x * blockDim.x + threadIdx.x, (int64_t)gridDim.x * blockDim.x);
     for (int64_t i = (int64_t)blockIdx.x * blockDim.x + threadIdx.x; i < n_slots; i += (int64_t)gridDim.x * blockDim.x) {
         const int64_t p = (sel_sampled_line(i >> SEL_LINE_LOG2) << SEL_LINE_LOG2) + (i & (SEL_LINE - 1));
-        const T d = s_v[i];
-        T y = (T)NAN;
-        uint16_t b = 0xFFFF;
-        if (p < n && d == d) {
-            b = nk_bin16(bcache[p]);
-            y = t_div(t_sub(d, vhat), slope_tan[p]);
-            if (b == 0xFFFF || !(y == y)) y = (T)NAN;
-        }
+        T y;
+        uint16_t b;
+        nk_slot_y<T>(s_v[i], p, n, slope_tan, bcache, vhat, y, b);
         s_v[i] = y;
         s_b[i] = b;
     }
@@ -148,23 +176,9 @@
     if (reset.base) select_reset_slice(reset, (int64_t)blockIdx.x * blockDim.x + threadIdx.x, (int64_t)gridDim.x * blockDim.x);
     for (int64_t i = (int64_t)blockIdx.x * blockDim.x + threadIdx.x; i < n_slots; i += (int64_t)gridDim.x * blockDim.x) {
         const int64_t p = (sel_sampled_line(i >> SEL_LINE_LOG2) << SEL_LINE_LOG2) + (i & (SEL_LINE - 1));
-        T y = (T)NAN;
-        uint16_t b = 0xFFFF;
-        if (p < n) {
-            const int64_t q = q0 + p;
-            int64_t li, j;
-            row_col(q, g.W, invW, li, j);
-            const BiTap t = bi_locate(g, li + g.roff, j);
-            const BiVals<T> tv = bi_load<T>(tba, t);
-            T val;
-            const bool in = bi_value<T>(g, tba, t, tv.a00, tv.a01, tv.a10, tv.a11, val);
-            const T d = t_sub(ref_m[q], val);
-            if (in && t_finite(d)) {
-                b = nk_bin16(bcache[p]);
-                y = t_div(t_sub(d, vhat), slope_tan[p]);
-                if (b == 0xFFFF || !(y == y)) y = (T)NAN;
-            }
-        }
+        T y;
+        uint16_t b;
+        nk_slot_dy<T>(ref_m, tba, g, q0, p, n, invW, slope_tan, bcache, vhat, y, b);
         s_v[i] = y;
         s_b[i] = b;
     }
@@ -201,6 +215,156 @@
         if (!(pr.dlo <= pr.dhi) || !nk_vhat_of<T>(1u, lo, hi, v, d)) ctr[3] = 1ull;
         *vhat = v;
         *delta = d;
+    }
+}
+
+constexpr int NKB_THREADS = 1024;
+constexpr int NKB_OUTER_COPIES = 16;
+constexpr int NKB_SLOTS_PER_THREAD_MAX = 60;
+static_assert(NKB_THREADS * NKB_SLOTS_PER_THREAD_MAX < 65536 && NKB_B % 2 == 0, "16-bit counters, two to a word");
+struct NkbMapArg { double lo0[NK_PREDICT_MAX_BINS], inv_w[NK_PREDICT_MAX_BINS]; };
+struct NkbEdgeArg { double lo0[NK_PREDICT_MAX_BINS], w[NK_PREDICT_MAX_BINS]; };
+inline size_t nkb_sample_lds(int nb) { return (size_t)nb * (16 + 4 * (NKB_B / 2 + 2 * NKB_OUTER_COPIES)); }
+inline size_t nkb_finish_lds(int nb) { return (size_t)nb * (8 + 4 * NKB_ROW); }
+inline int nkb_sample_grid(const xdemhip_ctx* ctx, int64_t n_slots) {
+    const int64_t need = (n_slots + (int64_t)NKB_THREADS * NKB_SLOTS_PER_THREAD_MAX - 1) / ((int64_t)NKB_THREADS * NKB_SLOTS_PER_THREAD_MAX);
+    const int g = grid_for(ctx, n_slots, NKB_THREADS, 2);
+    return need > g ? (int)need : g;
+}
+template <typename T, bool FROM_DH >
+__global__ __launch_bounds__(NKB_THREADS) void nk_bucket_sample_kernel(const T* __restrict__ ref_m, const T* __restrict__ tba, NkGeom g, int64_t q0, int64_t n,
+                                                                       double invW, int64_t n_slots, const T* __restrict__ s_d,
+                                                                       const T* __restrict__ slope_tan , const nk_bin_t* __restrict__ bcache ,
+                                                                       const typename KeyT<T>::type* klo_d, const typename KeyT<T>::type* khi_d, T* vhat_out,
+                                                                       T* delta_out, unsigned long long* ctr, const NkbMapArg grids, int nb,
+                                                                       uint32_t* __restrict__ table ) {
+    typedef typename KeyT<T>::type K;
+    extern __shared__ __attribute__((aligned(16))) unsigned char fz_smem[];
+    double* s_lo0 = reinterpret_cast<double*>(fz_smem);
+    double* s_inv = s_lo0 + nb;
+    uint32_t* c = reinterpret_cast<uint32_t*>(s_inv + nb);
+    uint32_t* outer = c + nb * (NKB_B / 2);
+    T vhat, delta;
+    const K lo = klo_d[0], hi = khi_d[0];
+    const bool ok = nk_vhat_of<T>((lo == (K)0 && hi == (K)~(K)0) ? 0u : 1u, lo, hi, vhat, delta);
+    if (blockIdx.x == 0 && threadIdx.x == 0) {
+        *vhat_out = vhat;
+        *delta_out = delta;
+        if (!ok) ctr[3] = 1ull;
+    }
+    for (int k = threadIdx.x; k < nb; k += blockDim.x) { s_lo0[k] = grids.lo0[k]; s_inv[k] = grids.inv_w[k]; }
+    for (int k = threadIdx.x; k < nb * (NKB_B / 2 + 2 * NKB_OUTER_COPIES); k += blockDim.x) c[k] = 0u;
+    __syncthreads();
+    const int copy = threadIdx.x & (NKB_OUTER_COPIES - 1);
+    for (int64_t i = (int64_t)blockIdx.x * blockDim.x + threadIdx.x; i < n_slots; i += (int64_t)gridDim.x * blockDim.x) {
+        const int64_t p = (sel_sampled_line(i >> SEL_LINE_LOG2) << SEL_LINE_LOG2) + (i & (SEL_LINE - 1));
+        T y;
+        uint16_t b;
+        if (FROM_DH) nk_slot_y<T>(s_d[i], p, n, slope_tan, bcache, vhat, y, b);
+        else nk_slot_dy<T>(ref_m, tba, g, q0, p, n, invW, slope_tan, bcache, vhat, y, b);
+        if (y == y && (int)b < nb) {
+            NkbGrid gb;
+            gb.lo0 = s_lo0[b]; gb.inv_w = s_inv[b]; gb.w = 0.0;
+            const int k = nkb_bucket((double)y, gb);
+            if (k == 0) atomicAdd(&outer[((int)b * 2 + 0) * NKB_OUTER_COPIES + copy], 1u);
+            else if (k == NKB_B + 1) atomicAdd(&outer[((int)b * 2 + 1) * NKB_OUTER_COPIES + copy], 1u);
+            else atomicAdd(&c[(int)b * (NKB_B / 2) + ((k - 1) >> 1)], 1u << (16 * ((k - 1) & 1)));
+        }
+    }
+    __syncthreads();
+    for (int k = threadIdx.x; k < nb * NKB_B; k += blockDim.x) {
+        const int b = k / NKB_B, pos = k - b * NKB_B;
+        const uint32_t v = (c[k >> 1] >> (16 * (k & 1))) & 0xFFFFu;
+        if (v) atomicAdd(&table[b * NKB_ROW + 1 + pos], v);
+    }
+    for (int k = threadIdx.x; k < nb * 2; k += blockDim.x) {
+        const uint32_t* o = outer + k * NKB_OUTER_COPIES;
+        uint32_t v = 0;
+#pragma unroll
+        for (int q = 0; q < NKB_OUTER_COPIES; ++q) v += o[q];
+        if (v) atomicAdd(&table[(k >> 1) * NKB_ROW + ((k & 1) ? NKB_B + 1 : 0)], v);
+    }
+}
+
+template <typename T>
+__global__ __launch_bounds__(NKB_THREADS) void nk_bucket_finish_kernel(uint32_t* __restrict__ table, const NkbEdgeArg grids, int nb, uint32_t narrow,
+                                                                       typename KeyT<T>::type* klo, typename KeyT<T>::type* khi, uint32_t* rbs,
+                                                                       uint32_t* __restrict__ info, unsigned long long* ctr) {
+    typedef typename KeyT<T>::type K;
+    extern __shared__ __attribute__((aligned(16))) unsigned char fz_smem[];
+    K* range = reinterpret_cast<K*>(fz_smem);
+    uint32_t* rows = reinterpret_cast<uint32_t*>(fz_smem + (size_t)nb * 8);
+    constexpr int U = 8;
+    for (int k0 = threadIdx.x; k0 < nb * NKB_ROW; k0 += blockDim.x * U) {
+        uint32_t v[U];
+#pragma unroll
+        for (int u = 0; u < U; ++u) {
+            const int k = k0 + u * (int)blockDim.x;
+            v[u] = k < nb * NKB_ROW ? table[k] : 0u;
+        }
+#pragma unroll
+        for (int u = 0; u < U; ++u) {
+            const int k = k0 + u * (int)blockDim.x;
+            if (k < nb * NKB_ROW) { rows[k] = v[u]; if (v[u]) table[k] = 0u; }
+        }
+    }
+    __syncthreads();
+    const int lane = threadIdx.x & 63, wave = threadIdx.x >> 6, n_waves = blockDim.x >> 6;
+    constexpr int PER_LANE = (NKB_ROW + 63) / 64;
+    for (int b = wave; b < nb; b += n_waves) {
+        uint32_t* row = rows + b * NKB_ROW;
+        uint32_t v[PER_LANE], mine = 0;
+#pragma unroll
+        for (int q = 0; q < PER_LANE; ++q) {
+            const int k = lane * PER_LANE + q;
+            v[q] = k < NKB_ROW ? row[k] : 0u;
+            mine += v[q];
+        }
+        uint32_t incl = mine;
+#pragma unroll
+        for (int off = 1; off < 64; off <<= 1) {
+            const uint32_t t = __shfl_up(incl, off);
+            if (lane >= off) incl += t;
+        }
+        uint32_t run = incl - mine;
+#pragma unroll
+        for (int q = 0; q < PER_LANE; ++q) {
+            const int k = lane * PER_LANE + q;
+            run += v[q];
+            if (k < NKB_ROW) row[k] = run;
+        }
+        __builtin_amdgcn_wave_barrier();
+        __builtin_amdgcn_fence(__ATOMIC_ACQ_REL, "wavefront");
+        if (lane == 0) {
+            NkbGrid gb;
+            gb.lo0 = grids.lo0[b]; gb.w = grids.w[b]; gb.inv_w = 0.0;
+            const NkbBracket br = nkb_bracket(row, narrow, gb);
+            K lo = (K)0, hi = (K)~(K)0;
+            int flag = br.flag;
+            if (br.count > 0 && !flag) {
+                const T vlo = nkb_edge_lo<T>(gb, br.k_lo), vhi = nkb_edge_hi<T>(gb, br.k_hi);
+                if (vlo <= vhi && t_finite(vlo) && t_finite(vhi)) { lo = key_of(vlo); hi = key_of(vhi); }
+                else flag = 1;
+            }
+            if (br.count > 0 && flag) ctr[7] = 1ull;
+            klo[b] = lo;
+            khi[b] = hi;
+            range[b] = hi >= lo ? (K)(hi - lo) : (K)0;
+            info[4 * b + 0] = (uint32_t)br.count;
+            info[4 * b + 1] = (uint32_t)br.below;
+            info[4 * b + 2] = (uint32_t)br.upto;
+            info[4 * b + 3] = (uint32_t)flag;
+        }
+    }
+    __syncthreads();
+    if (wave == 0) {
+        K r = 0;
+        for (int k = lane; k < nb; k += 64) r = range[k] > r ? range[k] : r;
+        for (int off = 32; off > 0; off >>= 1) {
+            const K o = k_shfl_down(r, off);
+            r = o > r ? o : r;
+        }
+        if (lane == 0) *rbs = rebase_shift_of(r);
     }
 }
 
@@ -244,6 +408,7 @@
                                                        double* wg_sums ,
                                                        const uint64_t* __restrict__ badbits = nullptr, int64_t bad_wpr = 0) {
     typedef typename KeyT<T>::type K;
+    if (ctr[7] != 0) return;
     constexpr int SEG = NKZ_CAP / 4;
     static_assert(SEG >= 2 * 64, "a segment holds at least two rows of candidates");
     constexpr int SEG_D = 128;
diff --git a/xdem_amd/csrc/nuthkaab.hip b/xdem_amd/csrc/nuthkaab.hip
--- a/xdem_amd/csrc/nuthkaab.hip
+++ b/xdem_amd/csrc/nuthkaab.hip
@@ -7,6 +7,7 @@
 #include "select.h"
 #include "select_run.h"
 #include "nk_geom.h"
+#include "nk_buckets.h"
 #include "nk_aux.h"
 #include "rank_select.h"
 
@@ -439,6 +440,9 @@
     double pr_st = 0;
     std::vector<double> pr_med, pr_w, pr_mid;
     std::vector<unsigned char> pr_ok;
+    std::vector<unsigned char> pr_empty;
+    uint32_t* nkb_table = nullptr;
+    int64_t n_bucketed = 0, n_bucket_fallback = 0;
     double pr_err = 1e30, pr_err_d = 1e30;
     double pr_dpx = 1e30;
     int pr_cooldown = 0;
@@ -637,7 +641,8 @@
 
 template <typename T>
 int nk_step_onepass(xdemhip_nk_plan* P, const NkGeom& g, int64_t q0, int64_t n, int nb, bool* done, double* vshift, int64_t* n_valid,
-                    double* y_mean, double* y_std, double* edges_out, int64_t* counts, double* medians, bool allow_predict = true) {
+                    double* y_mean, double* y_std, double* edges_out, int64_t* counts, double* medians, bool allow_predict = true,
+                    bool allow_buckets = true) {
     typedef typename KeyT<T>::type K;
     *done = false;
     xdemhip_ctx* ctx = P->ctx;
@@ -733,6 +738,30 @@
     const bool predict_d = !predict && allow_predict && ctx->nk_predict != 0 && P->pr_have && P->pr_nb == nb && P->pr_cooldown == 0 &&
                            pr_expect_d <= 0.35 && dpx <= 0.6 && P->pr_wd > 0;
     if (P->pr_cooldown > 0 && allow_predict) --P->pr_cooldown;
+    bool buckets = allow_buckets && !predict && !mr && ctx->nk_bucket_brackets != 0 && P->nkb_table && P->pr_have && P->pr_nb == nb &&
+                   nb <= NK_PREDICT_MAX_BINS && (int)P->pr_w.size() == nb && (int)P->pr_empty.size() == nb &&
+                   nkb_sample_lds(nb) <= 64 * 1024 && nkb_finish_lds(nb) <= 128 * 1024;
+    NkbMapArg nkb_map;
+    NkbEdgeArg nkb_edge;
+    const int nkb_per_w = dpx <= 0.2 ? NKB_PER_W : NKB_PER_W / 2;
+    for (int b = 0; buckets && b < nb; ++b) {
+        NkbGrid gb = {0.0, 0.0, 0.0};
+        if (P->pr_ok[b]) {
+            gb = nkb_grid(P->pr_med[b] - (dE * sin(P->pr_mid[b]) + dN * cos(P->pr_mid[b])), P->pr_w[b], nkb_per_w);
+            if (!(gb.w > 0.0)) buckets = false;
+        } else if (!P->pr_empty[b]) {
+            buckets = false;
+        }
+        nkb_map.lo0[b] = nkb_edge.lo0[b] = gb.lo0;
+        nkb_map.inv_w[b] = gb.inv_w;
+        nkb_edge.w[b] = gb.w;
+    }
+    constexpr double NKB_MAX_MOVE_PX = 0.55;
+    if (buckets && dpx > NKB_MAX_MOVE_PX && ctx->nk_bucket_brackets != 2) {
+        buckets = false;
+        ++P->n_bucket_fallback;
+    }
+    uint32_t* nkb_info = P->nkb_table ? P->nkb_table + (size_t)nbm * NKB_ROW : nullptr;
     double pr_h = 1.0;
     T* s_v = static_cast<T*>(ws->s_vals);
     bool fused = false;
@@ -789,6 +818,26 @@
         rc = edges_and_bins();
         if (rc) return rc;
     }
+    if (buckets) {
+        const size_t lds_s = nkb_sample_lds(nb), lds_f = nkb_finish_lds(nb);
+        const int grid_s = nkb_sample_grid(ctx, n_slots);
+        if (predict_d) {
+            rc = set_big_lds(ctx, nk_bucket_sample_kernel<T, false>, lds_s);
+            if (rc) return rc;
+            hipLaunchKernelGGL((nk_bucket_sample_kernel<T, false>), dim3(grid_s), dim3(NKB_THREADS), lds_s, ctx->stream, ref_m, tba, g, q0, n, 1.0 / (double)P->W,
+                               n_slots, static_cast<const T*>(nullptr), st_all + q0, P->bcache + q0, klo_d, khi_d, d_vhat, d_delta, ctr, nkb_map, nb, P->nkb_table);
+        } else {
+            rc = set_big_lds(ctx, nk_bucket_sample_kernel<T, true>, lds_s);
+            if (rc) return rc;
+            hipLaunchKernelGGL((nk_bucket_sample_kernel<T, true>), dim3(grid_s), dim3(NKB_THREADS), lds_s, ctx->stream, ref_m, tba, g, q0, n, 1.0 / (double)P->W,
+                               n_slots, static_cast<const T*>(s_v), st_all + q0, P->bcache + q0, klo_d, khi_d, d_vhat, d_delta, ctr, nkb_map, nb, P->nkb_table);
+        }
+        rc = set_big_lds(ctx, nk_bucket_finish_kernel<T>, lds_f);
+        if (rc) return rc;
+        hipLaunchKernelGGL((nk_bucket_finish_kernel<T>), dim3(1), dim3(NKB_THREADS), lds_f, ctx->stream, P->nkb_table, nkb_edge, nb, (uint32_t)narrow, klo_y, khi_y,
+                           rbs_y, nkb_info, ctr);
+        XD_HIP_CHECK(ctx, hipGetLastError());
+    } else {
     if (predict_d)
         hipLaunchKernelGGL((nk_sample_dy_kernel<T>), dim3(grid_for(ctx, n_slots, 256, 8)), dim3(256), 0, ctx->stream, ref_m, tba, g, q0, n,
                            1.0 / (double)P->W, n_slots, s_v, ws->s_bins, st_all + q0, P->bcache + q0, klo_d, khi_d, d_vhat, d_delta, ctr,
@@ -802,6 +851,7 @@
     if (rc) return rc;
     if (!fused) hipLaunchKernelGGL((bracket_finish_kernel<K>), dim3(1), dim3(64), 0, ctx->stream, d_st, nb, 0, low_mask, klo_y, khi_y, rbs_y);
     XD_HIP_CHECK(ctx, hipGetLastError());
+    }
     }
     int n_wg = 0;
     {
@@ -929,17 +979,18 @@
     std::vector<SelState<K>> h_st(nb);
     std::vector<uint64_t> h_succ(nb);
     std::vector<uint64_t> cnt_t(mr ? 3 * (size_t)nb : 0);
+    std::vector<uint32_t> h_nkb(buckets ? 4 * (size_t)nb : 0);
     std::vector<K> khi(nb);
     K h_kd[2] = {0, 0};
-    const int n_pk = mr ? 14 : 13;
+    const int n_pk = (mr || buckets) ? 14 : 13;
     {
         FzPack pk;
         void* dsts[14] = {cnt.data(), klo.data(), h_ctr, &h_rbs, info, sums, &h_vhat, edges.data(), h_st.data(), h_succ.data(), khi.data(), &h_kd[0], &h_kd[1],
-                          cnt_t.data()};
+                          buckets ? (void*)h_nkb.data() : (void*)cnt_t.data()};
         const void* srcs[14] = {cnt_y, klo_y, ctr, rbs_y, scratch + OFF_INFO, d_sums, d_vhat, d_edges, scratch + OFF_STATE, scratch + off_succ(nb), khi_y, klo_d,
-                                khi_d, cnt_true};
+                                khi_d, buckets ? (const void*)nkb_info : (const void*)cnt_true};
         const size_t sizes[14] = {8 * 3 * (size_t)nb, sizeof(K) * nb, 128, 8, 32, 40, sizeof(T), sizeof(T) * (nb + 1), sizeof(SelState<K>) * nb, 8 * (size_t)nb,
-                                  sizeof(K) * nb, sizeof(K), sizeof(K), 8 * 3 * (size_t)nb};
+                                  sizeof(K) * nb, sizeof(K), sizeof(K), buckets ? 16 * (size_t)nb : 8 * 3 * (size_t)nb};
         uint32_t off = 0;
         pk.n = n_pk;
         for (int k = 0; k < n_pk; ++k) {
@@ -960,6 +1011,11 @@
     }
     std::vector<SelResult<K>> hs(nb);
     for (int k = 0; k < nb; ++k) { hs[k].st = h_st[k]; hs[k].succ = h_succ[k]; }
+    if (buckets && h_ctr[7] != 0) {
+        ++P->n_bucket_fallback;
+        if (getenv("XDEMHIP_DEBUG")) fprintf(stderr, "[xdemhip] one-pass step: bucket brackets fall back to the stored sample (shift change %.2e px)\n", dpx);
+        return nk_step_onepass<T>(P, g, q0, n, nb, done, vshift, n_valid, y_mean, y_std, edges_out, counts, medians, false, false);
+    }
     if ((h_ctr[2] != 0 || h_ctr[3] != 0) && getenv("XDEMHIP_DEBUG"))
         fprintf(stderr, "[xdemhip] one-pass step falls through: overflow flag %llu, miss flag %llu, dh candidates %llu, bin candidates %llu\n", h_ctr[2], h_ctr[3],
                 h_ctr[1], h_ctr[5]);
@@ -992,8 +1048,19 @@
             P->fz_offn += 1;
         };
         if (!predict_d) take(h_ctr[10], h_ctr[11], h_ctr[12]);
+        auto take_buckets = [&](uint64_t tot, uint64_t lt, uint64_t in, const uint32_t* rep) {
+            if (tot < 4096 || in < 64 || in >= tot || rep[0] == 0 || rep[2] <= rep[1]) return;
+            const double span = (double)(rep[2] - rep[1]), r = (double)((rep[0] - 1) / 2);
+            const double h = (double)sel_narrowed(sel_bracket_halfwidth(rep[0]), (uint32_t)narrow);
+            const double centre = (double)lt + (double)in * ((r + 0.5 - (double)rep[1]) / span);
+            const double o = fabs((double)(tot - 1) * 0.5 - centre) / ((double)in * h / span) * unit;
+            worst = o > worst ? o : worst;
+            P->fz_off2 += o * o;
+            P->fz_offn += 1;
+        };
         for (int b = 0; b < nb; ++b) {
             if (mr) take(cnt_t[b], cnt_t[nb + b], cnt_t[2 * nb + b]);
+            else if (buckets) take_buckets(cnt[b], cnt[nb + b], cnt[2 * nb + b], &h_nkb[4 * (size_t)b]);
             else take(cnt[b], cnt[nb + b], cnt[2 * nb + b]);
         }
         P->fz_worst = worst > P->fz_worst ? worst : P->fz_worst;
@@ -1053,6 +1120,9 @@
             if (getenv("XDEMHIP_DEBUG"))
                 fprintf(stderr, "[xdemhip] one-pass step (%s, half widths x %.2f): shift change %.2e px, centres off by %.3f (bins) / %.3f (dh) sampled half widths\n",
                         predict ? "PREDICTED brackets" : (predict_d ? "sampled brackets, PREDICTED bracket of the median of dh" : "sampled brackets"), pr_h, dpx, P->pr_err, P->pr_err_d);
+            if (getenv("XDEMHIP_DEBUG"))
+                fprintf(stderr, "[xdemhip] one-pass step: bin brackets from %s, %llu bin candidates, %llu dh candidates\n", buckets ? "value buckets" : (predict ? "the prediction" : "the stored sample"),
+                        h_ctr[5], h_ctr[1]);
         } else {
             P->pr_err = P->pr_err_d = 1e30;
             P->pr_dpx = 1e30;
@@ -1061,13 +1131,16 @@
             const double norm = narrow >= (int)SEL_NARROW_16THS ? 0.5 / sel_narrow_unit((uint32_t)narrow) : 1.0;
             P->pr_w.assign(nb, 0.0);
             for (int b = 0; b < nb; ++b)
-                if (counts[b] > 0 && khi[b] >= klo[b]) P->pr_w[b] = norm * 0.5 * ((double)val_of(khi[b]) - (double)val_of(klo[b]));
+                if (counts[b] > 0 && khi[b] >= klo[b])
+                    P->pr_w[b] = norm * fmax(0.0, 0.5 * ((double)val_of(khi[b]) - (double)val_of(klo[b])) - (buckets ? 0.5 * nkb_edge.w[b] : 0.0));
             if (!predict_d) P->pr_wd = h_kd[1] >= h_kd[0] ? norm * 0.5 * ((double)val_of(h_kd[1]) - (double)val_of(h_kd[0])) : 0.0;
         }
         P->pr_med.assign(medians, medians + nb);
         P->pr_mid = mid;
         P->pr_ok.assign(nb, 0);
         for (int b = 0; b < nb; ++b) P->pr_ok[b] = (counts[b] > 0 && P->pr_w[b] > 0 && std::isfinite(P->pr_w[b]) && std::isfinite(medians[b])) ? 1 : 0;
+        P->pr_empty.assign(nb, 0);
+        for (int b = 0; b < nb; ++b) P->pr_empty[b] = counts[b] == 0 ? 1 : 0;
         P->pr_v = vs;
         P->pr_st = sums[2] > 0 ? cntd / sums[2] : 0.0;
         P->pr_sx = g.dc;
@@ -1076,6 +1149,7 @@
         P->pr_have = true;
         if (predict) ++P->n_predicted;
         if (predict_d) ++P->n_predicted_d;
+        if (buckets) ++P->n_bucketed;
     }
     *done = true;
     return XDEMHIP_OK;
@@ -1360,6 +1434,13 @@
             if (P->fz_pack) (void)hipFree(P->fz_pack);
             P->fz = nullptr; P->cd_vals = nullptr; P->c_st = nullptr; P->fz_pack = nullptr;
         }
+        const size_t nkb_bytes = (size_t)P->ws.nb_max * (NKB_ROW + 4) * 4;
+        if (P->fz && (hipMalloc(reinterpret_cast<void**>(&P->nkb_table), nkb_bytes) != hipSuccess ||
+                      hipMemsetAsync(P->nkb_table, 0, nkb_bytes, ctx->stream) != hipSuccess)) {
+            (void)hipGetLastError();
+            if (P->nkb_table) (void)hipFree(P->nkb_table);
+            P->nkb_table = nullptr;
+        }
     }
     if (P->nan_rule >= 2 && (int64_t)n >= SEL_BRACKET_MIN_N) {
         P->bad_wpr = (W + 63) / 64 + 2;
@@ -1396,7 +1477,7 @@
     if (P->own_inputs) { (void)hipFree(P->ref); (void)hipFree(P->tba); if (inl_created) (void)hipFree(inl_created); }
     if (P->sub_inlier) (void)hipFree(P->sub_inlier);
     void* bufs[] = {P->slope_tan, P->aspect, P->dh, P->y, P->valid, P->bins, P->bcache, P->scratch, P->ref_m, P->ext_idx, P->ext_cnt,
-                    P->fz, P->cd_vals, P->c_st, P->fz_pack, P->badbits, P->mr_a, P->mr_b, P->mr_small, P->wg_sums};
+                    P->fz, P->cd_vals, P->c_st, P->fz_pack, P->nkb_table, P->badbits, P->mr_a, P->mr_b, P->mr_small, P->wg_sums};
     for (void* b : bufs)
         if (b) (void)hipFree(b);
     xd::sel_ws_free(P->ws);
@@ -1478,6 +1559,13 @@
     if (predicted) *predicted = P->n_predicted;
     if (predicted_dh_only) *predicted_dh_only = P->n_predicted_d;
     if (missed) *missed = P->n_predict_miss;
+    return XDEMHIP_OK;
+}
+
+int xdemhip_nk_bracket_counts(xdemhip_nk_plan* P, int64_t* bucketed, int64_t* fell_back) {
+    if (!P) return XDEMHIP_EINVAL;
+    if (bucketed) *bucketed = P->n_bucketed;
+    if (fell_back) *fell_back = P->n_bucket_fallback;
     return XDEMHIP_OK;
 }
 
diff --git a/xdem_amd/csrc/sel_rule.h b/xdem_amd/csrc/sel_rule.h
--- /dev/null
+++ b/xdem_amd/csrc/sel_rule.h
@@ -0,0 +1,25 @@
+#pragma once
+#include <math.h>
+#include <stdint.h>
+
+#if defined(__HIPCC__)
+#define XD_RULE_HD __host__ __device__ inline
+#else
+#define XD_RULE_HD inline
+#endif
+
+namespace xd {
+
+XD_RULE_HD uint64_t sel_bracket_halfwidth(uint64_t m) {
+    return (uint64_t)(3.0 * sqrt(8.0 * (double)m)) + 32;
+}
+constexpr uint32_t SEL_NARROW_16THS = 16;
+XD_RULE_HD uint64_t sel_narrowed(uint64_t h_full, uint32_t narrow) {
+    const uint64_t w = h_full - 32;
+    return (narrow < SEL_NARROW_16THS ? (w >> narrow) : ((w * (uint64_t)(narrow - SEL_NARROW_16THS)) >> 4)) + 32;
+}
+XD_RULE_HD double sel_narrow_unit(uint32_t narrow) {
+    return narrow < SEL_NARROW_16THS ? 1.0 / (double)(1u << narrow) : (double)(narrow - SEL_NARROW_16THS) / 16.0;
+}
+
+}
diff --git a/xdem_amd/csrc/select.h b/xdem_amd/csrc/select.h
--- a/xdem_amd/csrc/select.h
+++ b/xdem_amd/csrc/select.h
@@ -2,6 +2,8 @@
 #include <hip/hip_runtime.h>
 #include <math.h>
 #include <stdint.h>
+
+#include "sel_rule.h"
 
 namespace xd {
 
@@ -42,17 +44,6 @@
 enum { SEL_MEDIAN = 0, SEL_BRACKET_LO = 1, SEL_BRACKET_HI = 2, SEL_GIVEN = 3, SEL_BRACKET_LO_WIDE = 4, SEL_BRACKET_HI_WIDE = 5,
        SEL_BRACKET_DUAL = 6  };
 
-__host__ __device__ inline uint64_t sel_bracket_halfwidth(uint64_t m) {
-    return (uint64_t)(3.0 * sqrt(8.0 * (double)m)) + 32;
-}
-constexpr uint32_t SEL_NARROW_16THS = 16;
-__host__ __device__ inline uint64_t sel_narrowed(uint64_t h_full, uint32_t narrow) {
-    const uint64_t w = h_full - 32;
-    return (narrow < SEL_NARROW_16THS ? (w >> narrow) : ((w * (uint64_t)(narrow - SEL_NARROW_16THS)) >> 4)) + 32;
-}
-__host__ __device__ inline double sel_narrow_unit(uint32_t narrow) {
-    return narrow < SEL_NARROW_16THS ? 1.0 / (double)(1u << narrow) : (double)(narrow - SEL_NARROW_16THS) / 16.0;
-}
 constexpr uint32_t PAIR_DEFF_WIDE = 4096, PAIR_DEFF_SPREAD = 4;
 __host__ __device__ inline uint64_t sel_bracket_halfwidth_wide(uint64_t m, uint32_t deff = PAIR_DEFF_WIDE) {
     return (uint64_t)(3.0 * sqrt((double)deff * (double)m)) + 64;
```
